# Borda/pyImSegm

Measured on AMD Instinct MI355X. Metric: Mpixels/s end-to-end SLIC+fts+GC, 2048x2048 RGB; % HBM roofline, higher is better.
Workload: dtype f64; 1 GPU; single 2048x2048 RGB uint8 per GPU, SLIC(sp_size=46, K=2025, 10 sweeps) + colour mean/std/energy + 3-class alpha-expansion GC (gc_regul=2.0, edge=model), pre-fitted GMM, host numpy in -> segm int32 in host numpy (BASELINE configs[1]); bench_config=2, images_per_launch_chain=1, images_in_flight_per_gpu=4, hardware_queues=4, input_memory=pageable numpy, input_ring=default (one rank: measured in round 4), parallelism=images sharded over 1 GPU(s), 4 in flight per GPU (one HIP stream each)

## Files before the change

include/imsegm_hip.h:

```cpp
#ifndef IMSEGM_HIP_H
#define IMSEGM_HIP_H

#include <stddef.h>
#include <stdint.h>

#ifdef __cplusplus
extern "C" {
#endif

#define IMSEGM_API __attribute__((visibility("default")))

#define IMSEGM_U8 0
#define IMSEGM_F64 1
#define IMSEGM_F32 2

#define IMSEGM_E_FUSED_PATH (-3)

#define IMSEGM_E_FIT_CAPS (-4)

typedef struct imsegm_ctx imsegm_ctx;
typedef struct imsegm_image2d imsegm_image2d;

IMSEGM_API const char *imsegm_last_error(void);
IMSEGM_API int imsegm_version(void);
IMSEGM_API int imsegm_device_count(int *count_out);
IMSEGM_API int imsegm_device_pci_bus_id(int device, char *id_out, int capacity);
IMSEGM_API int imsegm_device_mem_info(int device, size_t *free_bytes_out, size_t *total_bytes_out);
IMSEGM_API int imsegm_init(int hardware_queues);
IMSEGM_API void imsegm_debug_reload_env(void);

IMSEGM_API int imsegm_host_alloc(size_t bytes, void **ptr_out);
IMSEGM_API void imsegm_host_free(void *ptr);

IMSEGM_API int imsegm_device_alloc(int device, size_t bytes, void **ptr_out);
IMSEGM_API void imsegm_device_free(void *ptr);
IMSEGM_API int imsegm_set_device(int device);

IMSEGM_API int imsegm_ctx_create(int device, imsegm_ctx **ctx_out);
IMSEGM_API void imsegm_ctx_destroy(imsegm_ctx *ctx);
IMSEGM_API int imsegm_ctx_synchronize(imsegm_ctx *ctx);
IMSEGM_API int imsegm_ctx_stream(imsegm_ctx *ctx, void **hip_stream_out);
IMSEGM_API int imsegm_ctx_copy(imsegm_ctx *ctx, void *dst, const void *src, size_t bytes, int synchronize);

IMSEGM_API int imsegm_ctx_profile_enable(imsegm_ctx *ctx, int enable);
IMSEGM_API int imsegm_ctx_profile_reset(imsegm_ctx *ctx);
IMSEGM_API int imsegm_ctx_profile_get(imsegm_ctx *ctx, int group, double *total_ms_out, int *count_out);

IMSEGM_API int imsegm_image2d_create(imsegm_ctx *ctx, int height, int width, imsegm_image2d **img_out);
IMSEGM_API void imsegm_image2d_destroy(imsegm_image2d *img);

IMSEGM_API int imsegm_image2d_upload(imsegm_image2d *img, const void *host_pixels, int dtype);

IMSEGM_API int imsegm_image2d_slic(imsegm_image2d *img, int minmax_normalize, int n_segments, double compactness,
                        const double *taps_z, int radius_z, const double *taps_y, int radius_y,
                        const double *taps_x, int radius_x, int max_iter, int enforce_connectivity,
                        double min_size_factor, double max_size_factor, int start_label,
                        int max_candidates, int slic_zero, int *n_labels_out);

IMSEGM_API int imsegm_image2d_get_labels(imsegm_image2d *img, int64_t *labels_out);
IMSEGM_API int imsegm_image2d_set_labels(imsegm_image2d *img, const int32_t *labels, int n_labels);
IMSEGM_API long imsegm_debug_conn_general_runs(void);
IMSEGM_API int imsegm_debug_slic_sweep_runs(long *persistent_runs_out, long *fallback_runs_out);
IMSEGM_API long imsegm_debug_gc_grid_fallbacks(void);
IMSEGM_API int imsegm_image2d_enforce_connectivity(imsegm_image2d *img, const int32_t *labels, long min_size, long max_size,
                                                   int start_label, int *n_labels_out);
IMSEGM_API int imsegm_image2d_label_hist(imsegm_image2d *img, const int32_t *annot, int nb_annot, int64_t *hist_out);
IMSEGM_API int imsegm_image2d_get_lab(imsegm_image2d *img, double *lab_out);
IMSEGM_API int imsegm_image2d_get_nearest(imsegm_image2d *img, int32_t *nearest_out);

IMSEGM_API int imsegm_image2d_color_stats(imsegm_image2d *img, double *mean_out, double *energy_out, double *var_out);

IMSEGM_API int imsegm_image2d_graph(imsegm_image2d *img, int32_t *edges_out, int edge_capacity, int *n_edges_out,
                         double *centres_out, uint8_t *present_out);

IMSEGM_API int imsegm_image2d_gather(imsegm_image2d *img, const int32_t *graph_labels, const double *proba,
                          int n_classes, int32_t *segm_out, double *soft_out);

IMSEGM_API int imsegm_image2d_lm_features(imsegm_image2d *img, const double *weights, const int *n_kernels, int n_batteries, int radius,
                                          double clip, int feature_mask, double *features_out);

IMSEGM_API int imsegm_image2d_lm_features_sep(imsegm_image2d *img, const double *weights, const int *n_kernels, const int *dense_parity,
                                              const double *sep_taps, const int *sep_groups, const int *sep_rank, int n_batteries,
                                              int radius, double clip, int feature_mask, double *features_out);

IMSEGM_API int imsegm_image2d_lm_prepare(imsegm_image2d *img, const double *taps, int radius, const double *channel_mix);
IMSEGM_API int imsegm_image2d_lm_battery(imsegm_image2d *img, const double *weights, int n_kernels, int radius,
                                         double clip, double *sum_squares_out);
IMSEGM_API int imsegm_image2d_response_stats(imsegm_image2d *img, double mul, double div, double *mean_out,
                                             double *energy_out, double *var_out);
IMSEGM_API int imsegm_image2d_response_median(imsegm_image2d *img, double mul, double div, double *median_out);
IMSEGM_API int imsegm_image2d_response_mean_gradient(imsegm_image2d *img, double mul, double div, double *mean_out);
IMSEGM_API int imsegm_image2d_get_response(imsegm_image2d *img, double *planes_out);

IMSEGM_API int imsegm_volume_create(imsegm_ctx *ctx, int depth, int height, int width, imsegm_image2d **vol_out);
IMSEGM_API int imsegm_volume_upload(imsegm_image2d *vol, const void *host_voxels, int dtype, double slic_offset,
                                    double slic_scale);
IMSEGM_API int imsegm_volume_slic(imsegm_image2d *vol, int n_segments, double compactness, const double *taps_z,
                                  int radius_z, const double *taps_y, int radius_y, const double *taps_x, int radius_x,
                                  const double *spacing, int max_iter, int enforce_connectivity, double min_size_factor,
                                  double max_size_factor, int start_label, int *n_labels_out);
IMSEGM_API int imsegm_volume_label_cc(imsegm_image2d *vol, int *n_labels_out);
IMSEGM_API int imsegm_volume_gray_stats(imsegm_image2d *vol, double *mean_out, double *energy_out, double *var_out);
IMSEGM_API int imsegm_volume_graph(imsegm_image2d *vol, int32_t *edges_out, int edge_capacity, int *n_edges_out,
                                   double *centres_out, uint8_t *present_out);

IMSEGM_API int imsegm_image2d_features_color(imsegm_image2d *img, int feature_mask, double *features_out);

IMSEGM_API int imsegm_image2d_features_place(imsegm_image2d *img, int total_columns, int column);
IMSEGM_API int imsegm_image2d_get_features(imsegm_image2d *img, double *features_out, int capacity_columns);

typedef struct {
    int n_features, n_classes;
    const double *scaler_mean;
    const double *scaler_scale;
    const double *prec_chol;
    const double *mu_proj;
    const double *log_det;
    const double *log_weights;
    double const_term;
} imsegm_gmm;

#define IMSEGM_EDGE_CONST 0
#define IMSEGM_EDGE_SPATIAL 1
#define IMSEGM_EDGE_MODEL_LT 2
#define IMSEGM_EDGE_MODEL_L1 3
#define IMSEGM_EDGE_MODEL_L2 4
#define IMSEGM_EDGE_FEATURES 5
#define IMSEGM_EDGE_SPATIAL_NORM 0x100

typedef struct {
    int edge_capacity;
    int n_edges;
    int32_t *edges;
    double *edge_weights;
    int32_t *edge_weights_int;
    double *unary;
    int32_t *unary_int;
    double *centres;
    int64_t *energy;
    int keep_soft_on_device;
    int segm_u8;
    int soft_f32;
} imsegm_terms_debug;

// ... 66 lines not shown
```

pyimsegm_amd/_hip.py:

```python
import ctypes as C
import functools
import os
import threading

import numpy as np

_HERE = os.path.dirname(os.path.abspath(__file__))
LIB_PATH = os.environ.get('IMSEGM_HIP_LIBRARY') or os.path.join(_HERE, 'libimsegm_hip.so')

U8, F64, F32 = 0, 1, 2
PROFILE_GROUPS = {
    'slic_assign': 0,
    'slic': 1,
    'connectivity': 2,
    'color_stats': 3,
    'graph': 4,
    'graphcut': 5,
    'gather': 6,
    'slic_preprocess': 7,
    'terms': 8,
    'texture': 9,
}


class HipUnavailableError(RuntimeError):
    """the HIP library or a HIP device is not available (no CPU fallback exists)"""


class HipError(RuntimeError):
    """a C-ABI call returned an error status"""


class HipFusedPathError(HipError):
    """``IMSEGM_E_FUSED_PATH`` of include/imsegm_hip.h: the fused back half (``imsegm_image2d_segment`` /
    ``imsegm_image2d_graph_prepare``) does not apply to this label map on this device -- nothing is wrong with the session, the
    caller takes the staged calls (graph, terms, ``cut_general_graph``, gather) instead"""


class HipFitCapsError(HipError):
    """``IMSEGM_E_FIT_CAPS`` of include/imsegm_hip.h: the table or the model is outside the caps of the device fit
    (``imsegm_kmeans_lloyd`` / ``imsegm_mixture_em``: 16 features, 8 components, 16 restarts; the ``_wide`` pair: 17 to 256
    features, 8 components, 16 restarts) -- nothing is wrong with the context, the caller fits on the host"""


IMSEGM_E_FUSED_PATH = -3
IMSEGM_E_FIT_CAPS = -4


_lib = None
_lib_lock = threading.Lock()

_vp = C.c_void_p
_ip = C.POINTER(C.c_int)

class GmmParams(C.Structure):
    _fields_ = [('n_features', C.c_int), ('n_classes', C.c_int), ('scaler_mean', _vp), ('scaler_scale', _vp),
                ('prec_chol', _vp), ('mu_proj', _vp), ('log_det', _vp), ('log_weights', _vp), ('const_term', C.c_double)]


class TermsDebug(C.Structure):
    _fields_ = [('edge_capacity', C.c_int), ('n_edges', C.c_int), ('edges', _vp), ('edge_weights', _vp),
                ('edge_weights_int', _vp), ('unary', _vp), ('unary_int', _vp), ('centres', _vp), ('energy', _vp),
                ('keep_soft_on_device', C.c_int), ('segm_u8', C.c_int), ('soft_f32', C.c_int)]


EDGE_TYPES = {'': 0, 'const': 0, 'spatial': 1 | 0x100, 'model': 2 | 0x100, 'model_lT': 2, 'model_l1': 3, 'model_l2': 4,
              'features': 5 | 0x100}

_SIGNATURES = {
    'imsegm_last_error': (C.c_char_p, []),
    'imsegm_host_alloc': (C.c_int, [C.c_size_t, C.POINTER(_vp)]),
    'imsegm_host_free': (None, [_vp]),
    'imsegm_device_alloc': (C.c_int, [C.c_int, C.c_size_t, C.POINTER(_vp)]),
    'imsegm_device_free': (None, [_vp]),
    'imsegm_set_device': (C.c_int, [C.c_int]),
    'imsegm_ctx_stream': (C.c_int, [_vp, C.POINTER(_vp)]),
    'imsegm_ctx_copy': (C.c_int, [_vp, _vp, _vp, C.c_size_t, C.c_int]),
    'imsegm_image2d_features_color': (C.c_int, [_vp, C.c_int, _vp]),
    'imsegm_image2d_features_place': (C.c_int, [_vp, C.c_int, C.c_int]),
    'imsegm_image2d_get_features': (C.c_int, [_vp, _vp, C.c_int]),
    'imsegm_image2d_run_color': (C.c_int, [_vp, _vp, C.c_int, C.c_int, C.c_int, C.c_double, _vp, C.c_int, C.c_int, C.c_int, C.c_int,
                                           C.c_int, C.POINTER(GmmParams), C.c_int, _vp, C.c_int, C.c_double, C.c_int, _vp, _vp, _vp, _ip]),
    'imsegm_device_mem_info': (C.c_int, [C.c_int, C.POINTER(C.c_size_t), C.POINTER(C.c_size_t)]),
    'imsegm_image2d_graph_prepare': (C.c_int, [_vp]),
    'imsegm_image2d_segment': (C.c_int, [_vp, C.POINTER(GmmParams), _vp, C.c_int, _vp, C.c_int, C.c_double, C.c_int, _vp, _vp, _vp,
                                         _vp, _vp, C.POINTER(TermsDebug)]),
    'imsegm_version': (C.c_int, []),
    'imsegm_device_count': (C.c_int, [_ip]),
    'imsegm_ctx_create': (C.c_int, [C.c_int, C.POINTER(_vp)]),
    'imsegm_ctx_destroy': (None, [_vp]),
    'imsegm_ctx_synchronize': (C.c_int, [_vp]),
    'imsegm_ctx_profile_enable': (C.c_int, [_vp, C.c_int]),
    'imsegm_ctx_profile_reset': (C.c_int, [_vp]),
    'imsegm_ctx_profile_get': (C.c_int, [_vp, C.c_int, C.POINTER(C.c_double), _ip]),
    'imsegm_image2d_create': (C.c_int, [_vp, C.c_int, C.c_int, C.POINTER(_vp)]),
    'imsegm_image2d_destroy': (None, [_vp]),
    'imsegm_image2d_upload': (C.c_int, [_vp, _vp, C.c_int]),
    'imsegm_image2d_slic': (C.c_int, [_vp, C.c_int, C.c_int, C.c_double, _vp, C.c_int, _vp, C.c_int, _vp, C.c_int,
                                      C.c_int, C.c_int, C.c_double, C.c_double, C.c_int, C.c_int, C.c_int, _ip]),
    'imsegm_image2d_get_labels': (C.c_int, [_vp, _vp]),
    'imsegm_image2d_set_labels': (C.c_int, [_vp, _vp, C.c_int]),
    'imsegm_image2d_enforce_connectivity': (C.c_int, [_vp, _vp, C.c_long, C.c_long, C.c_int, _vp]),
    'imsegm_debug_conn_general_runs': (C.c_long, []),
    'imsegm_debug_slic_sweep_runs': (C.c_int, [_vp, _vp]),
    'imsegm_debug_gc_grid_fallbacks': (C.c_long, []),
    'imsegm_assume_bg_on_boundary': (C.c_int, [_vp, _vp, C.c_int, C.c_int, _vp, C.c_int, _ip]),
    'imsegm_image2d_all_finite': (C.c_int, [_vp, _ip]),
    'imsegm_image2d_lm_features': (C.c_int, [_vp, _vp, _vp, C.c_int, C.c_int, C.c_double, C.c_int, _vp]),
    'imsegm_batch2d_create': (C.c_int, [_vp, C.c_int, C.c_int, C.c_int, C.POINTER(_vp)]),
    'imsegm_batch2d_destroy': (None, [_vp]),
    'imsegm_batch2d_run_color': (C.c_int, [_vp, C.c_int, _vp, C.c_int, C.c_int, C.c_int, C.c_double, _vp, C.c_int, C.c_int, C.c_int,
                                           C.c_int, _vp, C.c_int, _vp, C.c_int, C.c_double, C.c_int, _vp, _vp, _vp]),
    'imsegm_batch2d_device_ptr': (C.c_int, [_vp, C.c_int, C.c_int, C.POINTER(_vp)]),
    'imsegm_device_pci_bus_id': (C.c_int, [C.c_int, C.c_char_p, C.c_int]),
    'imsegm_init': (C.c_int, [C.c_int]),
    'imsegm_debug_reload_env': (None, []),
    'imsegm_image2d_label_hist': (C.c_int, [_vp, _vp, C.c_int, _vp]),
    'imsegm_image2d_get_lab': (C.c_int, [_vp, _vp]),
    'imsegm_image2d_get_nearest': (C.c_int, [_vp, _vp]),
    'imsegm_image2d_color_stats': (C.c_int, [_vp, _vp, _vp, _vp]),
    'imsegm_image2d_graph': (C.c_int, [_vp, _vp, C.c_int, _ip, _vp, _vp]),
    'imsegm_image2d_gather': (C.c_int, [_vp, _vp, _vp, C.c_int, _vp, _vp]),
    'imsegm_image2d_lm_prepare': (C.c_int, [_vp, _vp, C.c_int, _vp]),
    'imsegm_image2d_lm_features_sep': (C.c_int, [_vp, _vp, _vp, _vp, _vp, _vp, _vp, C.c_int, C.c_int, C.c_double, C.c_int, _vp]),
    'imsegm_image2d_lm_battery': (C.c_int, [_vp, _vp, C.c_int, C.c_int, C.c_double, C.POINTER(C.c_double)]),
    'imsegm_image2d_response_stats': (C.c_int, [_vp, C.c_double, C.c_double, _vp, _vp, _vp]),
    'imsegm_image2d_response_median': (C.c_int, [_vp, C.c_double, C.c_double, _vp]),
    'imsegm_image2d_response_mean_gradient': (C.c_int, [_vp, C.c_double, C.c_double, _vp]),
    'imsegm_image2d_get_response': (C.c_int, [_vp, _vp]),
    'imsegm_image2d_device_ptr': (C.c_int, [_vp, C.c_int, C.POINTER(_vp)]),
    'imsegm_volume_create': (C.c_int, [_vp, C.c_int, C.c_int, C.c_int, C.POINTER(_vp)]),
    'imsegm_volume_upload': (C.c_int, [_vp, _vp, C.c_int, C.c_double, C.c_double]),
    'imsegm_volume_slic': (C.c_int, [_vp, C.c_int, C.c_double, _vp, C.c_int, _vp, C.c_int, _vp, C.c_int, _vp, C.c_int,
                                     C.c_int, C.c_double, C.c_double, C.c_int, _ip]),
    'imsegm_volume_label_cc': (C.c_int, [_vp, _ip]),
    'imsegm_volume_gray_stats': (C.c_int, [_vp, _vp, _vp, _vp]),
    'imsegm_volume_graph': (C.c_int, [_vp, _vp, C.c_int, _ip, _vp, _vp]),
    'imsegm_image2d_median': (C.c_int, [_vp, _vp]),
    'imsegm_image2d_mean_gradient': (C.c_int, [_vp, _vp]),
    'imsegm_label_hist2d': (C.c_int, [_vp, _vp, C.c_int, C.c_int, _vp, C.c_int, _vp, C.c_int, C.c_int, C.c_int, _vp]),
    'imsegm_ray_features_binary2d': (C.c_int, [_vp, _vp, C.c_int, C.c_int, _vp, C.c_int, _vp, C.c_int, C.c_int, _vp]),
    'imsegm_cut_general_graph': (C.c_int, [_vp, _vp, C.c_int, _vp, _vp, C.c_int, C.c_int, _vp, C.c_int, _vp,
                                           C.POINTER(C.c_int64)]),
    'imsegm_kmeans_lloyd': (C.c_int, [_vp, _vp, C.c_long, C.c_int, _vp, C.c_int, C.c_int, C.c_int, C.c_double, _vp, _vp, _vp, _vp, _vp]),
    'imsegm_mixture_em': (C.c_int, [_vp, C.c_int, C.c_int, _vp, _vp, _vp, _vp, C.c_double, C.c_double, C.c_int, _vp, _vp, _vp, _vp,
                                    _vp, _vp, _vp, _vp]),
    'imsegm_kmeans_lloyd_wide': (C.c_int, [_vp, _vp, C.c_long, C.c_int, _vp, C.c_int, C.c_int, C.c_int, C.c_double, _vp, _vp, _vp, _vp,
                                           _vp]),
    'imsegm_mixture_em_wide': (C.c_int, [_vp, C.c_int, C.c_int, _vp, _vp, _vp, _vp, C.c_double, C.c_double, C.c_int, _vp, _vp, _vp, _vp,
                                         _vp, _vp, _vp, _vp]),
}

EXPORTED_SYMBOLS = tuple(_SIGNATURES)


def load_library():
    global _lib
    with _lib_lock:
        if _lib is None:
            if not os.path.exists(LIB_PATH):
                raise HipUnavailableError(
                    'libimsegm_hip.so is not built (%s); run `python -m pyimsegm_amd.build`' % LIB_PATH)
            try:
                lib = C.CDLL(LIB_PATH)
            except OSError as ex:
                raise HipUnavailableError('cannot load %s: %s' % (LIB_PATH, ex))
            for name, (res, args) in _SIGNATURES.items():
                fn = getattr(lib, name)
                fn.restype = res
                fn.argtypes = args
            _lib = lib
    return _lib


def init(hardware_queues=8):
    status = load_library().imsegm_init(int(hardware_queues))
    if status < 0:
        raise HipError(load_library().imsegm_last_error().decode('utf-8', 'replace'))
    if status == 0:
        os.environ.setdefault('GPU_MAX_HW_QUEUES', str(int(hardware_queues)))
    return status == 0


def device_pci_bus_id(device=0):
    buf = C.create_string_buffer(64)
    _check(load_library().imsegm_device_pci_bus_id(int(device), buf, 64))
# ... 398 lines not shown
                        or not segm_out.flags.c_contiguous or not segm_out.flags.writeable:
                    raise ValueError('segm_out must be a writeable C-contiguous %s array of shape %r' % (want_dtype, tuple(self.shape)))
                out['segm'] = segm_out
            else:
                out['segm'] = alloc(self.shape, want_dtype)
        if want_soft:
            out['soft'] = alloc(self.shape + (nc, ), np.float32 if soft_f32 else np.float64)
        if want_graph_labels or debug:
            out['graph_labels'] = np.empty(k, dtype=np.int32)
        if want_proba or debug:
            out['proba'] = np.empty((k, nc), dtype=np.float64)
        dbg = None
        if debug or keep_soft_on_device or segm_u8 or soft_f32:
            dbg = TermsDebug()
            dbg.keep_soft_on_device = int(bool(keep_soft_on_device))
            dbg.segm_u8, dbg.soft_f32 = int(segm_u8), int(soft_f32)
        if debug:
            cap = (16 if len(self.shape) == 3 else 3) * k + 64
            ndim = len(self.shape)
            out.update(edges=np.empty((cap, 2), np.int32), edge_weights=np.empty(cap), edge_weights_int=np.empty(cap, np.int32),
                       unary=np.empty((k, nc)), unary_int=np.empty((k, nc), np.int32), centres=np.empty((k, ndim)),
                       energy=np.zeros(1, np.int64))
            dbg.edge_capacity = cap
            for name in ('edges', 'edge_weights', 'edge_weights_int', 'unary', 'unary_int', 'centres', 'energy'):
                setattr(dbg, name, _ptr(out[name]))
        _check(load_library().imsegm_image2d_segment(
            self._h, C.byref(gmm.params) if gmm is not None else None, _ptr(pr), nc, _ptr(pairwise), code, float(edge_cost),
            int(bool(use_graphcut)), _ptr(cl), _ptr(out.get('segm')), _ptr(out.get('soft')), _ptr(out.get('graph_labels')),
            _ptr(out.get('proba')), C.byref(dbg) if dbg is not None else None))
        if debug:
            ne = dbg.n_edges
            for name in ('edges', 'edge_weights', 'edge_weights_int'):
                out[name] = out[name][:ne]
            out['energy'] = int(out['energy'][0])
        return out

    def slic(self, n_segments, compactness, sigma=1., normalize=2, max_iter=10, enforce_connectivity=True,
             min_size_factor=0.5, max_size_factor=3., start_label=0, max_candidates=0, slic_zero=False):
        taps = gaussian_taps(sigma)
        r = -1 if taps is None else len(taps) - 1
        n_out = C.c_int(0)
        _check(load_library().imsegm_image2d_slic(
            self._h, int(normalize), int(n_segments), float(compactness), _ptr(taps), r, _ptr(taps), r, _ptr(taps), r,
            int(max_iter), int(bool(enforce_connectivity)), float(min_size_factor), float(max_size_factor),
            int(start_label), int(max_candidates), int(bool(slic_zero)), C.byref(n_out)))
        self.n_labels = n_out.value
        return self.n_labels

    def get_labels(self):
        out = np.empty(self.shape, dtype=np.int64)
        _check(load_library().imsegm_image2d_get_labels(self._h, _ptr(out)))
        return out

    def get_labels_int32(self):
        out = np.empty(self.shape, dtype=np.int32)
        src = _device_array(self, 0, self.shape, '<i4').__cuda_array_interface__['data'][0]
        self.ctx.copy(out.ctypes.data, src, out.nbytes, synchronize=True)
        return out

    def enforce_connectivity(self, labels, min_size, max_size, start_label=0):
        labels = np.ascontiguousarray(labels, dtype=np.int32)
        if labels.shape != self.shape:
            raise ValueError('label map %r does not match image %r' % (labels.shape, self.shape))
        n_out = C.c_int(0)
        _check(load_library().imsegm_image2d_enforce_connectivity(self._h, _ptr(labels), int(min_size), int(max_size),
                                                                  int(start_label), C.byref(n_out)))
        self.n_labels = n_out.value
        return self.get_labels()

    def set_labels(self, labels, n_labels=None):
        labels = np.ascontiguousarray(labels, dtype=np.int32)
        if labels.shape != self.shape:
            raise ValueError('label map %r does not match image %r' % (labels.shape, self.shape))
        if labels.size and labels.min() < 0:
            raise ValueError('labels must be non-negative')
        if n_labels is None:
            n_labels = int(labels.max()) + 1
        elif labels.size and int(labels.max()) >= n_labels:
            raise ValueError('label %d is out of range for n_labels = %d' % (int(labels.max()), n_labels))
        _check(load_library().imsegm_image2d_set_labels(self._h, _ptr(labels), int(n_labels)))
        self.n_labels = int(n_labels)
        return self

    def label_hist(self, annot, nb_annot=None):
        annot = np.ascontiguousarray(annot, dtype=np.int32)
        if annot.shape != self.shape:
            raise ValueError('annotation %r does not match the session %r' % (annot.shape, self.shape))
        if nb_annot is None:
            nb_annot = int(annot.max()) + 1 if annot.size else 1
        out = np.empty((self.n_labels, int(nb_annot)), dtype=np.int64)
        _check(load_library().imsegm_image2d_label_hist(self._h, _ptr(annot), int(nb_annot), _ptr(out)))
        return out

    def get_lab(self):
        out = np.empty((3,) + self.shape, dtype=np.float64)
        _check(load_library().imsegm_image2d_get_lab(self._h, _ptr(out)))
        return out

    def get_nearest(self):
        out = np.empty(self.shape, dtype=np.int32)
        _check(load_library().imsegm_image2d_get_nearest(self._h, _ptr(out)))
        return out

    def color_stats(self, mean=True, energy=True, var=True):
        k = self.n_labels
        m = np.empty((k, 3), dtype=np.float64) if mean else None
        e = np.empty((k, 3), dtype=np.float64) if energy else None
        v = np.empty((k, 3), dtype=np.float64) if var else None
        _check(load_library().imsegm_image2d_color_stats(self._h, _ptr(m), _ptr(e), _ptr(v)))
        return m, e, v

    def lm_prepare(self, sigma=150.):
        taps = gaussian_taps(sigma)
        radius = len(taps) - 1
        full = np.concatenate([taps[:0:-1], taps])
        mix = np.zeros((3, 3))
        for c_out in range(3):
            for j in range(-radius, radius + 1):
                i = (c_out + j) % 6
                mix[c_out, i if i < 3 else 5 - i] += full[j + radius]
        _check(load_library().imsegm_image2d_lm_prepare(self._h, _ptr(taps), radius, _ptr(np.ascontiguousarray(mix))))
        return self

    def lm_battery(self, battery, clip):
        battery = np.asarray(battery, dtype=np.float64)
        nk, side = battery.shape[0], battery.shape[1]
        if battery.ndim != 3 or battery.shape[2] != side or side % 2 != 1:
            raise ValueError('wrong battery dim %r' % (battery.shape, ))
        pad = {1: 1, 2: 2, 3: 4, 4: 4, 5: 8, 6: 8, 7: 8, 8: 8}.get(nk)
        if pad is None:
            raise ValueError('at most 8 kernels per battery')
        if pad != nk:
            battery = np.concatenate([battery, np.repeat(battery[-1:], pad - nk, axis=0)], axis=0)
        weights = np.ascontiguousarray(battery[:, ::-1, ::-1].transpose(2, 1, 0))
        ssq = C.c_double(0)
        _check(load_library().imsegm_image2d_lm_battery(self._h, _ptr(weights), pad, side // 2, float(clip), C.byref(ssq)))
        return float(np.sqrt(ssq.value))

    @staticmethod
    def _battery_weights(battery):
        battery = np.asarray(battery, dtype=np.float64)
        nk, side = battery.shape[0], battery.shape[1]
        if battery.ndim != 3 or battery.shape[2] != side or side % 2 != 1:
            raise ValueError('wrong battery dim %r' % (battery.shape, ))
        pad = {1: 1, 2: 2, 3: 4, 4: 4, 5: 8, 6: 8, 7: 8, 8: 8}.get(nk)
        if pad is None:
            raise ValueError('at most 8 kernels per battery')
        if pad != nk:
            battery = np.concatenate([battery, np.repeat(battery[-1:], pad - nk, axis=0)], axis=0)
        return np.ascontiguousarray(battery[:, ::-1, ::-1].transpose(2, 1, 0)), pad, side // 2

    SEPARABLE_TOLERANCE, SEPARABLE_MAX_RANK = 1e-13, 2

    MIRROR_TOLERANCE = 1e-12

    @classmethod
    def _mirror_pairs(cls, dense):
        left = list(range(len(dense)))
        pairs = []
        while left:
            a = left.pop(0)
            mirrored = dense[a][:, ::-1]
            bound = cls.MIRROR_TOLERANCE * np.abs(dense[a]).max()
            for b in left:
                hit = [m for m in (1., -1.) if np.abs(dense[b] - m * mirrored).max() <= bound]
                if hit:
# ... 493 lines not shown
```

pyimsegm_amd/csrc/api.hip:

```cpp
#include "../../include/imsegm_hip.h"
#include "slic.h"

#include <atomic>
#include <cstdio>
#include <cstdlib>
#include <cstring>
#include <vector>

namespace imsegm {

static thread_local std::string g_error;

void set_error(const std::string &msg) { g_error = msg; }

bool hip_ok(hipError_t e, const char *what, const char *file, int line)
{
    if (e == hipSuccess) return true;
    char buf[512];
    snprintf(buf, sizeof(buf), "HIP error %d (%s) in `%s` at %s:%d", (int)e, hipGetErrorString(e), what, file, line);
    g_error = buf;
    return false;
}

static Knobs read_knobs()
{
    auto flag = [](const char *n) { return getenv(n) != nullptr; };
    auto num = [](const char *n, int dflt) { const char *e = getenv(n); return e ? atoi(e) : dflt; };
    Knobs k;
    k.slic_graph = flag("IMSEGM_SLIC_GRAPH");
    k.pre_3pass = flag("IMSEGM_PRE_3PASS");
    k.separate_finalize = flag("IMSEGM_SEPARATE_FINALIZE");
    k.fuse_finalize = flag("IMSEGM_FUSE_FINALIZE");
    k.conn_general = flag("IMSEGM_CONN_GENERAL");
    k.gc_no_topo_regs = flag("IMSEGM_GC_NO_TOPO_REGS");
    k.sep_wide_tile = flag("IMSEGM_SEP_WIDE_TILE");
    k.cc_merge_full = flag("IMSEGM_CC_MERGE_FULL");
    k.label_general = flag("IMSEGM_LABEL_GENERAL");
    k.terms_one_workgroup = flag("IMSEGM_TERMS_ONE_WORKGROUP");
    k.adjacency_table = flag("IMSEGM_ADJACENCY_TABLE");
    k.brick_cap = num("IMSEGM_BRICK_CAP", 0);
    k.gc_lds_level = num("IMSEGM_GC_LDS_LEVEL", 4);
    k.gc_threads = num("IMSEGM_GC_THREADS", 0);
    k.gc_grid_min_sites = num("IMSEGM_GC_GRID_MIN_SITES", 0);
    k.gc_grid_blocks = num("IMSEGM_GC_GRID_BLOCKS", 0);
    k.gc_one_workgroup = flag("IMSEGM_GC_ONE_WORKGROUP");
    k.gc_grid_test_absent = flag("IMSEGM_GC_GRID_TEST_ABSENT");
    k.fused_bitmap_mb = num("IMSEGM_FUSED_BITMAP_MB", 0);
    const char *d = getenv("IMSEGM_PHASE_DUMP");
    k.phase_dump = d ? d : "";
    return k;
}
static std::atomic<const Knobs *> g_knobs{ nullptr };
const Knobs &knobs()
{
    const Knobs *k = g_knobs.load(std::memory_order_acquire);
    if (!k) {
        const Knobs *fresh = new Knobs(read_knobs());
        if (g_knobs.compare_exchange_strong(k, fresh, std::memory_order_acq_rel)) k = fresh;
        else delete fresh;
    }
    return *k;
}
void reload_knobs() { g_knobs.store(new Knobs(read_knobs()), std::memory_order_release); }

}

#include "session.h"

std::atomic<bool> g_runtime_started{ false };

extern "C" {

int imsegm_host_alloc(size_t bytes, void **ptr_out)
{
    g_runtime_started.store(true);
    if (!ptr_out) {
        set_error("null argument");
        return -1;
    }
    HIP_TRY(hipHostMalloc(ptr_out, bytes ? bytes : 1, hipHostMallocDefault));
    return 0;
}

void imsegm_host_free(void *ptr)
{
    if (ptr) (void)hipHostFree(ptr);
}

int imsegm_device_alloc(int device, size_t bytes, void **ptr_out)
{
    g_runtime_started.store(true);
    if (!ptr_out) {
        set_error("null argument");
        return -1;
    }
    HIP_TRY(hipSetDevice(device));
    HIP_TRY(hipMalloc(ptr_out, bytes ? bytes : 1));
    return 0;
}

void imsegm_device_free(void *ptr)
{
    if (ptr) (void)hipFree(ptr);
}

int imsegm_set_device(int device)
{
    g_runtime_started.store(true);
    HIP_TRY(hipSetDevice(device));
    return 0;
}

int imsegm_ctx_stream(imsegm_ctx *ctx, void **stream_out)
{
    if (bind(ctx)) return -1;
    *stream_out = ctx->stream;
    return 0;
}

int imsegm_ctx_copy(imsegm_ctx *ctx, void *dst, const void *src, size_t bytes, int synchronize)
{
    if (bind(ctx)) return -1;
    HIP_TRY(hipMemcpyAsync(dst, src, bytes, hipMemcpyDefault, ctx->stream));
    if (synchronize) HIP_TRY(hipStreamSynchronize(ctx->stream));
    return 0;
}

const char *imsegm_last_error(void) { return g_error.c_str(); }
int imsegm_version(void) { return 100; }
// ... 84 lines not shown
    if (bind(ctx)) return -1;
    HIP_TRY(hipStreamSynchronize(ctx->stream));
    return 0;
}

int imsegm_ctx_profile_enable(imsegm_ctx *ctx, int enable)
{
    if (bind(ctx)) return -1;
    ctx->collect();
    ctx->profile = enable != 0;
    return 0;
}

int imsegm_ctx_profile_reset(imsegm_ctx *ctx)
{
    if (bind(ctx)) return -1;
    ctx->collect();
    for (int i = 0; i < PG_COUNT; ++i) {
        ctx->acc_ms[i] = 0;
        ctx->acc_n[i] = 0;
    }
    return 0;
}

int imsegm_ctx_profile_get(imsegm_ctx *ctx, int group, double *total_ms_out, int *count_out)
{
    if (bind(ctx)) return -1;
    if (group < 0 || group >= PG_COUNT) {
        set_error("bad profile group");
        return -1;
    }
    ctx->collect();
    *total_ms_out = ctx->acc_ms[group];
    *count_out = ctx->acc_n[group];
    return 0;
}

int imsegm_image2d_create(imsegm_ctx *ctx, int height, int width, imsegm_image2d **img_out)
{
    if (bind(ctx)) return -1;
    if (height <= 0 || width <= 0 || (long)height * width > 0x3fffffffL) {
        set_error("bad image size");
        return -1;
    }
    imsegm_image2d *im = new imsegm_image2d();
    im->ctx = ctx;
    im->H = height;
    im->W = width;
    im->n = (size_t)height * width;
    *img_out = im;
    return 0;
}

void imsegm_image2d_destroy(imsegm_image2d *im)
{
    if (!im) return;
    (void)hipSetDevice(im->ctx->device);
    (void)hipStreamSynchronize(im->ctx->stream);
    DevBuf *all[] = { &im->img, &im->labA, &im->labB, &im->nearest, &im->labels, &im->conn_i32, &im->conn_u8, &im->small,
                      &im->cent, &im->tiles, &im->feat, &im->graph, &im->gather_lut, &im->gather_out_i, &im->gather_out_f,
                      &im->tex_planes, &im->tex_resp, &im->tex_small, &im->tex_aux, &im->vol_cent, &im->annot, &im->hist, &im->featK, &im->seg,
                      &im->gseg, &im->narrow };
    for (auto b : all) b->release();
    if (im->slic_fail_host) (void)hipHostFree(im->slic_fail_host);
    if (im->slic_exec) (void)hipGraphExecDestroy(im->slic_exec);
    delete im;
}

int imsegm_image2d_upload(imsegm_image2d *im, const void *host_pixels, int dtype)
{
    if (!im || bind(im->ctx)) return -1;
    if (wrong_kind(im, false)) return -1;
    im->tex_ready = false;
    size_t es = dtype == IMSEGM_U8 ? 1 : dtype == IMSEGM_F32 ? 4 : dtype == IMSEGM_F64 ? 8 : 0;
    if (!es) {
        set_error("unsupported dtype");
        return -1;
    }
    size_t bytes = im->n * 3 * es;
    if (im->img.ensure(bytes + 16)) return -1;
    HIP_TRY(hipMemcpyAsync(im->img.p, host_pixels, bytes, hipMemcpyHostToDevice, im->ctx->stream));
    if (!is_pinned(host_pixels)) HIP_TRY(hipStreamSynchronize(im->ctx->stream));
    im->dtype = dtype;
    im->feat_mask = 0;
    im->place_F = 0;
    return 0;
}

long imsegm_debug_conn_general_runs(void) { return conn_general_runs(); }

void imsegm_debug_reload_env(void) { reload_knobs(); }

long imsegm_debug_gc_grid_fallbacks(void) { return gc_grid_fallbacks(); }

int imsegm_debug_slic_sweep_runs(long *persistent_runs_out, long *fallback_runs_out)
{
    slic_sweep_counters(persistent_runs_out, fallback_runs_out);
    return 0;
}

int imsegm_image2d_all_finite(imsegm_image2d *im, int *all_finite_out)
{
    if (!im || !all_finite_out || bind(im->ctx)) return -1;
    if (im->dtype < 0 || !im->img.p) {
        set_error("all_finite needs an uploaded image or volume");
        return -1;
    }
    *all_finite_out = 1;
    if (im->dtype == IMSEGM_U8) return 0;
    hipStream_t st = im->ctx->stream;
    if (ensure_small(im)) return -1;
    unsigned int *count = reinterpret_cast<unsigned int *>(im->small.as<unsigned char>() + 256);
    const size_t values = im->is_volume ? im->n : im->n * 3;
    if (launch_count_nonfinite(im->img.p, im->dtype, values, count, st)) return -1;
    unsigned int bad = 0;
    HIP_TRY(hipMemcpyAsync(&bad, count, sizeof(bad), hipMemcpyDeviceToHost, st));
    HIP_TRY(hipStreamSynchronize(st));
    *all_finite_out = bad == 0;
    return 0;
}

int imsegm_image2d_device_ptr(imsegm_image2d *im, int which, void **ptr_out)
{
    if (!im || !ptr_out) {
        set_error("null argument");
        return -1;
    }
    if (which == 3 && (!im->have_labels || im->feat_mask == 0 || im->feat_F < 1)) {
        set_error("device_ptr: no resident feature table");
        return -1;
    }
    DevBuf *b = which == 0 ? &im->labels : which == 1 ? &im->gather_out_i : which == 2 ? &im->gather_out_f :
                which == 3 ? &im->featK : nullptr;
    if (!b || !b->p) {
        set_error("device_ptr: buffer not available");
        return -1;
    }
    *ptr_out = b->p;
    return 0;
}


}
```

pyimsegm_amd/csrc/api_fused.hip:

```cpp
#include "backhalf.h"

int imsegm::take_placement(imsegm_image2d *im, int own_F, bool to_host, int *table_F, int *col0)
{
    *table_F = own_F;
    *col0 = 0;
    if (im->place_F <= 0) return 0;
    const int total = im->place_F, column = im->place_col;
    im->place_F = 0;
    if (column + own_F > total) {
        set_error("features_place: the columns of this descriptor group do not fit the table");
        return -1;
    }
    if (to_host && own_F != total) {
        set_error("features_place: a group placed into a wider table stays on the device (imsegm_image2d_get_features reads the table)");
        return -1;
    }
    *table_F = total;
    *col0 = column;
    return 0;
}

extern "C" {

int imsegm_cut_general_graph(imsegm_ctx *ctx, const int32_t *edges, int n_edges, const double *edge_weights,
// ... 29 lines not shown
        return -1;
    }
    int32_t *ui = (int32_t *)(host + o_u), *wi = (int32_t *)(host + o_w), *si = (int32_t *)(host + o_s);
    int32_t *he = (int32_t *)(host + o_e), *arc_start = (int32_t *)(host + o_as), *arc_to = (int32_t *)(host + o_at);
    int32_t *arc_rev = (int32_t *)(host + o_ar), *edge_arc = (int32_t *)(host + o_ea);
    double mu = 0, mw = 0, mp = -DBL_MAX;
    for (size_t i = 0; i < (size_t)K * C; ++i) mu = std::max(mu, fabs(unary_cost[i]));
    for (int i = 0; i < E; ++i) mw = std::max(mw, fabs(edge_weights[i]));
    for (int i = 0; i < C * C; ++i) mp = std::max(mp, pairwise_cost[i]);
    double dwf = ((E > 0 && mw * mp > mu) ? mw * mp : mu) + 1e-10;
    for (size_t i = 0; i < (size_t)K * C; ++i) ui[i] = (int32_t)((unary_cost[i] / dwf) * 100000);
    for (int i = 0; i < E; ++i) wi[i] = (int32_t)((edge_weights[i] / dwf) * 1000);
    for (int i = 0; i < C * C; ++i) si[i] = (int32_t)(pairwise_cost[i] * 100);
    int smax = 0;
    for (int i = 0; i < C * C; ++i) smax = std::max(smax, std::abs(si[i]));
    for (int i = 0; i < E; ++i)
        if ((long long)std::abs(wi[i]) * smax > 10000000LL) {
            set_error("cut_general_graph: smoothness term is larger than GCO_MAX_ENERGYTERM");
            return -1;
        }
    if (E > 0) memcpy(he, edges, (size_t)E * 8);
    for (int i = 0; i <= K; ++i) arc_start[i] = 0;
    for (int j = 0; j < E; ++j) {
        arc_start[edges[2 * j] + 1]++;
        arc_start[edges[2 * j + 1] + 1]++;
    }
    for (int i = 0; i < K; ++i) arc_start[i + 1] += arc_start[i];
    {
        std::vector<int32_t> fill(arc_start, arc_start + K);
        for (int j = 0; j < E; ++j) {
            int a = edges[2 * j], b = edges[2 * j + 1];
            int ia = fill[a]++, ib = fill[b]++;
            arc_to[ia] = b;
            arc_to[ib] = a;
            arc_rev[ia] = ib;
            arc_rev[ib] = ia;
            edge_arc[2 * j] = ia;
            edge_arc[2 * j + 1] = ib;
        }
    }
    unsigned char *dev = ctx->gc_buf.as<unsigned char>();
    void *work = dev;
    unsigned char *io = dev + work_bytes;
    int32_t *d_lab = (int32_t *)(io + o_lab);
    long long *d_energy = (long long *)(io + o_en);
    int32_t *d_status = (int32_t *)(io + o_st);
    HIP_TRY(hipMemcpyAsync(io, host, up_bytes, hipMemcpyHostToDevice, st));
    HIP_TRY(hipMemsetAsync(d_status, 0, 4, st));
    GcProblem p;
    p.K = K; p.C = C; p.E = E;
    p.edges = (int32_t *)(io + o_e); p.w = (int32_t *)(io + o_w); p.unary = (int32_t *)(io + o_u); p.smooth = (int32_t *)(io + o_s);
    p.metric = smooth_is_metric(si, C);
    int sp = ctx->begin(PG_GC);
    if (launch_alpha_expansion(p, (int32_t *)(io + o_as), (int32_t *)(io + o_at), (int32_t *)(io + o_ar), (int32_t *)(io + o_ea),
                               n_iter, d_lab, d_energy, d_status, work, st))
        return -1;
    ctx->end(sp);
    HIP_TRY(hipMemcpyAsync(host + o_lab, d_lab, io_bytes - o_lab, hipMemcpyDeviceToHost, st));
    HIP_TRY(hipStreamSynchronize(st));
    memcpy(labels_out, host + o_lab, (size_t)K * 4);
    long long energy = *reinterpret_cast<long long *>(host + o_en);
    const int32_t misc[4] = { K, E, 0, *reinterpret_cast<int32_t *>(host + o_st) };
    if (backhalf_status(misc, 1)) return -1;
    if (energy_out) *energy_out = energy;
    return 0;
}


int imsegm_image2d_features_color(imsegm_image2d *im, int feature_mask, double *features_out)
{
    if (!im || bind(im->ctx)) return -1;
    if (!im->have_labels || im->dtype < 0) {
        set_error("features_color needs an uploaded image and a label map");
        return -1;
    }
    if (feature_mask < 1 || feature_mask > 7) {
        set_error("features_color: feature_mask is a combination of 1 (mean), 2 (std), 4 (energy)");
        return -1;
    }
    imsegm_ctx *ctx = im->ctx;
    hipStream_t st = ctx->stream;
    const int K = im->n_labels;
    double maxabs = 255.0;
    if (im->dtype != IMSEGM_U8) {
        if (ensure_small(im)) return -1;
        unsigned long long *keys = im->small.as<unsigned long long>();
        double *minmax = reinterpret_cast<double *>(keys + 2);
        if (launch_minmax(im->img.p, im->dtype, im->is_volume ? im->n : im->n * 3, keys, minmax, st)) return -1;
        double mm[2];
        HIP_TRY(hipMemcpyAsync(mm, minmax, 16, hipMemcpyDeviceToHost, st));
        HIP_TRY(hipStreamSynchronize(st));
        maxabs = std::max(fabs(mm[0]), fabs(mm[1]));
        if (!(maxabs < 1e300)) maxabs = 1e300;
    }
    if (im->feat.ensure(stats_scratch_bytes(K))) return -1;
    const StatsScratch ss = stats_scratch_at(im->feat.p, K);
    int sp = ctx->begin(PG_STATS);
    int rc;
    if (im->is_volume)
        rc = launch_color_stats(im->img.p, im->dtype, im->labels.as<int32_t>(), im->D * im->H, im->W, K, maxabs, (feature_mask & 2) != 0,
                                ss.acc, ss.mean, ss.energy, ss.var, ss.mean32, st, 1, 0, 1.0, 1.0, 0);
    else
        rc = launch_color_stats(im->img.p, im->dtype, im->labels.as<int32_t>(), im->H, im->W, K, maxabs, (feature_mask & 2) != 0, ss.acc,
                                ss.mean, ss.energy, ss.var, ss.mean32, st, 0, 0, 1.0, 1.0, -1);
    if (rc) return -1;
    const int F = color_feature_columns(feature_mask);
    int table_F = F, col0 = 0;
    if (take_placement(im, F, features_out != nullptr, &table_F, &col0)) return -1;
    if (im->featK.ensure((size_t)K * table_F * 8 + 64)) return -1;
    if (launch_features_assemble(ss.mean, ss.energy, ss.var, K, feature_mask, im->featK.as<double>(), st, table_F, col0)) return -1;
    ctx->end(sp);
    im->feat_mask = table_F == F ? feature_mask : 8;
    im->feat_F = table_F;
    if (features_out) {
        HIP_TRY(hipMemcpyAsync(features_out, im->featK.p, (size_t)K * F * 8, hipMemcpyDeviceToHost, st));
        HIP_TRY(hipStreamSynchronize(st));
    }
    return 0;
}

int imsegm_image2d_features_place(imsegm_image2d *im, int total_columns, int column)
{
    if (!im || bind(im->ctx)) return -1;
    if (total_columns < 1 || column < 0 || column >= total_columns) {
        set_error("features_place: 0 <= column < total_columns is required");
        return -1;
    }
    im->place_F = total_columns;
    im->place_col = column;
    return 0;
}

int imsegm_image2d_get_features(imsegm_image2d *im, double *features_out, int capacity_columns)
{
    if (!im || bind(im->ctx)) return -1;
    if (!im->have_labels || im->feat_mask == 0 || im->feat_F < 1) {
        set_error("get_features: no resident feature table");
        return -1;
    }
    if (!features_out || capacity_columns != im->feat_F) {
        set_error("get_features: the table has a different number of columns");
        return -1;
    }
    hipStream_t st = im->ctx->stream;
    HIP_TRY(hipMemcpyAsync(features_out, im->featK.p, (size_t)im->n_labels * im->feat_F * 8, hipMemcpyDeviceToHost, st));
    HIP_TRY(hipStreamSynchronize(st));
    return 0;
}

static int default_edge_capacity(const imsegm_image2d *im, int K) { return im->is_volume ? 16 * K + 64 : 3 * K + 64; }

static GraphPlan graph_plan(const imsegm_image2d *im, int K, int edge_capacity)
{
    auto al = [](size_t v) { return (v + 63) & ~(size_t)63; };
    GraphPlan g;
    g.K = K;
    g.Ecap = edge_capacity > 0 ? edge_capacity : default_edge_capacity(im, K);
    g.words = cdiv(K, 32);
    g.table = im->is_volume && ((double)K * (double)g.words * 4.0 > 256e6 || knobs().adjacency_table);
    g.cap = g.table ? 64 : 0;
    size_t d = 0;
    g.o_head = d; d += 64;
    g.o_edges = d; d += al((size_t)g.Ecap * 8);
    g.o_as = d; d += al((size_t)(K + 1) * 4);
    g.o_at = d; d += al((size_t)g.Ecap * 8);
    g.o_ar = d; d += al((size_t)g.Ecap * 8);
    g.o_ea = d; d += al((size_t)g.Ecap * 8);
    g.o_deg = d; d += al((size_t)K * 4);
    g.o_dlow = d; d += al((size_t)K * 4);
    g.o_es = d; d += al((size_t)K * 4);
    g.o_cent = d; d += al((size_t)K * 3 * 8);
    g.o_present = d; d += al((size_t)K);
    g.o_store = d; d += al(g.table ? (size_t)K * g.cap * 4 : (size_t)K * g.words * 4);
    g.o_cacc = d; d += al((size_t)K * 4 * 8);
    g.o_wp = d; d += g.table ? 0 : al((size_t)K * g.words * 4);
    g.bytes = d + 256;
    return g;
}

__global__ void k_graph_head(int32_t *head, int K)
{
    head[0] = K;
    head[1] = 0;
    head[2] = 0;
}

static int graph_enqueue(imsegm_image2d *im, const GraphPlan &g, int32_t *K_dev, int32_t *E_dev)
{
    imsegm_ctx *ctx = im->ctx;
    hipStream_t st = ctx->stream;
    if (im->gseg.ensure(g.bytes)) return -1;
    unsigned char *gb = im->gseg.as<unsigned char>();
    int32_t *head = reinterpret_cast<int32_t *>(gb + g.o_head);
    if (!K_dev || g.table) hipLaunchKernelGGL(k_graph_head, 1, 1, 0, st, head, g.K);
    if (!K_dev) {
        K_dev = head;
        E_dev = head + 1;
    }
    int32_t *store = reinterpret_cast<int32_t *>(gb + g.o_store);
    long long *cacc = reinterpret_cast<long long *>(gb + g.o_cacc);
    double *centres = reinterpret_cast<double *>(gb + g.o_cent);
    int sp = ctx->begin(PG_GRAPH);
    if (g.table) {
        if (launch_vol_adjacency_table(im->labels.as<int32_t>(), im->D, im->H, im->W, g.K, store, g.cap, head + 2, cacc, centres, gb + g.o_present, st))
            return -1;
        if (launch_graph_csr_table(store, K_dev, g.K, g.cap, head + 2, reinterpret_cast<int32_t *>(gb + g.o_deg), reinterpret_cast<int32_t *>(gb + g.o_dlow),
                                   reinterpret_cast<int32_t *>(gb + g.o_as), reinterpret_cast<int32_t *>(gb + g.o_es), E_dev, g.Ecap,
                                   reinterpret_cast<int32_t *>(gb + g.o_edges), reinterpret_cast<int32_t *>(gb + g.o_at),
                                   reinterpret_cast<int32_t *>(gb + g.o_ar), reinterpret_cast<int32_t *>(gb + g.o_ea), st))
            return -1;
    } else {
        uint32_t *bitmap = reinterpret_cast<uint32_t *>(store);
        if (im->is_volume) {
            if (launch_vol_adjacency(im->labels.as<int32_t>(), im->D, im->H, im->W, g.K, g.words, bitmap, cacc, centres, gb + g.o_present, st)) return -1;
        } else if (launch_adjacency_bitmap(im->labels.as<int32_t>(), im->H, im->W, g.K, bitmap, cacc, centres, gb + g.o_present, st)) {
            return -1;
        }
        if (launch_graph_csr(bitmap, K_dev, g.K, g.words, reinterpret_cast<int32_t *>(gb + g.o_wp), reinterpret_cast<int32_t *>(gb + g.o_deg),
                             reinterpret_cast<int32_t *>(gb + g.o_dlow), reinterpret_cast<int32_t *>(gb + g.o_as),
                             reinterpret_cast<int32_t *>(gb + g.o_es), E_dev, g.Ecap, reinterpret_cast<int32_t *>(gb + g.o_edges),
                             reinterpret_cast<int32_t *>(gb + g.o_at), reinterpret_cast<int32_t *>(gb + g.o_ar),
                             reinterpret_cast<int32_t *>(gb + g.o_ea), st))
            return -1;
    }
    ctx->end(sp);
    return 0;
}

static int graph_store_fits(imsegm_image2d *im, const GraphPlan &g)
{
    if (g.table) return 0;
    const double pair_bytes = 2.0 * (double)g.K * (double)g.words * 4.0;
    const int cap_mb = knobs().fused_bitmap_mb;
    if (cap_mb > 0 && pair_bytes > 1048576.0 * cap_mb) {
        set_error("segment: too many labels for the fused path (adjacency bitmap: IMSEGM_FUSED_BITMAP_MB)");
        return IMSEGM_E_FUSED_PATH;
    }
    if (pair_bytes > 16e6) {
        size_t free_b = 0, total_b = 0;
        HIP_TRY(hipMemGetInfo(&free_b, &total_b));
        const double usable = (double)free_b + (double)im->gseg.cap - 0.1 * (double)total_b;
        if (pair_bytes > usable || pair_bytes > 48e9) {
            set_error("segment: too many labels for the fused path (adjacency bitmap: the device has no room for it)");
            return IMSEGM_E_FUSED_PATH;
        }
    }
    return 0;
}

int imsegm_image2d_graph_prepare(imsegm_image2d *im)
{
    if (!im || bind(im->ctx)) return -1;
    if (!im->have_labels) {
        set_error("graph_prepare needs a label map");
        return -1;
    }
    im->graph_ready = false;
    const GraphPlan g = graph_plan(im, im->n_labels, 0);
    if (int rc = graph_store_fits(im, g)) return rc;
    if (graph_enqueue(im, g, nullptr, nullptr)) return -1;
    im->gplan = g;
    im->graph_ready = true;
    return 0;
}

static int segment_impl(imsegm_image2d *im, const imsegm_gmm *gmm, const double *proba, int n_classes,
                        const double *pairwise, int edge_type, double edge_cost, int use_graphcut,
                        const int32_t *classes_lut, int32_t *segm_out, double *soft_out, int32_t *graph_labels_out,
                        double *proba_out, imsegm_terms_debug *debug_out, int edge_capacity, int *edges_found)
{
    if (!im || bind(im->ctx)) return -1;
    if (!im->have_labels) {
        set_error("segment needs a label map");
        return -1;
    }
    const int K = im->n_labels, C = n_classes;
    if (C < 1 || C > 16 || !pairwise || (!gmm && !proba)) {
        set_error("segment: 1..16 classes, a pairwise matrix and either a class model or probabilities are required");
        return -1;
    }
    BackHalf bh;
    if (decode_edge_type(edge_type, &bh.edge_code, &bh.spatial_norm)) return -1;
    const bool need_features = gmm != nullptr || bh.edge_code == 5;
    if (need_features && im->feat_mask == 0) {
        set_error("segment: the class model / edge type needs the resident feature table (imsegm_image2d_features_color)");
        return -1;
    }
    const int F = need_features ? im->feat_F : 0;
    if (gmm && (gmm->n_features != F || gmm->n_classes != C)) {
        set_error("segment: class model does not match the resident features / number of classes");
        return -1;
    }
    if (check_pairwise(pairwise, C)) return -1;
    const bool prepared = im->graph_ready && im->gplan.K == K && (edge_capacity <= 0 || im->gplan.Ecap >= edge_capacity);
    const GraphPlan g = prepared ? im->gplan : graph_plan(im, K, edge_capacity);
    im->graph_ready = false;
    if (!prepared)
        if (int rc = graph_store_fits(im, g)) return rc;
// ... 17 lines not shown
    ctx->mark_stage_in_flight();
    int32_t *misc = bh.misc();
    bh.K_dev = misc; bh.E_dev = misc + 1;
    if (!prepared && graph_enqueue(im, g, bh.K_dev, bh.E_dev)) return -1;
    unsigned char *gb = im->gseg.as<unsigned char>();
    int32_t *ghead = reinterpret_cast<int32_t *>(gb + g.o_head);
    if (prepared) bh.E_dev = ghead + 1;
    bh.edges = reinterpret_cast<int32_t *>(gb + g.o_edges); bh.centres = reinterpret_cast<double *>(gb + g.o_cent);
    bh.arc_start = reinterpret_cast<int32_t *>(gb + g.o_as); bh.arc_to = reinterpret_cast<int32_t *>(gb + g.o_at);
    bh.arc_rev = reinterpret_cast<int32_t *>(gb + g.o_ar); bh.edge_arc = reinterpret_cast<int32_t *>(gb + g.o_ea);
    if (im->gather_out_i.ensure(n * 4)) return -1;
    const bool want_soft = soft_out != nullptr || (debug_out && debug_out->keep_soft_on_device);
    if (want_soft && im->gather_out_f.ensure(n * C * 8)) return -1;
    bh.features = need_features ? im->featK.as<double>() : nullptr;
    bh.labels = im->labels.as<int32_t>(); bh.n = n;
    bh.segm_out = im->gather_out_i.as<int32_t>(); bh.soft_out = want_soft ? im->gather_out_f.as<double>() : nullptr;
    bh.K_cap = K; bh.Ecap = g.Ecap; bh.ndim = im->is_volume ? 3 : 2;
    bh.edge_cost = edge_cost; bh.use_graphcut = use_graphcut;
    if (backhalf_enqueue(ctx, bh)) return -1;
    const bool segm_u8 = debug_out && debug_out->segm_u8, soft_f32 = debug_out && debug_out->soft_f32;
    if ((segm_u8 && segm_out) || (soft_f32 && soft_out)) {
        const size_t off_soft = (n + 255) & ~(size_t)255;
        if (im->narrow.ensure(off_soft + n * C * 4 + 64)) return -1;
        unsigned char *nb = im->narrow.as<unsigned char>();
        if (segm_u8 && segm_out) {
            if (launch_narrow_labels_u8(im->gather_out_i.as<int32_t>(), nb, n, st)) return -1;
            HIP_TRY(hipMemcpyAsync(segm_out, nb, n, hipMemcpyDeviceToHost, st));
            segm_out = nullptr;
        }
        if (soft_f32 && soft_out) {
            float *f32 = reinterpret_cast<float *>(nb + off_soft);
            if (launch_narrow_soft_f32(im->gather_out_f.as<double>(), f32, n * C, st)) return -1;
            HIP_TRY(hipMemcpyAsync(soft_out, f32, n * C * 4, hipMemcpyDeviceToHost, st));
            soft_out = nullptr;
        }
    }
    if (segm_out) HIP_TRY(hipMemcpyAsync(segm_out, im->gather_out_i.p, n * 4, hipMemcpyDeviceToHost, st));
    if (soft_out) HIP_TRY(hipMemcpyAsync(soft_out, im->gather_out_f.p, n * C * 8, hipMemcpyDeviceToHost, st));
    if (graph_labels_out) HIP_TRY(hipMemcpyAsync(graph_labels_out, bh.at<int32_t>(bh.scr.d_gl), (size_t)K * 4, hipMemcpyDeviceToHost, st));
    if (proba_out) HIP_TRY(hipMemcpyAsync(proba_out, bh.at<double>(bh.scr.d_proba), (size_t)K * C * 8, hipMemcpyDeviceToHost, st));
    int32_t hmisc[4] = { 0, 0, 0, 0 }, hgraph[4] = { 0, 0, 0, 0 };
    HIP_TRY(hipMemcpyAsync(hmisc, misc, sizeof(hmisc), hipMemcpyDeviceToHost, st));
    if (prepared || g.table) HIP_TRY(hipMemcpyAsync(hgraph, ghead, sizeof(hgraph), hipMemcpyDeviceToHost, st));
    if (debug_out) {
        if (debug_out->unary) HIP_TRY(hipMemcpyAsync(debug_out->unary, bh.at<double>(bh.scr.d_unary), (size_t)K * C * 8, hipMemcpyDeviceToHost, st));
        if (debug_out->unary_int) HIP_TRY(hipMemcpyAsync(debug_out->unary_int, bh.at<int32_t>(bh.scr.d_unary_i), (size_t)K * C * 4, hipMemcpyDeviceToHost, st));
        if (debug_out->centres) HIP_TRY(hipMemcpyAsync(debug_out->centres, bh.centres, (size_t)K * bh.ndim * 8, hipMemcpyDeviceToHost, st));
        if (debug_out->energy) HIP_TRY(hipMemcpyAsync(debug_out->energy, misc + 4, 8, hipMemcpyDeviceToHost, st));
    }
    HIP_TRY(hipStreamSynchronize(st));
    const int E = prepared ? hgraph[1] : hmisc[1];
    if (g.table && hgraph[2]) {
        set_error("segment: too many labels for the fused path (a label with more than 64 neighbours in the neighbour table)");
        return IMSEGM_E_FUSED_PATH;
    }
    if (debug_out) {
        debug_out->n_edges = E;
        const int Ec = std::min(E, debug_out->edge_capacity);
        if (Ec > 0) {
            if (debug_out->edges) HIP_TRY(hipMemcpy(debug_out->edges, bh.edges, (size_t)Ec * 8, hipMemcpyDeviceToHost));
            if (debug_out->edge_weights) HIP_TRY(hipMemcpy(debug_out->edge_weights, bh.at<double>(bh.scr.d_w), (size_t)Ec * 8, hipMemcpyDeviceToHost));
            if (debug_out->edge_weights_int) HIP_TRY(hipMemcpy(debug_out->edge_weights_int, bh.at<int32_t>(bh.scr.d_wi), (size_t)Ec * 4, hipMemcpyDeviceToHost));
        }
    }
    if (edges_found) *edges_found = E;
    return backhalf_status(hmisc, use_graphcut);
}

int imsegm_image2d_segment(imsegm_image2d *im, const imsegm_gmm *gmm, const double *proba, int n_classes,
                           const double *pairwise, int edge_type, double edge_cost, int use_graphcut,
                           const int32_t *classes_lut, int32_t *segm_out, double *soft_out, int32_t *graph_labels_out,
                           double *proba_out, imsegm_terms_debug *debug_out)
{
    int found = 0;
    int rc = segment_impl(im, gmm, proba, n_classes, pairwise, edge_type, edge_cost, use_graphcut, classes_lut, segm_out, soft_out,
                          graph_labels_out, proba_out, debug_out, 0, &found);
    if (rc == -2)
        rc = segment_impl(im, gmm, proba, n_classes, pairwise, edge_type, edge_cost, use_graphcut, classes_lut, segm_out, soft_out,
                          graph_labels_out, proba_out, debug_out, found + 64, &found);
    return rc == -2 ? -1 : rc;
}


int imsegm_image2d_run_color(imsegm_image2d *im, const void *host_pixels, int dtype, int minmax_normalize, int n_segments,
                             double compactness, const double *taps, int radius, int max_iter, int start_label, int slic_zero,
                             int feature_mask, const imsegm_gmm *gmm, int n_classes, const double *pairwise, int edge_type,
                             double edge_cost, int use_graphcut, const int32_t *classes_lut, int32_t *segm_out, double *soft_out,
                             int *n_labels_out)
{
    if (imsegm_image2d_upload(im, host_pixels, dtype)) return -1;
    int n_labels = 0;
    if (imsegm_image2d_slic(im, minmax_normalize, n_segments, compactness, taps, radius, taps, radius, taps, radius, max_iter, 1, 0.5,
                            3.0, start_label, 0, slic_zero, &n_labels))
        return -1;
    if (n_labels_out) *n_labels_out = n_labels;
    if (imsegm_image2d_features_color(im, feature_mask, nullptr)) return -1;
    return imsegm_image2d_segment(im, gmm, nullptr, n_classes, pairwise, edge_type, edge_cost, use_graphcut, classes_lut, segm_out,
                                  soft_out, nullptr, nullptr, nullptr);
}

}
```

pyimsegm_amd/csrc/api_image2d.hip:

```cpp
#include "session.h"

int slic_geometry(int H, int W, int n_segments, double compactness, int minmax_normalize, int max_candidates, int slic_zero,
                  SlicState &s, SlicGeometry &geo)
{
    long shape[3] = { 1, H, W };
    GridAxis ax[3];
    regular_grid3(shape, n_segments, ax);
    long ny = 0, nx = 0;
    for (long y = ax[1].start; y < H; y += ax[1].step) ny++;
    for (long x = ax[2].start; x < W; x += ax[2].step) nx++;
    const int K = (int)(ny * nx);
    if (K < 1) {
        set_error("slic: empty centroid grid");
        return -1;
    }
    double fsteps[3];
    for (int i = 0; i < 3; ++i) fsteps[i] = ax[i].all ? 1.0 : (double)ax[i].step;
    float step = (float)std::max(fsteps[0], std::max(fsteps[1], fsteps[2]));
    GridAxis axk[3];
    regular_grid3(shape, K, axk);
    memset(&s, 0, sizeof(s));
    s.H = H; s.W = W; s.K = K;
    s.step_y = axk[1].all ? 1 : (int)axk[1].step;
    s.step_x = axk[2].all ? 1 : (int)axk[2].step;
// ... 110 lines not shown
        if (!phase_buf) {
            HIP_TRY(hipMalloc(&phase_buf, PHASE_SLOTS * 32 * sizeof(long long)));
            HIP_TRY(hipMemset(phase_buf, 0, PHASE_SLOTS * 32 * sizeof(long long)));
        }
        s.phase_prof = phase_buf;
    }
    if (!im->slic_fail_host) HIP_TRY(hipHostMalloc((void **)&im->slic_fail_host, 64, hipHostMallocDefault));
    slic_place_state(s, geo, im->cent.as<unsigned char>(), im->tiles.as<unsigned char>(), premax, im->slic_fail_host);
    double *init_dev = nullptr;

    const ProfHook hook = ctx->hook();
    const bool use_graph = !ctx->profile && !s.phase_prof && knobs().slic_graph;
    bool used_persistent = false;
    if (use_graph) {
        struct SlicGraphKey {
            SlicState s;
            const double *lab;
            int32_t *labels;
            int max_iter, max_cand;
        } key;
        memset(&key, 0, sizeof(key));
        memcpy(&key.s, &s, sizeof(s));
        key.lab = im->labA.as<double>(); key.labels = im->nearest.as<int32_t>();
        key.max_iter = max_iter; key.max_cand = max_candidates;
        const bool same = im->slic_exec && im->slic_key.size() == sizeof(key) && !memcmp(im->slic_key.data(), &key, sizeof(key));
        if (!same) {
            if (im->slic_exec) {
                HIP_TRY(hipGraphExecDestroy(im->slic_exec));
                im->slic_exec = nullptr;
            }
            if (slic_prepare_device()) return -1;
            hipGraph_t graph = nullptr;
            HIP_TRY(hipStreamBeginCapture(st, hipStreamCaptureModeThreadLocal));
            SlicState captured = s;
            captured.done = nullptr;
            const int rc = launch_slic_iterations(captured, im->labA.as<double>(), init_dev, im->nearest.as<int32_t>(), max_iter,
                                                  max_candidates, hook, st);
            const hipError_t ec = hipStreamEndCapture(st, &graph);
            if (rc || ec != hipSuccess || !graph) {
                if (graph) (void)hipGraphDestroy(graph);
                if (!rc) set_error(std::string("slic: stream capture failed: ") + hipGetErrorString(ec));
                return -1;
            }
            const hipError_t ei = hipGraphInstantiate(&im->slic_exec, graph, nullptr, nullptr, 0);
            (void)hipGraphDestroy(graph);
            if (ei != hipSuccess) {
                im->slic_exec = nullptr;
                set_error(std::string("slic: graph instantiation failed: ") + hipGetErrorString(ei));
                return -1;
            }
            im->slic_key.assign(reinterpret_cast<unsigned char *>(&key), reinterpret_cast<unsigned char *>(&key) + sizeof(key));
        }
        HIP_TRY(hipGraphLaunch(im->slic_exec, st));
    } else {
        if (launch_slic_iterations(s, im->labA.as<double>(), init_dev, im->nearest.as<int32_t>(), max_iter, max_candidates, hook, st,
                                   &used_persistent))
            return -1;
    }

    if (s.phase_prof) {
        std::vector<long long> all((size_t)PHASE_SLOTS * 32);
        HIP_TRY(hipMemcpy(all.data(), s.phase_prof, all.size() * 8, hipMemcpyDeviceToHost));
        HIP_TRY(hipMemset(s.phase_prof, 0, all.size() * 8));
        bool any = false;
        for (size_t i = 15; i < all.size() && !any; i += 16) any = all[i] != 0;
        if (any && !knobs().phase_dump.empty()) {
            FILE *f = fopen(knobs().phase_dump.c_str(), "wb");
            if (f) {
                fwrite(all.data(), 8, all.size(), f);
                fclose(f);
            }
        }
        long long h[32] = { 0 };
        for (size_t i = 0; i < all.size(); ++i) h[i % 32] += all[i];
        for (int v = 0; v < 2; ++v) {
            const long long *q = h + v * 16;
            if (!q[15]) continue;
            fprintf(stderr, "[phase prof %s] waves=%lld  cycles/wave:", v ? "accum" : "last ", q[15]);
            for (int j = 0; j < 10; ++j) fprintf(stderr, " p%d=%.0f", j, (double)q[j] / (double)q[15]);
            fprintf(stderr, "\n");
        }
    }
    int n_labels = K + start_label;
    for (int attempt = 0; attempt < 2; ++attempt) {
        if (attempt == 1) {
            slic_sweep_note_fallback();
            SlicState plain = s;
            plain.done = nullptr;
            if (launch_slic_iterations(plain, im->labA.as<double>(), init_dev, im->nearest.as<int32_t>(), max_iter, max_candidates, hook, st))
                return -1;
        }
        if (enforce_connectivity) {
            double segment_size = (double)n / (double)K;
            long min_size = (long)(min_size_factor * segment_size);
            long max_size = (long)(max_size_factor * segment_size);
            if (im->conn_i32.ensure(conn_i32_bytes(n, H, W)) || im->conn_u8.ensure(2 * n + 64)) return -1;
            ConnWork w = make_conn_work(im);
            int spc = ctx->begin(PG_CONN);
            if (launch_enforce_connectivity(im->nearest.as<int32_t>(), 1, H, W, min_size, max_size, start_label, w,
                                            im->labels.as<int32_t>(), &n_labels, st))
                return -1;
            ctx->end(spc);
        } else {
            if (start_label != 0) {
                set_error("enforce_connectivity=False is only supported with start_label=0");
                return -1;
            }
            HIP_TRY(hipMemcpyAsync(im->labels.p, im->nearest.p, n * 4, hipMemcpyDeviceToDevice, st));
            if (used_persistent) HIP_TRY(hipStreamSynchronize(st));
        }
        if (!used_persistent || *im->slic_fail_host == 0) break;
        static const bool verbose = getenv("IMSEGM_DEBUG_SWEEPS") != nullptr;
        if (verbose) fprintf(stderr, "[slic sweeps] %d x %d, K = %d: handed back, code %d\n", H, W, K, *im->slic_fail_host);
        used_persistent = false;
    }
    ctx->end(sp_all);
    im->n_labels = n_labels;
    im->have_labels = true;
    im->labels_connected = false;
    im->graph_ready = false;
    if (n_labels_out) *n_labels_out = n_labels;
    return 0;
}

int imsegm_image2d_get_labels(imsegm_image2d *im, int64_t *labels_out)
{
    if (!im || bind(im->ctx)) return -1;
    if (!im->have_labels) {
        set_error("no label map");
        return -1;
    }
    std::vector<int32_t> tmp(im->n);
    HIP_TRY(hipMemcpyAsync(tmp.data(), im->labels.p, im->n * 4, hipMemcpyDeviceToHost, im->ctx->stream));
    HIP_TRY(hipStreamSynchronize(im->ctx->stream));
    for (size_t i = 0; i < im->n; ++i) labels_out[i] = tmp[i];
    return 0;
}

int imsegm_image2d_set_labels(imsegm_image2d *im, const int32_t *labels, int n_labels)
{
    if (!im || bind(im->ctx)) return -1;
    if (n_labels < 1) {
        set_error("n_labels must be positive");
        return -1;
    }
    if (im->labels.ensure(im->n * 4)) return -1;
    HIP_TRY(hipMemcpyAsync(im->labels.p, labels, im->n * 4, hipMemcpyHostToDevice, im->ctx->stream));
    HIP_TRY(hipStreamSynchronize(im->ctx->stream));
    im->n_labels = n_labels;
    im->have_labels = true;
    im->labels_connected = false;
    im->graph_ready = false;
    return 0;
}

int imsegm_image2d_enforce_connectivity(imsegm_image2d *im, const int32_t *labels, long min_size, long max_size, int start_label,
                                        int *n_labels_out)
{
    if (!im || bind(im->ctx)) return -1;
    if (!labels || min_size < 0 || max_size < 1) {
        set_error("enforce_connectivity: label map, min_size >= 0 and max_size >= 1 are required");
        return -1;
    }
    if (start_label != 0 && start_label != 1) {
        set_error("start_label should be 0 or 1.");
        return -1;
    }
    hipStream_t st = im->ctx->stream;
    const size_t n = im->n;
    if (im->nearest.ensure(n * 4) || im->labels.ensure(n * 4)) return -1;
    if (im->conn_i32.ensure(conn_i32_bytes(n, im->D == 1 ? im->H : 0, im->D == 1 ? im->W : 0)) || im->conn_u8.ensure(2 * n + 64)) return -1;
    HIP_TRY(hipMemcpyAsync(im->nearest.p, labels, n * 4, hipMemcpyHostToDevice, st));
    ConnWork w = make_conn_work(im);
    int n_labels = 0;
    if (launch_enforce_connectivity(im->nearest.as<int32_t>(), im->D, im->H, im->W, min_size, max_size, start_label, w,
                                    im->labels.as<int32_t>(), &n_labels, st))
        return -1;
    im->n_labels = n_labels;
    im->have_labels = true;
    im->labels_connected = false;
    im->graph_ready = false;
    if (n_labels_out) *n_labels_out = n_labels;
    return 0;
}

int imsegm_image2d_label_hist(imsegm_image2d *im, const int32_t *annot, int nb_annot, int64_t *hist_out)
{
    if (!im || bind(im->ctx)) return -1;
    if (!im->have_labels) {
        set_error("label_hist needs a label map (run slic or set_labels first)");
        return -1;
    }
    if (!annot || !hist_out || nb_annot < 1) {
        set_error("label_hist: annotation, output and a positive number of annotation labels are required");
        return -1;
    }
    const size_t bins = (size_t)im->n_labels * (size_t)nb_annot;
    if (bins > ((size_t)1 << 31)) {
        set_error("label_hist: histogram of more than 2^31 bins");
        return -1;
    }
    hipStream_t st = im->ctx->stream;
    if (im->annot.ensure(im->n * 4 + 32) || im->hist.ensure(bins * 8)) return -1;
    HIP_TRY(hipMemcpyAsync(im->annot.p, annot, im->n * 4, hipMemcpyHostToDevice, st));
    if (launch_label_hist(im->labels.as<int32_t>(), im->annot.as<int32_t>(), im->n, im->n_labels, nb_annot,
                          im->hist.as<unsigned long long>(), st))
        return -1;
    HIP_TRY(hipMemcpyAsync(hist_out, im->hist.p, bins * 8, hipMemcpyDeviceToHost, st));
    HIP_TRY(hipStreamSynchronize(st));
    return 0;
}

int imsegm_image2d_get_lab(imsegm_image2d *im, double *lab_out)
{
    if (!im || bind(im->ctx)) return -1;
    if (wrong_kind(im, false)) return -1;
    if (im->labA.cap < 3 * im->n * 8) {
        set_error("slic has not been run");
        return -1;
    }
    HIP_TRY(hipMemcpyAsync(lab_out, im->labA.p, 3 * im->n * 8, hipMemcpyDeviceToHost, im->ctx->stream));
    HIP_TRY(hipStreamSynchronize(im->ctx->stream));
    return 0;
}

int imsegm_image2d_get_nearest(imsegm_image2d *im, int32_t *nearest_out)
{
    if (!im || bind(im->ctx)) return -1;
    if (im->nearest.cap < im->n * 4) {
        set_error("slic has not been run");
        return -1;
    }
    HIP_TRY(hipMemcpyAsync(nearest_out, im->nearest.p, im->n * 4, hipMemcpyDeviceToHost, im->ctx->stream));
    HIP_TRY(hipStreamSynchronize(im->ctx->stream));
    return 0;
}

int imsegm_image2d_color_stats(imsegm_image2d *im, double *mean_out, double *energy_out, double *var_out)
{
    if (!im || bind(im->ctx)) return -1;
    if (wrong_kind(im, false)) return -1;
    if (!im->have_labels || im->dtype < 0) {
        set_error("color_stats needs an uploaded image and a label map");
        return -1;
    }
    imsegm_ctx *ctx = im->ctx;
    hipStream_t st = ctx->stream;
    double maxabs = 255.0;
    if (im->dtype != IMSEGM_U8) {
        if (ensure_small(im)) return -1;
        unsigned long long *keys = im->small.as<unsigned long long>();
        double *minmax = reinterpret_cast<double *>(keys + 2);
        if (launch_minmax(im->img.p, im->dtype, im->n * 3, keys, minmax, st)) return -1;
        double mm[2];
        HIP_TRY(hipMemcpyAsync(mm, minmax, 16, hipMemcpyDeviceToHost, st));
        HIP_TRY(hipStreamSynchronize(st));
        maxabs = std::max(fabs(mm[0]), fabs(mm[1]));
        if (!(maxabs < 1e300)) maxabs = 1e300;
    }
    return stats_run(im, im->img.p, im->dtype, maxabs, 0, 0, 1.0, 1.0, mean_out, energy_out, var_out);
}

int imsegm_image2d_graph(imsegm_image2d *im, int32_t *edges_out, int edge_capacity, int *n_edges_out,
                         double *centres_out, uint8_t *present_out)
// ... 123 lines not shown
```

pyimsegm_amd/csrc/batch.hip:

```cpp
#include "backhalf.h"

#include <string>

struct imsegm_batch2d {
    imsegm_ctx *ctx = nullptr;
    int B = 0, H = 0, W = 0;
    size_t n = 0;
    DevBuf arena;
    size_t slice = 0;
    std::vector<unsigned char> key;
    int *fail_host = nullptr;
    void *pinned = nullptr;
    size_t pinned_cap = 0;
    int last_n = 0;
    std::vector<int> n_labels;
};

namespace {

using namespace imsegm;

inline size_t al256(size_t v) { return (v + 255) & ~(size_t)255; }

struct Layout {
// ... 136 lines not shown
    if (!(compactness > 0) || n_segments < 1 || max_iter < 1 || (start_label != 0 && start_label != 1)) {
        set_error("slic: n_segments, compactness and max_iter must be positive, start_label 0 or 1");
        return -1;
    }
    if (feature_mask < 1 || feature_mask > 7 || !gmm || C < 1 || C > 16 || !pairwise) {
        set_error("batch2d_run_color: colour features (mask 1..7), a device class model, 1..16 classes and a pairwise matrix are required");
        return -1;
    }
    BackHalf bh;
    if (decode_edge_type(edge_type, &bh.edge_code, &bh.spatial_norm)) return -1;
    const int F = color_feature_columns(feature_mask);
    if (gmm->n_features != F || gmm->n_classes != C) {
        set_error("segment: class model does not match the resident features / number of classes");
        return -1;
    }
    if (check_pairwise(pairwise, C)) return -1;
    Taps tz, ty, tx;
    if (fill_taps(tz, taps, radius) || fill_taps(ty, taps, radius) || fill_taps(tx, taps, radius)) return -1;
    if (radius > 8 || knobs().pre_3pass) {
        set_error("batch2d_run_color: blur radius above 8 (sigma > 2) takes the single-image path");
        return -1;
    }

    SlicState s;
    SlicGeometry geo;
    if (slic_geometry(H, W, n_segments, compactness, minmax_normalize, 0, 0, s, geo)) return -1;
    const int K = geo.K;
    const double segment_size = (double)n / (double)K;
    const long min_size = (long)(0.5 * segment_size), max_size = (long)(3.0 * segment_size);
    if (min_size < 1) {
        set_error("batch2d_run_color: superpixels of under two pixels take the single-image path");
        return -1;
    }
    const Layout L = make_layout(H, W, es, K, geo.n_tiles, min_size, C, F);
    const size_t slice = L.total;
    const size_t stage_row = al256(std::max<size_t>(L.par.bytes, 256));
    const size_t arena_bytes = slice * bt->B + stage_row * bt->B + 4096;
    const bool same = bt->key.size() == sizeof(L) && !memcmp(bt->key.data(), &L, sizeof(L)) && bt->slice == slice && bt->arena.cap >= arena_bytes;
    if (!same) {
        HIP_TRY(hipStreamSynchronize(st));
        if (bt->arena.ensure(arena_bytes)) return -1;
        HIP_TRY(hipMemsetAsync(bt->arena.p, 0, bt->arena.cap, st));
        bt->slice = slice;
        bt->key.assign(reinterpret_cast<const unsigned char *>(&L), reinterpret_cast<const unsigned char *>(&L) + sizeof(L));
    }
    if (!bt->fail_host) HIP_TRY(hipHostMalloc((void **)&bt->fail_host, 64, hipHostMallocDefault));
    unsigned char *base = bt->arena.as<unsigned char>();
    unsigned char *stage_dev = base + slice * bt->B;
    ZBatch zb;
    zb.nz = n_images;
    zb.zs = slice;
    bt->last_n = n_images;

    bool all_pinned = true;
    for (int b = 0; b < n_images; ++b) {
        if (!host_pixels[b]) {
            set_error("batch2d_run_color: null image");
            return -1;
        }
        HIP_TRY(hipMemcpyAsync(base + (size_t)b * slice + L.img, host_pixels[b], n * 3 * es, hipMemcpyHostToDevice, st));
        all_pinned = all_pinned && is_pinned(host_pixels[b]);
    }
    if (!all_pinned) HIP_TRY(hipStreamSynchronize(st));

    unsigned long long *keys = reinterpret_cast<unsigned long long *>(base + L.small);
    double *minmax = reinterpret_cast<double *>(keys + 2);
    double *premax = minmax + 2;
    double *lab = reinterpret_cast<double *>(base + L.lab);
    int32_t *nearest = reinterpret_cast<int32_t *>(base + L.nearest), *labels = reinterpret_cast<int32_t *>(base + L.labels);
    const int sp_all = ctx->begin(PG_SLIC);
    const int sp_pre = ctx->begin(PG_PRE);
    if (launch_minmax(base + L.img, dtype, n * 3, keys, minmax, st, premax, zb)) return -1;
    if (launch_preprocess_color2d(base + L.img, dtype, H, W, minmax_normalize, minmax, tz, ty, tx, 1.0 / compactness, lab, nullptr, premax,
                                  st, true, zb))
        return -1;
    ctx->end(sp_pre);
    slic_place_state(s, geo, base + L.cent, base + L.tiles, premax, bt->fail_host);
    const ProfHook hook = ctx->hook();
    bool fused_update = false;
    if (launch_slic_iterations(s, lab, nullptr, nearest, max_iter, 0, hook, st, &fused_update, zb)) return -1;

    ConnWork w = conn_work_from(reinterpret_cast<int32_t *>(base + L.conn_i32), L.conn_i32_bytes, base + L.conn_u8, n);
    std::vector<int> &nl = bt->n_labels;
    for (int attempt = 0; attempt < 2; ++attempt) {
        if (attempt == 1) {
            slic_sweep_note_fallback();
            SlicState plain = s;
            plain.done = nullptr;
            if (launch_slic_iterations(plain, lab, nullptr, nearest, max_iter, 0, hook, st, nullptr, zb)) return -1;
        }
        const int spc = ctx->begin(PG_CONN);
        if (launch_enforce_connectivity_batch(nearest, H, W, min_size, max_size, start_label, w, labels, nl.data(), st, zb,
                                              reinterpret_cast<int32_t *>(stage_dev)))
            return -1;
        ctx->end(spc);
        if (!fused_update || *bt->fail_host == 0) break;
        fused_update = false;
    }
    for (int b = 0; b < n_images; ++b) {
        if (nl[b] >= 0) continue;
        unsigned char *sb = base + (size_t)b * slice;
        ConnWork wb = conn_work_from(reinterpret_cast<int32_t *>(sb + L.conn_i32), L.conn_i32_bytes, sb + L.conn_u8, n);
        int got = 0;
        if (launch_enforce_connectivity(reinterpret_cast<int32_t *>(sb + L.nearest), 1, H, W, min_size, max_size, start_label, wb,
                                        reinterpret_cast<int32_t *>(sb + L.labels), &got, st))
            return -1;
        nl[b] = got;
    }
    ctx->end(sp_all);
    int K_cap = 1;
    for (int b = 0; b < n_images; ++b) {
        if (nl[b] > L.Kb) {
            set_error("batch2d_run_color: more labels than the bound the buffers were sized for");
            return -1;
        }
        K_cap = std::max(K_cap, nl[b]);
        if (n_labels_out) n_labels_out[b] = nl[b];
    }
    const int words = cdiv(K_cap, 32);
    const int Ecap = std::min(L.Ecap, 3 * K_cap + 64);

    {
        const StatsScratch ss = stats_scratch_at(base + L.feat, L.Kb);
        const double *mm_dev = nullptr;
        if (dtype != IMSEGM_U8) {
            if (launch_minmax(base + L.img, dtype, n * 3, keys, minmax, st, nullptr, zb)) return -1;
            mm_dev = minmax;
        }
        const int sps = ctx->begin(PG_STATS);
        if (launch_color_stats(base + L.img, dtype, labels, H, W, K_cap, 255.0, (feature_mask & 2) != 0, ss.acc, ss.mean, ss.energy, ss.var,
                               ss.mean32, st, 0, 0, 1.0, 1.0, -1, nullptr, zb, mm_dev))
            return -1;
        if (launch_features_assemble(ss.mean, ss.energy, ss.var, K_cap, feature_mask, reinterpret_cast<double *>(base + L.featK), st, 0, 0, zb))
            return -1;
        ctx->end(sps);
    }

    unsigned char *seg = base + L.seg;
    if (batch_pinned(bt, stage_row * n_images + 64)) return -1;
    unsigned char *host = static_cast<unsigned char *>(bt->pinned);
    memset(host, 0, stage_row);
    bh.par = L.par; bh.scr = L.scr; bh.C = C; bh.F = F;
    param_fill(bh, host, nl[0], pairwise, classes_lut, gmm, nullptr);
    for (int b = 1; b < n_images; ++b) {
        memcpy(host + (size_t)b * stage_row, host, stage_row);
        reinterpret_cast<int32_t *>(host + (size_t)b * stage_row + L.par.o_misc)[0] = nl[b];
    }
    HIP_TRY(hipMemcpyAsync(stage_dev, host, stage_row * n_images, hipMemcpyHostToDevice, st));
    if (launch_copy_rows(seg, slice, stage_dev, stage_row, L.par.bytes, n_images, st)) return -1;
    bh.base = seg;
    int32_t *misc = bh.misc();
    bh.K_dev = misc; bh.E_dev = misc + 1;

    uint32_t *bitmap = reinterpret_cast<uint32_t *>(seg + L.d_bitmap);
    long long *cacc = reinterpret_cast<long long *>(seg + L.d_cacc);
    bh.centres = reinterpret_cast<double *>(seg + L.d_cent); bh.edges = reinterpret_cast<int32_t *>(seg + L.d_edges);
    bh.arc_start = reinterpret_cast<int32_t *>(seg + L.d_as); bh.arc_to = reinterpret_cast<int32_t *>(seg + L.d_at);
    bh.arc_rev = reinterpret_cast<int32_t *>(seg + L.d_ar); bh.edge_arc = reinterpret_cast<int32_t *>(seg + L.d_ea);
    const int spg = ctx->begin(PG_GRAPH);
    if (launch_adjacency_bitmap(labels, H, W, K_cap, bitmap, cacc, bh.centres, seg + L.d_present, st, zb)) return -1;
    if (launch_graph_csr(bitmap, bh.K_dev, K_cap, words, reinterpret_cast<int32_t *>(seg + L.d_wp), reinterpret_cast<int32_t *>(seg + L.d_deg),
                         reinterpret_cast<int32_t *>(seg + L.d_dlow), bh.arc_start, reinterpret_cast<int32_t *>(seg + L.d_es), bh.E_dev, Ecap,
                         bh.edges, bh.arc_to, bh.arc_rev, bh.edge_arc, st, zb))
        return -1;
    ctx->end(spg);

    bh.features = reinterpret_cast<double *>(base + L.featK);
    bh.labels = labels; bh.n = n;
    bh.segm_out = reinterpret_cast<int32_t *>(base + L.segm_out); bh.soft_out = nullptr;
    bh.K_cap = K_cap; bh.Ecap = Ecap; bh.ndim = 2;
    bh.edge_cost = edge_cost; bh.use_graphcut = use_graphcut; bh.zb = zb;
    if (backhalf_enqueue(ctx, bh)) return -1;
    if (segm_out)
        for (int b = 0; b < n_images; ++b)
            if (segm_out[b])
                HIP_TRY(hipMemcpyAsync(segm_out[b], base + (size_t)b * slice + L.segm_out, n * 4, hipMemcpyDeviceToHost, st));
    if (launch_copy_rows(stage_dev, 16, misc, slice, 16, n_images, st)) return -1;
    std::vector<int32_t> hmisc((size_t)4 * n_images);
    HIP_TRY(hipMemcpyAsync(hmisc.data(), stage_dev, (size_t)16 * n_images, hipMemcpyDeviceToHost, st));
    HIP_TRY(hipStreamSynchronize(st));
    for (int b = 0; b < n_images; ++b) {
        const int rc = backhalf_status(hmisc.data() + (size_t)4 * b, use_graphcut);
        if (rc == -2) set_error("batch2d_run_color: image " + std::to_string(b) + " has more graph edges than a planar graph of its labels");
        if (rc) return -1;
    }
    return 0;
}

}
```

pyimsegm_amd/csrc/common.h:

```cpp
#pragma once
#include <hip/hip_runtime.h>
#include <stdint.h>
#include <string>
#include <type_traits>

#define IMSEGM_WAVE 64

namespace imsegm {

void set_error(const std::string &msg);
bool hip_ok(hipError_t e, const char *what, const char *file, int line);

#define HIP_TRY(expr)                                                                   \
    do {                                                                                \
        if (!::imsegm::hip_ok((expr), #expr, __FILE__, __LINE__)) return -1;            \
    } while (0)

struct Knobs {
    bool slic_graph, pre_3pass, separate_finalize, fuse_finalize, conn_general, gc_no_topo_regs,
        adjacency_table,
        cc_merge_full,
        terms_one_workgroup,
        label_general,
        sep_wide_tile;
    int brick_cap;
    int gc_lds_level;
    int gc_threads;
    int gc_grid_min_sites;
    int gc_grid_blocks;
    bool gc_one_workgroup;
    bool gc_grid_test_absent;
    int fused_bitmap_mb;
    std::string phase_dump;
};
const Knobs &knobs();
void reload_knobs();

constexpr int IMSEGM_MAX_DEVICES = 64;
__host__ __device__ static inline int cdiv(long a, long b) { return (int)((a + b - 1) / b); }

struct ZBatch {
    int nz = 1;
    size_t zs = 0;
};
template <typename T> __device__ __forceinline__ T *zshift(T *p, size_t zs)
{
    typedef typename std::conditional<std::is_const<T>::value, const char, char>::type byte_t;
    T *const shifted = reinterpret_cast<T *>(reinterpret_cast<byte_t *>(p) + (size_t)blockIdx.z * zs);
    return p ? shifted : nullptr;
}
template <typename T> __device__ __forceinline__ T *zshift_nn(T *p, size_t zs)
{
    typedef typename std::conditional<std::is_const<T>::value, const char, char>::type byte_t;
    return reinterpret_cast<T *>(reinterpret_cast<byte_t *>(p) + (size_t)blockIdx.z * zs);
}
#define ZSHIFT(p, zs) (p) = ::imsegm::zshift((p), (zs))
#define ZSHIFT_NN(p, zs) (p) = ::imsegm::zshift_nn((p), (zs))

__device__ __forceinline__ double det_cbrt(double x)
{
    long long i = __double_as_longlong(x);
    i = 0x553ef0ff289dd796LL - i / 3;
    double y = __longlong_as_double(i);
    const double third = 1.0 / 3.0;
#pragma unroll
    for (int it = 0; it < 5; ++it) {
        double y3 = y * y * y;
        double r = 1.0 - x * y3;
        y = y + y * (r * third);
    }
    double yy = y * y;
    double c = x * yy;
    double e = c * c * c - x;
    c = c - e * (yy * third);
    return c;
}

__device__ __forceinline__ double div_by_const_in_range(double x, double c, double rc)
{
    const double q = x * rc;
    const double r = fma(-q, c, x);
    return fma(r, rc, q);
}
#define DIV_CONST_IN_RANGE(x, C) ::imsegm::div_by_const_in_range((x), (C), 1.0 / (C))

__device__ __forceinline__ double det_pow24(double t)
{
    long long i = __double_as_longlong(t);
    i = 0x4cb8a8c154c985f0LL - i / 5;
    double y = __longlong_as_double(i);
#pragma unroll
    for (int it = 0; it < 5; ++it) {
        double y2 = y * y;
        double y5 = y2 * y2 * y;
        double r = 1.0 - t * y5;
        y = y + y * (r * 0.2);
    }
    double p = t * y;
    return p * p * p;
}

__device__ __forceinline__ void rgb2lab_px(double r, double g, double b, double &L, double &A, double &B)
{
    double lin[3] = { r, g, b };
#pragma unroll
    for (int c = 0; c < 3; ++c) {
        double v = lin[c];
        lin[c] = (v > 0.04045) ? det_pow24((v + 0.055) / 1.055) : v / 12.92;
    }
    double X = lin[0] * 0.412453 + lin[1] * 0.357580 + lin[2] * 0.180423;
    double Y = lin[0] * 0.212671 + lin[1] * 0.715160 + lin[2] * 0.072169;
    double Z = lin[0] * 0.019334 + lin[1] * 0.119193 + lin[2] * 0.950227;
    double f[3] = { X / 0.95047, Y / 1.0, Z / 1.08883 };
#pragma unroll
// ... 353 lines not shown
```

pyimsegm_amd/csrc/connectivity.hip:

```cpp
#include "slic.h"

#include <atomic>

namespace imsegm {

enum { ST_ACTIVE = 0, ST_FINAL = 1 };
enum { CNT_OVER = 0, CNT_SMALL = 1, CNT_CURSOR = 2, CNT_KEPT = 3, CNT_FALLBACK = 4, CNT_BIG = 5, CNT_LITTLE = 6,
       CNT_LROOT = 8, CNT_FLAG = 9, CNT_FB = 10, CNT_FB2 = 11 };

__device__ __forceinline__ int neighbour(int p, int D, int H, int W, int d)
{
    const int x = p % W, y = (p / W) % H, z = p / (W * H);
    switch (d) {
        case 0: return x + 1 < W ? p + 1 : -1;
        case 1: return x > 0 ? p - 1 : -1;
        case 2: return y + 1 < H ? p + W : -1;
        case 3: return y > 0 ? p - W : -1;
        case 4: return z + 1 < D ? p + W * H : -1;
        default: return z > 0 ? p - W * H : -1;
    }
}

__device__ __forceinline__ int uf_find(const int32_t *parent, int a)
{
// ... 1342 lines not shown
                        __asm__ volatile("" ::: "memory");
                        if (lane == 0) cs[cu] = 3;
                        if (u0 == 1) { if (lane == k) { c = cu + 1; cs[c] = (uint8_t)(4 + k); } ++k; }
                        if (u1 == 1) { if (lane == k) { c = cu - 1; cs[c] = (uint8_t)(4 + k); } ++k; }
                        if (u2 == 1) { if (lane == k) { c = cu + bw; cs[c] = (uint8_t)(4 + k); } ++k; }
                        if (u3 == 1) { if (lane == k) { c = cu - bw; cs[c] = (uint8_t)(4 + k); } ++k; }
                        f = k;
                        continue;
                    }
                    const bool act = lane < f;
                    if (!act) c = 2 * bw + 2;
                    const int v0 = cs[c + 1], v1 = cs[c - 1], v2 = cs[c + bw], v3 = cs[c - bw];
                    const int e0 = cs[c + 2], e1 = cs[c - 2], e2 = cs[c + 2 * bw], e3 = cs[c - 2 * bw];
                    const int epp = cs[c + 1 + bw], epm = cs[c + 1 - bw], emp = cs[c - 1 + bw], emm = cs[c - 1 - bw];
                    auto lower = [lane](int v) { return (unsigned int)(v - 4) < (unsigned int)lane; };
                    const bool w0 = act && v0 == 1 && !(lower(e0) || lower(epp) || lower(epm));
                    const bool w1 = act && v1 == 1 && !(lower(e1) || lower(emp) || lower(emm));
                    const bool w2 = act && v2 == 1 && !(lower(e2) || lower(epp) || lower(emp));
                    const bool w3 = act && v3 == 1 && !(lower(e3) || lower(epm) || lower(emm));
                    const unsigned long long con = __ballot(act && (v0 == 2 || v1 == 2 || v2 == 2 || v3 == 2));
                    if (con) {
                        const int cand = v3 == 2 ? c - bw : (v2 == 2 ? c + bw : (v1 == 2 ? c - 1 : c + 1));
                        adj_cell = __builtin_amdgcn_readlane(cand, 63 - __clzll((long long)con));
                    }
                    const unsigned long long b0 = __ballot(w0), b1 = __ballot(w1), b2 = __ballot(w2), b3 = __ballot(w3);
                    const int total = __popcll(b0) + __popcll(b1) + __popcll(b2) + __popcll(b3);
                    if (total > 64) {
                        reject = true;
                        break;
                    }
                    const int p0 = __popcll(b0 & lt) + __popcll(b1 & lt) + __popcll(b2 & lt) + __popcll(b3 & lt);
                    const int p1 = p0 + (w0 ? 1 : 0), p2 = p1 + (w1 ? 1 : 0), p3 = p2 + (w2 ? 1 : 0);
                    __asm__ volatile("" ::: "memory");
                    if (act) cs[c] = 3;
                    if (w0) { fr[p0] = c + 1; cs[c + 1] = (uint8_t)(4 + p0); }
                    if (w1) { fr[p1] = c - 1; cs[c - 1] = (uint8_t)(4 + p1); }
                    if (w2) { fr[p2] = c + bw; cs[c + bw] = (uint8_t)(4 + p2); }
                    if (w3) { fr[p3] = c - bw; cs[c - bw] = (uint8_t)(4 + p3); }
                    f = total;
                    __asm__ volatile("" ::: "memory");
                    c = fr[lane];
                }
            }
        }
        if (tid == 0) {
            if (reject) {
                adjptr[root] = -1;
                const int i = atomicAdd(&counters[rej_counter], 1);
                if (i < CONN_FB_CAP) {
                    rej_list[i] = root;
                    rej_bbox[6 * i + 0] = ry; rej_bbox[6 * i + 1] = y1;
                    rej_bbox[6 * i + 2] = x0; rej_bbox[6 * i + 3] = x1;
                    rej_bbox[6 * i + 4] = 0; rej_bbox[6 * i + 5] = 0;
                }
            } else {
                int adj = -1;
                if (adj_cell >= 0) {
                    const int cy = adj_cell / bw, cx = adj_cell - cy * bw;
                    adj = parent[parent[(size_t)(by0 + cy) * W + bx0 + cx]];
                }
                adjptr[root] = adj;
            }
        }
    }
}

__global__ void __launch_bounds__(256)
k_lroot_labels(const int32_t *__restrict__ lroots, const int32_t *__restrict__ ntile, int n_slots,
               const int32_t *__restrict__ counters, const int32_t *__restrict__ parent,
               const int32_t *__restrict__ csize, const int32_t *__restrict__ adjptr, int min_size, int32_t *newlabel, size_t zs)
{
    ZSHIFT(lroots, zs); ZSHIFT(ntile, zs); ZSHIFT(counters, zs); ZSHIFT(parent, zs); ZSHIFT(csize, zs); ZSHIFT(adjptr, zs); ZSHIFT(newlabel, zs);
    if (counters[CNT_FLAG]) return;
    const int i = blockIdx.x * 256 + threadIdx.x;
    if (i >= n_slots || (i & (CT_SLOTS - 1)) >= ntile[i / CT_SLOTS]) return;
    const int r = lroots[i];
    int g = parent[r];
    const bool kept_root = g == r && csize[g] >= min_size;
    if (kept_root) return;
    while (g >= 0 && csize[g] < min_size) g = adjptr[g];
    newlabel[r] = g >= 0 ? newlabel[g] : 0;
}

static int conn_fast_2d(const int32_t *labels_in, int H, int W, int min_size, int max_size, int start_label, const ConnWork &w,
                        int32_t *labels_out, int *n_kept, bool *ok, hipStream_t st, ZBatch zb = ZBatch(), int32_t *batch_stage = nullptr)
{
    if (zb.nz > 1 && !batch_stage) {
        set_error("connectivity: a batch needs a staging area for its counters");
        return -1;
    }
    const int n = H * W;
    const unsigned nz = (unsigned)zb.nz;
    const size_t zs = zb.zs;
    const dim3 tiles(cdiv(W, CT_W), cdiv(H, CT_H), nz);
    const int n_tiles = tiles.x * tiles.y, n_slots = n_tiles * CT_SLOTS;
    if (CONN_DENSE_INTS + (size_t)n_tiles * (3 * CT_SLOTS + 1) > w.dense_ints) {
        for (unsigned b = 0; b < nz; ++b) ok[b] = false;
        return 0;
    }
    const ConnDense d = conn_dense(w, n_tiles);
    int32_t *ymax_g = w.queue, *xmin_g = w.slotmap, *xmax_g = w.bbox;
    std::vector<int32_t> host_counters((size_t)16 * nz);
    if (launch_zero(w.counters, 16 * sizeof(int32_t), st, zb)) return -1;
    hipLaunchKernelGGL(k_ccl_tile, tiles, 256, 0, st, labels_in, H, W, w.parent, w.csize, ymax_g, xmin_g, xmax_g, d.lroots, d.lsize,
                       d.lbox, d.ntile, w.counters, zs);
    const long nborder = (long)((H - 1) / CT_H) * W + (long)((W - 1) / CT_W) * H;
    if (nborder > 0)
        hipLaunchKernelGGL(k_ccl_border, dim3(cdiv(nborder, 256), 1, nz), 256, 0, st, labels_in, H, W, w.parent, w.counters, zs);
    const dim3 lgrid(cdiv(n_slots, 256), 1, nz);
    hipLaunchKernelGGL(k_lroot_merge, lgrid, 256, 0, st, d.lroots, d.lsize, d.lbox, d.ntile, n_slots, w.counters, w.parent, w.csize, ymax_g,
                       xmin_g, xmax_g, W, zs);
    hipLaunchKernelGGL(k_root_classify, dim3(cdiv(n_slots, 1024), 1, nz), 1024, 0, st, d.lroots, d.ntile, n_slots, w.counters, w.parent, w.csize,
                       min_size, max_size, d.kept, w.list, zs);
    const int bfs_blocks = nz > 1 ? std::max(64, 2048 / (int)nz) : 2048;
    hipLaunchKernelGGL(k_small_bfs_reg, dim3(bfs_blocks + 1, 1, nz), 256, BR_CELLS + 256, st, w.list, w.counters + CNT_SMALL, n, w.counters, w.parent,
                       ymax_g, xmin_g, xmax_g, H, W, w.adjptr, d.fb_list, (int)CNT_FB, d.fb_bbox, BR_CELLS, 1, d.kept, start_label,
                       d.sorted, w.newlabel, zs);
    {
        static bool big_attr[IMSEGM_MAX_DEVICES];
        int dev = 0;
        HIP_TRY(hipGetDevice(&dev));
        if (dev < 0 || dev >= IMSEGM_MAX_DEVICES || !big_attr[dev]) {
            HIP_TRY(hipFuncSetAttribute((const void *)k_small_bfs_reg, hipFuncAttributeMaxDynamicSharedMemorySize, BR_CELLS_BIG + 256));
            if (dev >= 0 && dev < IMSEGM_MAX_DEVICES) big_attr[dev] = true;
        }
    }
    hipLaunchKernelGGL(k_small_bfs_reg, dim3(nz > 1 ? 32 : 128, 1, nz), 256, BR_CELLS_BIG + 256, st, d.fb_list, w.counters + CNT_FB, CONN_FB_CAP,
                       w.counters, w.parent, ymax_g, xmin_g, xmax_g, H, W, w.adjptr, d.fb2_list, (int)CNT_FB2, d.fb2_bbox, BR_CELLS_BIG, 0,
                       d.kept, start_label, d.sorted, w.newlabel, zs);
    hipLaunchKernelGGL((k_small_bfs_wave<8192, 2048, true>), dim3(nz > 1 ? 64 : 256, 1, nz), 64, 0, st, d.fb2_list, w.counters, w.counters + CNT_FB2,
                       w.parent, d.fb2_bbox, 1, H, W, (const int32_t *)nullptr, CONN_FB_CAP, w.adjptr, d.fb_reject, zs);
    hipLaunchKernelGGL(k_lroot_labels, lgrid, 256, 0, st, d.lroots, d.ntile, n_slots, w.counters, w.parent, w.csize, w.adjptr, min_size,
                       w.newlabel, zs);
    hipLaunchKernelGGL(k_write_labels, dim3(cdiv(cdiv(n, 4), 256), 1, nz), 256, 0, st, w.parent, w.newlabel, n, labels_out,
                       (const int32_t *)(w.counters + CNT_FLAG), zs);
    HIP_TRY(hipGetLastError());
    if (nz == 1) {
        HIP_TRY(hipMemcpyAsync(host_counters.data(), w.counters, 16 * sizeof(int32_t), hipMemcpyDeviceToHost, st));
    } else {
        int32_t *stage = batch_stage;
        if (launch_copy_rows(stage, 16 * sizeof(int32_t), w.counters, zs, 16 * sizeof(int32_t), (int)nz, st)) return -1;
        HIP_TRY(hipMemcpyAsync(host_counters.data(), stage, (size_t)nz * 16 * sizeof(int32_t), hipMemcpyDeviceToHost, st));
    }
    HIP_TRY(hipStreamSynchronize(st));
    for (unsigned b = 0; b < nz; ++b) {
        const int32_t *hc = host_counters.data() + (size_t)16 * b;
        ok[b] = hc[CNT_FLAG] == 0 && hc[CNT_OVER] == 0 && hc[CNT_FALLBACK] == 0 && hc[CNT_KEPT] <= CONN_KEPT_CAP &&
                hc[CNT_FB] <= CONN_FB_CAP && hc[CNT_FB2] <= CONN_FB_CAP;
        n_kept[b] = hc[CNT_KEPT];
    }
    return 0;
}

int launch_enforce_connectivity_batch(const int32_t *labels_in, int H, int W, long min_size_l, long max_size_l, int start_label, ConnWork w,
                                      int32_t *labels_out, int *n_labels_out, hipStream_t st, ZBatch zb, int32_t *stage_dev)
{
    const int min_size = (int)std::min<long>(min_size_l, 0x7fffffff);
    const int max_size = (int)std::min<long>(max_size_l, 0x7fffffff);
    std::vector<int> n_kept(zb.nz);
    std::vector<char> ok(zb.nz);
    static_assert(sizeof(bool) == sizeof(char), "ok flags");
    if (conn_fast_2d(labels_in, H, W, min_size, max_size, start_label, w, labels_out, n_kept.data(), reinterpret_cast<bool *>(ok.data()), st, zb,
                     stage_dev))
        return -1;
    for (int b = 0; b < zb.nz; ++b) n_labels_out[b] = ok[b] ? (n_kept[b] > 0 ? start_label + n_kept[b] : 1) : -1;
    return 0;
}

static std::atomic<long> g_conn_general_runs{0};
long conn_general_runs() { return g_conn_general_runs.load(); }

int launch_enforce_connectivity(const int32_t *labels_in, int D, int H, int W, long min_size_l, long max_size_l,
                                int start_label, ConnWork w, int32_t *labels_out, int *n_labels_out_host,
                                hipStream_t st)
{
    const int n = D * H * W;
    const int grid = cdiv(n, 256);
    const int min_size = (int)std::min<long>(min_size_l, 0x7fffffff);
    const int max_size = (int)std::min<long>(max_size_l, 0x7fffffff);
    uint8_t *state = w.visited + n;
    int32_t host_counters[16];

    if (D == 1 && !knobs().conn_general) {
        bool ok = false;
        int n_kept = 0;
        if (conn_fast_2d(labels_in, H, W, min_size, max_size, start_label, w, labels_out, &n_kept, &ok, st)) return -1;
        if (ok) {
            *n_labels_out_host = n_kept > 0 ? start_label + n_kept : 1;
            return 0;
        }
        g_conn_general_runs.fetch_add(1);
    }

    HIP_TRY(hipMemsetAsync(w.counters, 0, 16 * sizeof(int32_t), st));
    conn_ccl_round<true>(labels_in, D, H, W, max_size, w, state, st);
    if (conn_tail(w.csize, w.adjptr, D, H, W, min_size, start_label, w, labels_out, st, true, max_size)) return -1;
    HIP_TRY(hipMemcpyAsync(host_counters, w.counters, 8 * sizeof(int32_t), hipMemcpyDeviceToHost, st));
    HIP_TRY(hipStreamSynchronize(st));

    if (host_counters[CNT_OVER] > 0) {
        int32_t *csize_final = w.adjptr;
        HIP_TRY(hipMemsetAsync(state, ST_ACTIVE, n, st));
        for (int round = 0;; ++round) {
            HIP_TRY(hipMemsetAsync(w.visited, 0, n, st));
            HIP_TRY(hipMemsetAsync(w.counters, 0, 3 * sizeof(int32_t), st));
            conn_ccl_round<false>(labels_in, D, H, W, max_size, w, state, st);
            HIP_TRY(hipMemcpyAsync(host_counters, w.counters, 4 * sizeof(int32_t), hipMemcpyDeviceToHost, st));
            HIP_TRY(hipStreamSynchronize(st));
            int n_over = host_counters[CNT_OVER];
            if (n_over > 0) {
                if ((long)n_over * max_size > (long)n) {
                    set_error("enforce_connectivity: internal queue overflow");
                    return -1;
                }
                hipLaunchKernelGGL(k_oversize_bfs, cdiv(n_over, 64), 64, 0, st, w.list, n_over, w.parent, state, D, H, W,
                                   max_size, w.queue, w.visited, w.counters);
            }
            hipLaunchKernelGGL(k_oversize_commit, grid, 256, 0, st, w.parent, state, csize_final, w.csize, w.visited, n,
                               max_size);
            if (n_over == 0) break;
            if (round > n) {
                set_error("enforce_connectivity: did not converge");
                return -1;
            }
        }
        if (conn_tail(csize_final, w.csize, D, H, W, min_size, start_label, w, labels_out, st, false)) return -1;
        HIP_TRY(hipMemcpyAsync(host_counters, w.counters, 8 * sizeof(int32_t), hipMemcpyDeviceToHost, st));
        HIP_TRY(hipStreamSynchronize(st));
    }
    int n_kept = host_counters[CNT_KEPT];
    *n_labels_out_host = n_kept > 0 ? start_label + n_kept : 1;
    return 0;
}

}
```

pyimsegm_amd/csrc/graph.hip:

```cpp
#include "slic.h"

namespace imsegm {

constexpr int GR_ROWS = 4;
constexpr int GR_SLOTS = 64;

__global__ void __launch_bounds__(256)
k_adjacency_centres(const int32_t *__restrict__ labels, int H, int W, int K, int words, uint32_t *bitmap,
                    long long *__restrict__ cacc, size_t zs)
{
    ZSHIFT(labels, zs); ZSHIFT(bitmap, zs); ZSHIFT(cacc, zs);
    __shared__ int h_key[GR_SLOTS], h_n[GR_SLOTS], h_sy[GR_SLOTS], h_sx[GR_SLOTS];
    const int lane = threadIdx.x & 63, wave = threadIdx.x >> 6;
    if (threadIdx.x < GR_SLOTS) {
        h_key[threadIdx.x] = -1;
        h_n[threadIdx.x] = 0;
        h_sy[threadIdx.x] = 0;
        h_sx[threadIdx.x] = 0;
    }
    __syncthreads();
    const int x = blockIdx.x * 64 + lane;
    const int y0 = (blockIdx.y * 4 + wave) * GR_ROWS;
    const bool xin = x < W;
    int lab[GR_ROWS + 1], right[GR_ROWS];
// ... 131 lines not shown
{
    const int lane = threadIdx.x & 63;
    const int b = (blockIdx.x * blockDim.x + threadIdx.x) >> 6;
    if (b >= K) return;
    int c = 0;
    for (int i = lane; i < cap; i += 64) {
        const int a = table[(size_t)b * cap + i];
        c += a >= 0 && a < b;
    }
#pragma unroll
    for (int off = 32; off > 0; off >>= 1) c += __shfl_xor(c, off, 64);
    if (lane == 0) rowcount[b] = c;
}

__global__ void __launch_bounds__(256) k_table_emit(const int32_t *__restrict__ table, int K, int cap, const int32_t *__restrict__ offsets,
                                                    int32_t *edges, int capacity)
{
    const int lane = threadIdx.x & 63;
    const int b = (blockIdx.x * blockDim.x + threadIdx.x) >> 6;
    if (b >= K) return;
    const int32_t *row = table + (size_t)b * cap;
    const int o = offsets[b];
    for (int i = lane; i < cap; i += 64) {
        const int a = row[i];
        if (a < 0 || a >= b) continue;
        int rank = 0;
        for (int j = 0; j < cap; ++j) {
            const int other = row[j];
            rank += other >= 0 && other < a;
        }
        if (o + rank < capacity) {
            edges[2 * (o + rank) + 0] = a;
            edges[2 * (o + rank) + 1] = b;
        }
    }
}

int launch_edge_extract_table(const int32_t *table, int K, int cap, int32_t *rowcount, int32_t *edges_out, int edge_capacity,
                              int32_t *n_edges_dev, hipStream_t st)
{
    hipLaunchKernelGGL(k_table_rowcount, cdiv((long)K * 64, 256), 256, 0, st, table, K, cap, rowcount);
    hipLaunchKernelGGL(k_edge_scan, 1, 256, 0, st, rowcount, K, n_edges_dev);
    hipLaunchKernelGGL(k_table_emit, cdiv((long)K * 64, 256), 256, 0, st, table, K, cap, rowcount, edges_out, edge_capacity);
    HIP_TRY(hipGetLastError());
    return 0;
}

__global__ void __launch_bounds__(256) k_zero_words(uint32_t *p, size_t words, size_t zs)
{
    ZSHIFT(p, zs);
    for (size_t i = (size_t)blockIdx.x * 256 + threadIdx.x; i < words; i += (size_t)gridDim.x * 256) p[i] = 0u;
}

int launch_zero(void *ptr, size_t bytes, hipStream_t st, ZBatch zb)
{
    if (zb.nz <= 1) {
        HIP_TRY(hipMemsetAsync(ptr, 0, bytes, st));
        return 0;
    }
    const size_t words = (bytes + 3) / 4;
    const int gx = (int)std::min<size_t>(std::max<size_t>(cdiv((long)words, 256 * 8), 1), 256);
    hipLaunchKernelGGL(k_zero_words, dim3(gx, 1, zb.nz), 256, 0, st, static_cast<uint32_t *>(ptr), words, zb.zs);
    HIP_TRY(hipGetLastError());
    return 0;
}

__global__ void __launch_bounds__(256) k_copy_rows(uint32_t *dst, size_t dst_stride, const uint32_t *src, size_t src_stride, size_t words)
{
    dst = zshift(dst, dst_stride);
    src = zshift(src, src_stride);
    for (size_t i = (size_t)blockIdx.x * 256 + threadIdx.x; i < words; i += (size_t)gridDim.x * 256) dst[i] = src[i];
}

int launch_copy_rows(void *dst, size_t dst_stride, const void *src, size_t src_stride, size_t bytes, int rows, hipStream_t st)
{
    const size_t words = (bytes + 3) / 4;
    const int gx = (int)std::min<size_t>(std::max<size_t>(cdiv((long)words, 256 * 4), 1), 64);
    hipLaunchKernelGGL(k_copy_rows, dim3(gx, 1, rows), 256, 0, st, static_cast<uint32_t *>(dst), dst_stride, static_cast<const uint32_t *>(src),
                       src_stride, words);
    HIP_TRY(hipGetLastError());
    return 0;
}

int launch_adjacency_bitmap(const int32_t *labels, int H, int W, int K, uint32_t *bitmap, long long *cacc, double *centres_out,
                            uint8_t *present_out, hipStream_t st, ZBatch zb)
{
    int words = cdiv(K, 32);
    const size_t bm_bytes = (size_t)K * words * sizeof(uint32_t), gap = (size_t)((const char *)cacc - (const char *)bitmap);
    if ((const char *)cacc >= (const char *)bitmap + bm_bytes && gap <= bm_bytes + 64) {
        if (launch_zero(bitmap, gap + (size_t)K * 3 * sizeof(long long), st, zb)) return -1;
    } else {
        if (launch_zero(bitmap, bm_bytes, st, zb) || launch_zero(cacc, (size_t)K * 3 * sizeof(long long), st, zb)) return -1;
    }
    dim3 grid(cdiv(W, 64), cdiv(H, 4 * GR_ROWS), zb.nz);
    hipLaunchKernelGGL(k_adjacency_centres, grid, 256, 0, st, labels, H, W, K, words, bitmap, cacc, zb.zs);
    hipLaunchKernelGGL(k_centres_finalize, dim3(cdiv(K, 256), 1, zb.nz), 256, 0, st, cacc, K, centres_out, present_out, zb.zs);
    HIP_TRY(hipGetLastError());
    return 0;
}

int launch_adjacency_centres(const int32_t *labels, int H, int W, int K, uint32_t *bitmap, long long *cacc,
                             int32_t *edges_out, int edge_capacity, int32_t *n_edges_dev, double *centres_out,
                             uint8_t *present_out, int32_t *rowcount, hipStream_t st)
{
    if (launch_adjacency_bitmap(labels, H, W, K, bitmap, cacc, centres_out, present_out, st, ZBatch())) return -1;
    return launch_edge_extract(bitmap, K, cdiv(K, 32), rowcount, edges_out, edge_capacity, n_edges_dev, st);
}

int launch_edge_extract(const uint32_t *bitmap, int K, int words, int32_t *rowcount, int32_t *edges_out, int edge_capacity,
                        int32_t *n_edges_dev, hipStream_t st)
{
    hipLaunchKernelGGL(k_edge_rowcount, cdiv(K, 256), 256, 0, st, bitmap, K, words, rowcount);
    hipLaunchKernelGGL(k_edge_scan, 1, 256, 0, st, rowcount, K, n_edges_dev);
    hipLaunchKernelGGL(k_edge_emit, cdiv(K, 256), 256, 0, st, bitmap, K, words, rowcount, edges_out, edge_capacity);
    HIP_TRY(hipGetLastError());
    return 0;
}

__global__ void __launch_bounds__(256)
k_gather_i32(const int32_t *__restrict__ lut, const int32_t *__restrict__ idx, size_t n, int32_t *__restrict__ out, size_t zs)
{
    ZSHIFT(lut, zs); ZSHIFT(idx, zs); ZSHIFT(out, zs);
    const size_t i = ((size_t)blockIdx.x * blockDim.x + threadIdx.x) * 4;
    if (i >= n) return;
    const bool aligned = ((reinterpret_cast<uintptr_t>(idx) | reinterpret_cast<uintptr_t>(out)) & 15) == 0;
    if (aligned && i + 4 <= n) {
        const int4 q = *reinterpret_cast<const int4 *>(idx + i);
        *reinterpret_cast<int4 *>(out + i) = make_int4(lut[q.x], lut[q.y], lut[q.z], lut[q.w]);
    } else {
        for (size_t j = i; j < n && j < i + 4; ++j) out[j] = lut[idx[j]];
    }
}

__global__ void __launch_bounds__(256)
k_gather_f64(const double *__restrict__ lut, int C, const int32_t *__restrict__ idx, size_t total,
             double *__restrict__ out)
{
    size_t i = (size_t)blockIdx.x * blockDim.x + threadIdx.x;
    if (i >= total) return;
    size_t p = i / C;
    int c = (int)(i - p * C);
    out[i] = lut[(size_t)idx[p] * C + c];
}

int launch_gather_labels(const int32_t *lut, const int32_t *idx, size_t n, int32_t *out, hipStream_t st, ZBatch zb)
{
    hipLaunchKernelGGL(k_gather_i32, dim3(cdiv(cdiv((long)n, 4), 256), 1, zb.nz), 256, 0, st, lut, idx, n, out, zb.zs);
    HIP_TRY(hipGetLastError());
    return 0;
}

int launch_gather_proba(const double *lut, int C, const int32_t *idx, size_t n, double *out, hipStream_t st)
{
    size_t total = n * C;
    hipLaunchKernelGGL(k_gather_f64, cdiv((long)total, 256), 256, 0, st, lut, C, idx, total, out);
    HIP_TRY(hipGetLastError());
    return 0;
}

}
```

pyimsegm_amd/csrc/session.h:

```cpp
#pragma once
#include "../../include/imsegm_hip.h"
#include "slic.h"

#include <atomic>
#include <cstdio>
#include <cstdlib>
#include <cstring>
#include <vector>

namespace imsegm {

struct DevBuf {
    void *p = nullptr;
    size_t cap = 0;
    int ensure(size_t bytes)
    {
        if (bytes <= cap) return 0;
        if (p) HIP_TRY(hipFree(p));
        p = nullptr;
        cap = 0;
        size_t want = bytes + bytes / 8 + 256;
        HIP_TRY(hipMalloc(&p, want));
        cap = want;
        return 0;
// ... 63 lines not shown
            hipEvent_t e = pool.back();
            pool.pop_back();
            return e;
        }
        hipEvent_t e;
        (void)hipEventCreate(&e);
        return e;
    }
    int begin(int group)
    {
        if (!profile) return -1;
        Span s;
        s.group = group;
        s.a = get_event();
        s.b = get_event();
        (void)hipEventRecord(s.a, stream);
        spans.push_back(s);
        return (int)spans.size() - 1;
    }
    void end(int id)
    {
        if (id >= 0) (void)hipEventRecord(spans[id].b, stream);
    }
    void pair(int group, hipEvent_t *a, hipEvent_t *b)
    {
        Span s;
        s.group = group;
        s.a = get_event();
        s.b = get_event();
        spans.push_back(s);
        *a = s.a;
        *b = s.b;
    }
    ProfHook hook()
    {
        ProfHook hook;
        if (profile) {
            hook.user = this;
            hook.begin = [](void *u, int g) { return static_cast<imsegm_ctx *>(u)->begin(g); };
            hook.end = [](void *u, int id) { static_cast<imsegm_ctx *>(u)->end(id); };
            hook.pair = [](void *u, int g, hipEvent_t *a, hipEvent_t *b) { static_cast<imsegm_ctx *>(u)->pair(g, a, b); };
        }
        return hook;
    }
    void collect()
    {
        if (spans.empty()) return;
        (void)hipStreamSynchronize(stream);
        for (auto &s : spans) {
            float ms = 0;
            if (hipEventElapsedTime(&ms, s.a, s.b) == hipSuccess) {
                acc_ms[s.group] += ms;
                acc_n[s.group] += 1;
            }
            pool.push_back(s.a);
            pool.push_back(s.b);
        }
        spans.clear();
    }
};

struct GraphPlan {
    int K = 0, Ecap = 0, cap = 0, words = 0;
    bool table = false;
    size_t o_head = 0, o_edges = 0, o_as = 0, o_at = 0, o_ar = 0, o_ea = 0, o_deg = 0, o_dlow = 0, o_es = 0, o_cent = 0, o_present = 0,
           o_store = 0, o_cacc = 0, o_wp = 0, bytes = 0;
};

struct imsegm_image2d {
    imsegm_ctx *ctx = nullptr;
    int D = 1, H = 0, W = 0;
    size_t n = 0;
    int dtype = -1;
    int n_labels = 0;
    bool have_labels = false;
    bool labels_connected = false;
    bool tex_ready = false;
    bool is_volume = false;
    double vol_off = 0.0, vol_scale = 1.0;
    DevBuf img, labA, labB, nearest, labels, conn_i32, conn_u8, small, cent, tiles, feat, graph, gather_lut, gather_out_i, gather_out_f,
        tex_planes, tex_resp, tex_small, tex_aux, vol_cent, annot, hist, featK, seg, gseg, narrow;
    GraphPlan gplan;
    bool graph_ready = false;
    int *slic_fail_host = nullptr;
    int feat_mask = 0, feat_F = 0;
    int place_F = 0, place_col = 0;
    hipGraphExec_t slic_exec = nullptr;
    std::vector<unsigned char> slic_key;
};

inline int wrong_kind(const imsegm_image2d *im, bool want_volume)
{
    if (im && im->is_volume != want_volume) {
        set_error(want_volume ? "this call needs a volume session" : "this call needs a 2-D colour image session");
        return 1;
    }
    return 0;
}

extern std::atomic<bool> g_runtime_started;

inline int bind(imsegm_ctx *ctx)
{
    if (!ctx) {
        set_error("null context");
        return -1;
    }
    HIP_TRY(hipSetDevice(ctx->device));
    return 0;
}

inline int ensure_small(imsegm_image2d *im)
{
    if (im->small.cap >= 4096) return 0;
    if (im->small.ensure(4096)) return -1;
    HIP_TRY(hipMemsetAsync(im->small.p, 0, 4096, im->ctx->stream));
    return 0;
}

struct GridAxis {
    long start, step;
    bool all;
};
inline void regular_grid3(const long shape[3], long n_points, GridAxis out[3])
{
    int order[3] = { 0, 1, 2 };
    std::stable_sort(order, order + 3, [&](int a, int b) { return shape[a] < shape[b]; });
    double sorted_dims[3] = { (double)shape[order[0]], (double)shape[order[1]], (double)shape[order[2]] };
    double space = sorted_dims[0] * sorted_dims[1] * sorted_dims[2];
    if (space <= (double)n_points) {
        for (int i = 0; i < 3; ++i) out[i] = { 0, 1, true };
        return;
    }
    double steps[3];
    for (int i = 0; i < 3; ++i) steps[i] = pow(space / (double)n_points, 1.0 / 3);
    bool any_small = false;
    for (int i = 0; i < 3; ++i) any_small |= sorted_dims[i] < steps[i];
    if (any_small) {
        for (int dim = 0; dim < 3; ++dim) {
            steps[dim] = sorted_dims[dim];
            double sp = 1.0;
            for (int j = dim + 1; j < 3; ++j) sp *= sorted_dims[j];
            if (dim < 2) {
                double s = pow(sp / (double)n_points, 1.0 / (3 - dim - 1));
                for (int j = dim + 1; j < 3; ++j) steps[j] = s;
            }
            bool ok = true;
            for (int j = 0; j < 3; ++j) ok &= sorted_dims[j] >= steps[j];
            if (ok) break;
        }
    }
    for (int i = 0; i < 3; ++i) {
        long start = (long)floor(steps[i] / 2.0);
        long step = (long)nearbyint(steps[i]);
        out[order[i]] = { start, step, false };
    }
}

inline int fill_taps(Taps &t, const double *w, int r)
{
    t.r = -1;
    for (int i = 0; i < 17; ++i) t.w[i] = 0;
    if (r < 0 || !w) return 0;
    if (r > 16) {
        set_error("gaussian kernel radius > 16 is not supported");
        return -1;
// ... 76 lines not shown
```

pyimsegm_amd/csrc/slic.h:

```cpp
#pragma once
#include "common.h"
#include <algorithm>
#include <cfloat>
#include <cmath>

namespace imsegm {

enum { DT_U8 = 0, DT_F64 = 1, DT_F32 = 2 };

struct Taps {
    int r;
    double w[17];
};

constexpr int SLIC_TILE_X = 64, SLIC_TILE_Y = 32, SLIC_MAXC = 64;
struct Cand {
    double cy, cx, cL, ca, cb;
    int4 win;
    int k;
    float ry, rx;
    float fL, fa, fb;
    double mdc;
};

// ... 43 lines not shown

int launch_minmax(const void *src, int dtype, size_t n, unsigned long long *keys, double *out2, hipStream_t st, double *also_zero = nullptr,
                  ZBatch zb = ZBatch());
int launch_preprocess_color2d(const void *img, int dtype, int H, int W, int normalize, const double *minmax_dev,
                              const Taps &tz, const Taps &ty, const Taps &tx, double ratio, double *bufA,
                              double *bufB, double *premax_dev, hipStream_t st, bool premax_zeroed = false, ZBatch zb = ZBatch());
int launch_absmax_f64(const double *src, size_t n, double *out_dev, hipStream_t st);
struct ProfHook {
    void *user = nullptr;
    int (*begin)(void *, int) = nullptr;
    void (*end)(void *, int) = nullptr;
    void (*pair)(void *, int, hipEvent_t *, hipEvent_t *) = nullptr;
};
int slic_prepare_device();
void slic_sweep_counters(long *persistent_runs, long *fallback_runs);
void slic_sweep_note_fallback();
int launch_slic_iterations(SlicState s, const double *lab, const double *init_yx_dev, int32_t *labels, int max_iter,
                           int max_cand, const ProfHook &prof, hipStream_t st, bool *fused_update = nullptr, ZBatch zb = ZBatch());

struct VolState {
    int D, H, W, K;
    int step_z, step_y, step_x;
    double spatial_weight;
    double sz, sy, sx;
    double *cen;
    int *win;
    long long *acc;
    const double *premax;
    int grid_0[3], grid_d[3], grid_n[3];
    int nbz, nby, nbx;
    int brick_cap;
    int *brick_count;
    int *brick_list;
    int *brick_entries;
    float *cen32;
    int *bbox;
};
constexpr int VOL_BX = 64, VOL_BY = 16, VOL_BZ = 16;
int launch_vol_preprocess(const void *src, int dtype, double off, double scale, int D, int H, int W, const Taps &tz, const Taps &ty,
                          const Taps &tx, double ratio, double *bufA, double *bufB, hipStream_t st);
int launch_vol_slic(VolState s, const double *vol, int32_t *labels, int max_iter, hipStream_t st);
int launch_vol_preprocess_f32(const float *src, int D, int H, int W, const Taps &tz, const Taps &ty, const Taps &tx, double ratio,
                              double *bufA, double *bufB, hipStream_t st);
int launch_vol_slic_f32(VolState s, const float *vol, int32_t *labels, int max_iter, hipStream_t st, const ProfHook *prof = nullptr);
int launch_label_cc(int32_t *labels_inout, int D, int H, int W, int32_t *parent, int32_t *newlabel, int32_t *blocksum,
                    int32_t *total_dev, hipStream_t st);
int launch_vol_adjacency(const int32_t *labels, int D, int H, int W, int K, int words, uint32_t *bitmap, long long *cacc,
                         double *centres, uint8_t *present, hipStream_t st);
int launch_vol_adjacency_table(const int32_t *labels, int D, int H, int W, int K, int32_t *table, int cap, int *overflow, long long *cacc,
                               double *centres, uint8_t *present, hipStream_t st);
int launch_edge_extract_table(const int32_t *table, int K, int cap, int32_t *rowcount, int32_t *edges_out, int edge_capacity,
                              int32_t *n_edges_dev, hipStream_t st);
int launch_edge_extract(const uint32_t *bitmap, int K, int words, int32_t *rowcount, int32_t *edges_out, int edge_capacity,
                        int32_t *n_edges_dev, hipStream_t st);

struct ConnWork {
    int32_t *parent;
    int32_t *csize;
    int32_t *newlabel;
    int32_t *adjptr;
    int32_t *queue;
    uint8_t *visited;
    int32_t *blocksum;
    int32_t *list;
    int32_t *counters;
    int32_t *slotmap;
    int32_t *bbox;
    int32_t *dense;
    size_t dense_ints;
};
constexpr size_t CONN_DENSE_INTS = 2 * 65536 + 16 * 4096;
constexpr int CONN_TILE_PIXELS = 64 * 32, CONN_TILE_SLOTS = 256;
static inline size_t conn_i32_bytes(size_t n, size_t H = 0, size_t W = 0)
{
    const size_t n_tiles = ((W + 63) / 64) * ((H + 31) / 32);
    return n * 4 * 8 + ((n / 4096) + 64) * 4 + 256 + (CONN_DENSE_INTS + n_tiles * (3 * CONN_TILE_SLOTS + 1)) * 4;
}
int launch_label_connected(int32_t *labels_inout, size_t n, int n_labels, int32_t *first, uint32_t *bitmap, int32_t *blocksum,
                           int32_t *counters, int32_t *total_dev, hipStream_t st);
long conn_general_runs();
long gc_grid_fallbacks();
int launch_enforce_connectivity(const int32_t *labels_in, int D, int H, int W, long min_size, long max_size,
                                int start_label, ConnWork w, int32_t *labels_out, int *n_labels_out_host,
                                hipStream_t st);
int launch_enforce_connectivity_batch(const int32_t *labels_in, int H, int W, long min_size, long max_size, int start_label, ConnWork w,
                                      int32_t *labels_out, int *n_labels_out, hipStream_t st, ZBatch zb, int32_t *stage_dev);

int launch_label_hist(const int32_t *labels, const int32_t *annot, size_t n, int K, int nb, unsigned long long *hist,
                      hipStream_t st);
int launch_color_stats(const void *img, int dtype, const int32_t *labels, int H, int W, int K, double maxabs,
                       int want_var, long long *acc, double *mean_out, double *energy_out, double *var_out,
                       float *mean32_scratch, hipStream_t st, int planar = 0, int prescale = 0, double mul = 1.0,
                       double div = 1.0, long plane_stride = -1, const double *ssq_dev = nullptr, ZBatch zb = ZBatch(),
                       const double *minmax_dev = nullptr);

struct SepJob {
    double *resp;
    const double *taps;
    int groups, rank, merge;
};
constexpr int SEP_MAX_JOBS = 5;
struct SepJobs {
    int n;
    SepJob job[SEP_MAX_JOBS];
};
int launch_battery_dense(const double *planes, int H, int W, const double *wgt_dev, int nk, int radius, double clip, double *resp,
                         hipStream_t st, int P, int parity);
size_t sep_sumsq_scratch(int H, int W, int P, int radius, int jobs);
int launch_battery_sep(const double *planes, int H, int W, int radius, double clip, const SepJobs &jobs, hipStream_t st, int P,
                       double *ssq_scratch, double *const *ssq_out);
int launch_response_sumsq(const double *resp, size_t count, double *partial, double *sumsq_dev, hipStream_t st);
int launch_texture_prepare(const void *img, int dtype, int H, int W, const double *taps_dev, int radius,
                           const double *mix_dev, double *planes, double *tmpA, double *tmpB, hipStream_t st, double *fullpad);
int launch_texture_prepare_volume(const void *vol, int dtype, int P, int H, int W, const double *taps_dev, int radius, double *planes,
                                  double *tmpA, double *tmpB, hipStream_t st, double *fullpad);
int launch_filter_battery(const double *planes, int H, int W, const double *wgt_dev, int nk, int radius, double clip,
                          double *resp, double *partial, double *sumsq_dev, hipStream_t st, int P = 3, const double *sep_dev = nullptr,
                          int sep_groups = 0, int sep_rank = 0, int parity = 0);

int launch_adjacency_centres(const int32_t *labels, int H, int W, int K, uint32_t *bitmap, long long *cacc,
                             int32_t *edges_out, int edge_capacity, int32_t *n_edges_dev, double *centres_out,
                             uint8_t *present_out, int32_t *rowcount, hipStream_t st);
int launch_adjacency_bitmap(const int32_t *labels, int H, int W, int K, uint32_t *bitmap, long long *cacc, double *centres_out,
                            uint8_t *present_out, hipStream_t st, ZBatch zb = ZBatch());
int launch_gather_labels(const int32_t *lut, const int32_t *idx, size_t n, int32_t *out, hipStream_t st, ZBatch zb = ZBatch());
int launch_zero(void *ptr, size_t bytes, hipStream_t st, ZBatch zb);
int launch_copy_rows(void *dst, size_t dst_stride, const void *src, size_t src_stride, size_t bytes, int rows, hipStream_t st);
int launch_gather_proba(const double *lut, int C, const int32_t *idx, size_t n, double *out, hipStream_t st);

int launch_boundary_minmax(const int32_t *labels, int W, const int rects[16], int32_t *out2_dev, hipStream_t st);
int launch_boundary_hist(const int32_t *labels, int W, const int rects[16], unsigned long long *hist_dev, int nb, hipStream_t st);
int launch_swap_labels(int32_t *labels, size_t n, int a, int b, hipStream_t st);
int launch_narrow_labels_u8(const int32_t *src, uint8_t *dst, size_t n, hipStream_t st);
int launch_narrow_soft_f32(const double *src, float *dst, size_t n, hipStream_t st);
int launch_count_nonfinite(const void *src, int dtype, size_t n, unsigned int *count_dev, hipStream_t st);

struct MedianNorm { int on; double mul, div; };
int launch_gradient_image(const void *src, void *dst, int dtype, int S, int H, int W, int C, hipStream_t st,
                          MedianNorm norm = MedianNorm{ 0, 1.0, 1.0 });
size_t median_scratch_bytes(size_t n, int K);
int launch_segment_median(const void *img, int dtype, int C, size_t pix_stride, size_t chan_stride, size_t n, const int32_t *labels,
                          int K, MedianNorm norm, void *scratch, size_t scratch_bytes, double *out, hipStream_t st);

int launch_label_hist2d(const int16_t *segm, int H, int W, const int32_t *windows, int P, const int16_t *selem, int SH, int SW,
                        int nb_labels, unsigned int *hist, hipStream_t st);
int launch_ray_features_binary2d(const int8_t *seg, int H, int W, const int32_t *positions, int P, const float *grad, int A, int edge,
                                 float *out, hipStream_t st);

struct GcProblem {
    int K, C, E;
    const int32_t *E_dev = nullptr;
    const int32_t *K_dev = nullptr;
    const int32_t *edges;
    const int32_t *w;
    const int32_t *unary;
    const int32_t *smooth;
    int metric = 0;
};
static inline int smooth_is_metric(const int32_t *s, int C)
{
    for (int a = 0; a < C; ++a) {
        if (s[a * C + a] != 0) return 0;
        for (int b = 0; b < C; ++b)
            if (s[a * C + b] < 0 || s[a * C + b] != s[b * C + a]) return 0;
    }
    for (int a = 0; a < C; ++a)
        for (int b = 0; b < C; ++b)
            for (int c = 0; c < C; ++c)
                if ((long long)s[a * C + b] > (long long)s[a * C + c] + (long long)s[c * C + b]) return 0;
    return 1;
}
int launch_alpha_expansion(GcProblem p, const int32_t *arc_start, const int32_t *arc_to, const int32_t *arc_rev,
                           const int32_t *edge_arc, int n_iter, int32_t *labels_dev, long long *energy_dev,
                           int32_t *status_dev, void *work, hipStream_t st, ZBatch zb = ZBatch());
size_t alpha_expansion_work_bytes(int K, int E);

struct TermsArgs {
    const int *Kp;
    int K_cap;
    const int *Ep;
    int edge_capacity;
    int F, C;
    const double *features;
    int gmm;
    const double *scaler_mean, *scaler_scale;
    const double *prec_chol;
    const double *mu_proj;
    const double *log_det;
    const double *log_w;
    double const_term;
    double *proba;
    int edge_type;
    int spatial_norm;
    double edge_cost;
    const int32_t *edges;
    const double *centres;
    int ndim;
    double *edge_dist, *edge_len;
    double *unary;
    double *weights;
    const double *pairwise;
    double pairwise_max;
    int32_t *unary_i, *weights_i;
    int smooth_max;
    int32_t *status;
    double *scalars;
    double *fstd;
// ... 17 lines not shown
```

pyimsegm_amd/csrc/stats.hip:

```cpp
#include "slic.h"

namespace imsegm {

constexpr int ST_ROWS = 16;
constexpr int ST_SLOTS = 64;

__device__ __forceinline__ void fix_split_sh(double v, double scale, long long &hi, long long &lo)
{
    double t = v * scale;
    long long h = (long long)t;
    double r = t - (double)h;
    hi = h;
    lo = (long long)(r * 4294967296.0);
}

template <typename T> __device__ __forceinline__ float load_f32(const T *p, size_t i) { return (float)p[i]; }

struct StatParams {
    int H, W, K;
    double scale_v, scale_e;
    int planar;
    size_t plane_stride;
    size_t n_pixels;
    int u8_int;
    int prescale;
    double mul, div;
    const double *ssq_dev;
    size_t zs;
    const double *minmax;
};

__host__ __device__ inline double pow2_scale(double n_pixels, double maxabs)
{
    int e_n, e_m;
    frexp(n_pixels, &e_n);
    frexp(maxabs > 0.0 ? maxabs : 1.0, &e_m);
    int sh = 62 - e_n - e_m;
    if (sh > 44 - e_m) sh = 44 - e_m;
    return ldexp(1.0, sh);
}

__host__ __device__ inline void stat_scales(double n_pixels, double maxabs, double &scale_v, double &scale_e)
{
    if (!(maxabs < 1e300)) maxabs = 1e300;
    scale_v = pow2_scale(n_pixels, maxabs);
    scale_e = pow2_scale(n_pixels, 4.0 * maxabs * maxabs);
}

__device__ __forceinline__ void image_scales(const StatParams &sp, double &scale_v, double &scale_e)
{
    scale_v = sp.scale_v;
    scale_e = sp.scale_e;
    if (sp.minmax) {
        stat_scales((double)sp.n_pixels, fmax(fabs(sp.minmax[0]), fabs(sp.minmax[1])), scale_v, scale_e);
    } else if (sp.prescale == 2) {
        const double norm = sqrt(*sp.ssq_dev);
        const bool dead = !(norm > 0.0) || norm > DBL_MAX;
        stat_scales((double)sp.n_pixels, dead ? 0.0 : fabs(log(1.0 + norm) / 0.03), scale_v, scale_e);
    }
}

template <typename T, int NC = 3, int PASS = 1> struct StatRows { static constexpr int value = (sizeof(T) == 8 || (NC == 1 && PASS == 1)) ? ST_ROWS / 2 : ST_ROWS; };

template <typename T, int PASS, bool U8INT, int NC = 3>
__global__ void __launch_bounds__(256, 4)
k_color_stats(const T *__restrict__ img, const int32_t *__restrict__ labels, StatParams sp,
              const float *__restrict__ mean32, long long *__restrict__ acc)
{
    constexpr int RW = StatRows<T, NC, PASS>::value;
    ZSHIFT(img, sp.zs); ZSHIFT(labels, sp.zs); ZSHIFT(mean32, sp.zs); ZSHIFT(acc, sp.zs); ZSHIFT(sp.ssq_dev, sp.zs);
    ZSHIFT(sp.minmax, sp.zs);
    double scale_v, scale_e;
    image_scales(sp, scale_v, scale_e);
    constexpr int NQ = (PASS == 1) ? 13 : 6;
    __shared__ int keys[ST_SLOTS];
    __shared__ long long lacc[ST_SLOTS][13];
    const int tid = threadIdx.x, lane = tid & 63, wave = tid >> 6;
    if (tid < ST_SLOTS) {
        keys[tid] = -1;
        for (int j = 0; j < NQ; ++j) lacc[tid][j] = 0;
    }
    __syncthreads();
    const int x = blockIdx.x * 64 + lane;
    const int y0 = (blockIdx.y * 4 + wave) * RW;
    static_assert(!U8INT || (PASS == 1 && sizeof(T) == 1 && NC == 3), "integer block sums: uint8 colour image, first pass");
    int lab[RW];
    float v[RW][NC];
    double mul = sp.mul, div = sp.div;
    bool dead = false;
    if (sp.prescale == 2) {
        const double norm = sqrt(*sp.ssq_dev);
        dead = !(norm > 0.0) || norm > DBL_MAX;
        mul = log(1.0 + norm) / 0.03;
        div = norm;
    }
#pragma unroll
    for (int r = 0; r < RW; ++r) {
        const int y = y0 + r;
        const bool ok = (y < sp.H) && (x < sp.W);
        const size_t p = ok ? (size_t)y * sp.W + x : 0;
        lab[r] = ok ? labels[p] : 0x7fffffff;
        if (NC == 3 && sizeof(T) == 1 && !sp.planar && !sp.prescale && p + 1 < sp.n_pixels) {
            uint32_t w;
            __builtin_memcpy(&w, reinterpret_cast<const uint8_t *>(img) + 3 * p, 4);
            v[r][0] = (float)(w & 0xffu);
            v[r][NC > 1 ? 1 : 0] = (float)((w >> 8) & 0xffu);
            v[r][NC > 1 ? 2 : 0] = (float)((w >> 16) & 0xffu);
            continue;
        }
#pragma unroll
        for (int c = 0; c < NC; ++c) {
            const size_t idx = NC == 1 ? p : (sp.planar ? (size_t)c * sp.plane_stride + p : 3 * p + c);
            v[r][c] = sp.prescale ? (dead ? 0.f : (float)(((double)img[idx] * mul) / div)) : load_f32(img, idx);
        }
    }
    double limb[(NC == 1 && PASS == 1) ? RW : 1][(NC == 1 && PASS == 1) ? 4 : 1];
    if constexpr (NC == 1 && PASS == 1) {
#pragma unroll
        for (int r = 0; r < RW; ++r) {
            const float val = v[r][0];
            const float term = __fmul_rn(val, val);
            const double t = (double)term * scale_e, h = trunc(t);
            const double tv = (double)val * scale_v, hv = trunc(tv);
            limb[r][0] = hv;
            limb[r][1] = trunc((tv - hv) * 4294967296.0);
            limb[r][2] = h;
            limb[r][3] = trunc((t - h) * 4294967296.0);
        }
    }
    while (true) {
        int mine = 0x7fffffff;
#pragma unroll
        for (int r = 0; r < RW; ++r) mine = min(mine, lab[r]);
        if (!__any(mine != 0x7fffffff)) break;
        const int k = row16_min_i32(mine);
        if constexpr (U8INT) {
            int qi[8] = { 0, 0, 0, 0, 0, 0, 0, 0 };
#pragma unroll
            for (int r = 0; r < RW; ++r) {
                if (lab[r] != k || k == 0x7fffffff) continue;
                lab[r] = 0x7fffffff;
                qi[0] += 1;
#pragma unroll
                for (int c = 0; c < 3; ++c) {
                    const int val = (int)v[r][c];
                    qi[1 + c] += val;
                    qi[4 + c] += val * val;
                }
            }
            const int toti = row16_reduce8_i32(qi, lane);
            const int j = ((lane >> 3) & 1) * 4 + ((lane >> 2) & 1) * 2 + ((lane >> 1) & 1);
            int slot = -1;
            if ((lane & 15) == 0 && k != 0x7fffffff) {
                int sidx = k & (ST_SLOTS - 1), probes = 0;
                while (probes < ST_SLOTS) {
                    int old = atomicCAS(&keys[sidx], -1, k);
                    if (old == -1 || old == k) break;
                    sidx = (sidx + 1) & (ST_SLOTS - 1);
                    ++probes;
                }
                slot = probes < ST_SLOTS ? sidx : -1;
            }
            slot = __shfl(slot, lane & 48, 64);
            if ((lane & 1) == 0 && j < 7 && toti != 0 && k != 0x7fffffff) {
                const int col = j == 0 ? 0 : (j < 4 ? 1 + 2 * (j - 1) : 7 + 2 * (j - 4));
                const long long tot = j == 0 ? (long long)toti
                                             : (long long)toti * (long long)(j < 4 ? scale_v : scale_e);
                if (slot >= 0) atomic_add_i64(&lacc[slot][col], tot);
                else atomic_add_i64(acc + (size_t)k * 13 + col, tot);
            }
            continue;
        }
        int slot = -1;
        if ((lane & 15) == 0 && k != 0x7fffffff) {
            int sidx = k & (ST_SLOTS - 1), probes = 0;
            while (probes < ST_SLOTS) {
                int old = atomicCAS(&keys[sidx], -1, k);
                if (old == -1 || old == k) break;
                sidx = (sidx + 1) & (ST_SLOTS - 1);
                ++probes;
            }
            slot = probes < ST_SLOTS ? sidx : -1;
        }
        slot = __shfl(slot, lane & 48, 64);
// ... 7 lines not shown
            for (int r = 0; r < RW; ++r) {
                const bool on = lab[r] == k && live;
                lab[r] = on ? 0x7fffffff : lab[r];
                if (PASS == 1) {
                    q[0] += on ? limb[r][0] : 0.0;
                    q[1] += on ? limb[r][1] : 0.0;
                    q[2] += on ? limb[r][2] : 0.0;
                    q[3] += on ? limb[r][3] : 0.0;
                    q[6] += on ? 1.0 : 0.0;
                } else if (on) {
                    const float d = __fsub_rn(v[r][0], m32);
                    float term = __fmul_rn(d, d);
                    asm volatile("" : "+v"(term));
                    const double t = (double)term * scale_e, h = trunc(t);
                    q[0] += h;
                    q[1] += trunc((t - h) * 4294967296.0);
                }
            }
            const long long tot = (long long)row16_reduce8_f64(reinterpret_cast<const double (&)[8]>(q), lane);
            const int j = ((lane >> 3) & 1) * 4 + ((lane >> 2) & 1) * 2 + ((lane >> 1) & 1);
            const bool owner = (lane & 1) == 0 && (PASS == 1 ? (j < 4 || j == 6) : j < 2);
            if (owner && tot != 0 && live) {
                const int col = PASS == 1 ? (j == 6 ? 0 : (j < 2 ? 1 + j : 5 + j)) : j;
                if (slot >= 0)
                    atomic_add_i64(&lacc[slot][col], tot);
                else
                    atomic_add_i64(acc + (size_t)k * 13 + ((PASS == 1) ? col : 7 + col), tot);
            }
            continue;
        }
        if constexpr (NC == 3) {
        auto one_round = [&](auto round_tag) {
            constexpr int round = decltype(round_tag)::value;
            double q[8];
#pragma unroll
            for (int j = 0; j < 8; ++j) q[j] = 0;
#pragma unroll
            for (int r = 0; r < RW; ++r) {
                if (lab[r] != k || k == 0x7fffffff) continue;
                if (PASS == 1 && round == 0) q[6] += 1.0;
#pragma unroll
                for (int c = 0; c < 3; ++c) {
                    float term;
                    if (PASS == 1) {
                        const float val = v[r][c];
                        term = round == 0 ? val : __fmul_rn(val, val);
                    } else {
                        const float d = __fsub_rn(v[r][c], mean32[3 * k + c]);
                        term = __fmul_rn(d, d);
                    }
                    asm volatile("" : "+v"(term));
                    const double t = (double)term * ((PASS == 1 && round == 0) ? scale_v : scale_e), h = trunc(t);
                    q[2 * c] += h;
                    q[2 * c + 1] += trunc((t - h) * 4294967296.0);
                }
            }
            const long long tot = (long long)row16_reduce8_f64(reinterpret_cast<const double (&)[8]>(q), lane);
            const int j = ((lane >> 3) & 1) * 4 + ((lane >> 2) & 1) * 2 + ((lane >> 1) & 1);
            const bool owner = (lane & 1) == 0 && (j < 6 || (PASS == 1 && round == 0 && j == 6));
            if (owner && tot != 0 && k != 0x7fffffff) {
                const int col = PASS == 1 ? (round == 0 ? (j == 6 ? 0 : 1 + j) : 7 + j) : j;
                if (slot >= 0)
                    atomic_add_i64(&lacc[slot][col], tot);
                else
                    atomic_add_i64(acc + (size_t)k * 13 + ((PASS == 1) ? col : 7 + col), tot);
            }
        };
        one_round(std::integral_constant<int, 0>());
        if (PASS == 1) one_round(std::integral_constant<int, 1>());
#pragma unroll
        for (int r = 0; r < RW; ++r)
            if (lab[r] == k) lab[r] = 0x7fffffff;
        }
    }
    __syncthreads();
    for (int i = tid; i < ST_SLOTS * NQ; i += 256) {
        int slot = i / NQ, j = i - slot * NQ;
        int k = keys[slot];
        if (k < 0) continue;
        long long val = lacc[slot][j];
        if (val == 0) continue;
        int col = (PASS == 1) ? j : 7 + j;
        atomic_add_i64(acc + (size_t)k * 13 + col, val);
    }
}

__global__ void k_stats_clear(long long *acc, int K, int from, int to, size_t zs)
{
    ZSHIFT(acc, zs);
    int i = blockIdx.x * blockDim.x + threadIdx.x;
    if (i >= K) return;
    for (int j = from; j < to; ++j) acc[(size_t)i * 13 + j] = 0;
}

__global__ void k_stats_finalize1(long long *__restrict__ acc, StatParams sp, double *mean_out, double *energy_out,
                                  float *mean32)
{
    ZSHIFT(acc, sp.zs); ZSHIFT(mean_out, sp.zs); ZSHIFT(energy_out, sp.zs); ZSHIFT(mean32, sp.zs);
    ZSHIFT(sp.ssq_dev, sp.zs); ZSHIFT(sp.minmax, sp.zs);
    int k = blockIdx.x * blockDim.x + threadIdx.x;
    if (k >= sp.K) return;
    double scale_v, scale_e;
    image_scales(sp, scale_v, scale_e);
    long long *a = acc + (size_t)k * 13;
    long long n = a[0];
    const bool gray = sp.planar && sp.plane_stride == 0 && !sp.prescale;
    for (int c = 0; c < 3; ++c) {
        const int s = gray ? 0 : c;
        double sv = (i64_to_double(a[1 + 2 * s]) + i64_to_double(a[2 + 2 * s]) * (1.0 / 4294967296.0)) / scale_v;
        double se = (i64_to_double(a[7 + 2 * s]) + i64_to_double(a[8 + 2 * s]) * (1.0 / 4294967296.0)) / scale_e;
        double m = n > 0 ? sv / (double)n : 0.0;
        double e = n > 0 ? se / (double)n : 0.0;
        if (mean_out) mean_out[3 * k + c] = m;
        if (energy_out) energy_out[3 * k + c] = e;
        mean32[3 * k + c] = (float)m;
    }
    for (int j = 7; j < 13; ++j) a[j] = 0;
}

__global__ void k_stats_finalize2(const long long *__restrict__ acc, StatParams sp, double *var_out)
{
    ZSHIFT(acc, sp.zs); ZSHIFT(var_out, sp.zs); ZSHIFT(sp.ssq_dev, sp.zs); ZSHIFT(sp.minmax, sp.zs);
    int k = blockIdx.x * blockDim.x + threadIdx.x;
    if (k >= sp.K) return;
    double scale_v, scale_e;
    image_scales(sp, scale_v, scale_e);
    const long long *a = acc + (size_t)k * 13;
    long long n = a[0];
    const bool gray = sp.planar && sp.plane_stride == 0 && !sp.prescale;
    for (int c = 0; c < 3; ++c) {
        const int j = gray ? 0 : c;
        double s = (i64_to_double(a[7 + 2 * j]) + i64_to_double(a[8 + 2 * j]) * (1.0 / 4294967296.0)) / scale_e;
        var_out[3 * k + c] = n > 0 ? s / (double)n : 0.0;
    }
}

template <typename T>
static void launch_pass(int pass, const T *img, const int32_t *labels, StatParams sp, const float *mean32,
                        long long *acc, hipStream_t st, int nz)
{
    dim3 grid(cdiv(sp.W, 64), cdiv(sp.H, 4 * StatRows<T>::value), nz);
    if (sp.planar && sp.plane_stride == 0 && !sp.prescale) {
        grid.y = cdiv(sp.H, 4 * (pass == 1 ? StatRows<T, 1, 1>::value : StatRows<T, 1, 2>::value));
        if (pass == 1) hipLaunchKernelGGL((k_color_stats<T, 1, false, 1>), grid, 256, 0, st, img, labels, sp, mean32, acc);
        else hipLaunchKernelGGL((k_color_stats<T, 2, false, 1>), grid, 256, 0, st, img, labels, sp, mean32, acc);
        return;
    }
    if (pass == 1 && sizeof(T) == 1 && sp.u8_int)
        hipLaunchKernelGGL((k_color_stats<T, 1, sizeof(T) == 1>), grid, 256, 0, st, img, labels, sp, mean32, acc);
    else if (pass == 1)
        hipLaunchKernelGGL((k_color_stats<T, 1, false>), grid, 256, 0, st, img, labels, sp, mean32, acc);
    else
        hipLaunchKernelGGL((k_color_stats<T, 2, false>), grid, 256, 0, st, img, labels, sp, mean32, acc);
}

int launch_color_stats(const void *img, int dtype, const int32_t *labels, int H, int W, int K, double maxabs,
                       int want_var, long long *acc, double *mean_out, double *energy_out, double *var_out,
                       float *mean32_scratch, hipStream_t st, int planar, int prescale, double mul, double div,
                       long plane_stride, const double *ssq_dev, ZBatch zb, const double *minmax_dev)
{
    StatParams sp;
    sp.zs = zb.zs;
    const unsigned nz = (unsigned)zb.nz;
    sp.H = H; sp.W = W; sp.K = K;
    sp.n_pixels = (size_t)H * W;
    sp.planar = planar; sp.prescale = prescale; sp.mul = mul; sp.div = div; sp.ssq_dev = ssq_dev;
    sp.plane_stride = plane_stride >= 0 ? (size_t)plane_stride : (size_t)H * W;
    sp.minmax = minmax_dev;
    stat_scales((double)H * W, maxabs, sp.scale_v, sp.scale_e);
    sp.u8_int = (dtype == DT_U8 && !prescale && sp.scale_v >= 1.0 && sp.scale_e >= 1.0) ? 1 : 0;
    const dim3 kgrid(cdiv(K, 256), 1, nz);
    hipLaunchKernelGGL(k_stats_clear, kgrid, 256, 0, st, acc, K, 0, 13, zb.zs);
    if (dtype == DT_U8) launch_pass<uint8_t>(1, (const uint8_t *)img, labels, sp, mean32_scratch, acc, st, zb.nz);
    else if (dtype == DT_F32) launch_pass<float>(1, (const float *)img, labels, sp, mean32_scratch, acc, st, zb.nz);
    else launch_pass<double>(1, (const double *)img, labels, sp, mean32_scratch, acc, st, zb.nz);
    hipLaunchKernelGGL(k_stats_finalize1, kgrid, 256, 0, st, acc, sp, mean_out, energy_out, mean32_scratch);
    if (want_var) {
        if (dtype == DT_U8) launch_pass<uint8_t>(2, (const uint8_t *)img, labels, sp, mean32_scratch, acc, st, zb.nz);
        else if (dtype == DT_F32) launch_pass<float>(2, (const float *)img, labels, sp, mean32_scratch, acc, st, zb.nz);
        else launch_pass<double>(2, (const double *)img, labels, sp, mean32_scratch, acc, st, zb.nz);
        hipLaunchKernelGGL(k_stats_finalize2, kgrid, 256, 0, st, acc, sp, var_out);
    }
    HIP_TRY(hipGetLastError());
    return 0;
}

constexpr int LH_RUN = 8;

__global__ void __launch_bounds__(256)
k_label_hist(const int32_t *__restrict__ labels, const int32_t *__restrict__ annot, size_t n, int K, int nb,
             unsigned long long *__restrict__ hist)
{
    const size_t base = ((size_t)blockIdx.x * 256 + threadIdx.x) * LH_RUN;
    if (base >= n) return;
    int lb[LH_RUN], an[LH_RUN];
    if (base + LH_RUN <= n) {
        const int4 l0 = *reinterpret_cast<const int4 *>(labels + base), l1 = *reinterpret_cast<const int4 *>(labels + base + 4);
        const int4 a0 = *reinterpret_cast<const int4 *>(annot + base), a1 = *reinterpret_cast<const int4 *>(annot + base + 4);
        lb[0] = l0.x; lb[1] = l0.y; lb[2] = l0.z; lb[3] = l0.w; lb[4] = l1.x; lb[5] = l1.y; lb[6] = l1.z; lb[7] = l1.w;
        an[0] = a0.x; an[1] = a0.y; an[2] = a0.z; an[3] = a0.w; an[4] = a1.x; an[5] = a1.y; an[6] = a1.z; an[7] = a1.w;
    } else {
#pragma unroll
        for (int i = 0; i < LH_RUN; ++i) {
            const bool ok = base + i < n;
            lb[i] = ok ? labels[base + i] : -1;
            an[i] = ok ? annot[base + i] : -1;
        }
    }
    long long cur = -1;
    unsigned run = 0;
#pragma unroll
    for (int i = 0; i < LH_RUN; ++i) {
        const bool ok = lb[i] >= 0 && lb[i] < K && an[i] >= 0 && an[i] < nb;
        const long long bin = ok ? (long long)lb[i] * nb + an[i] : -1;
        if (bin != cur) {
            if (cur >= 0) atomicAdd(hist + cur, (unsigned long long)run);
            cur = bin;
            run = 0;
        }
        run++;
    }
    if (cur >= 0) atomicAdd(hist + cur, (unsigned long long)run);
}

int launch_label_hist(const int32_t *labels, const int32_t *annot, size_t n, int K, int nb, unsigned long long *hist,
                      hipStream_t st)
{
    HIP_TRY(hipMemsetAsync(hist, 0, (size_t)K * nb * sizeof(unsigned long long), st));
    if (n) hipLaunchKernelGGL(k_label_hist, cdiv((long)((n + LH_RUN - 1) / LH_RUN), 256), 256, 0, st, labels, annot, n, K, nb, hist);
    HIP_TRY(hipGetLastError());
    return 0;
}

}
```

Measured before the change: 5793 Mpixels/s.

## Fuse label write-back with colour-stats pass 1 and adjacency/centre sums

Adds a fused kernel that resolves connectivity labels (parent→newlabel), writes the final label map, and in the same pass accumulates the first colour-stats moments, the adjacency bitmap and superpixel centre sums. Later stats and graph stages skip the work already done. This removes separate full-image passes over labels and pixels. In exchange it adds LDS hash tables, extra state flags and a size limit on tiles, and keeps a staged fallback behind an environment variable.

```diff
diff --git a/include/imsegm_hip.h b/include/imsegm_hip.h
--- a/include/imsegm_hip.h
+++ b/include/imsegm_hip.h
@@ -60,6 +60,7 @@
 IMSEGM_API int imsegm_image2d_get_labels(imsegm_image2d *img, int64_t *labels_out);
 IMSEGM_API int imsegm_image2d_set_labels(imsegm_image2d *img, const int32_t *labels, int n_labels);
 IMSEGM_API long imsegm_debug_conn_general_runs(void);
+IMSEGM_API int imsegm_debug_label_consumers(imsegm_image2d *img, const int32_t *labels, int n_labels);
 IMSEGM_API int imsegm_debug_slic_sweep_runs(long *persistent_runs_out, long *fallback_runs_out);
 IMSEGM_API long imsegm_debug_gc_grid_fallbacks(void);
 IMSEGM_API int imsegm_image2d_enforce_connectivity(imsegm_image2d *img, const int32_t *labels, long min_size, long max_size,
diff --git a/pyimsegm_amd/_hip.py b/pyimsegm_amd/_hip.py
--- a/pyimsegm_amd/_hip.py
+++ b/pyimsegm_amd/_hip.py
@@ -102,6 +102,7 @@
     'imsegm_image2d_set_labels': (C.c_int, [_vp, _vp, C.c_int]),
     'imsegm_image2d_enforce_connectivity': (C.c_int, [_vp, _vp, C.c_long, C.c_long, C.c_int, _vp]),
     'imsegm_debug_conn_general_runs': (C.c_long, []),
+    'imsegm_debug_label_consumers': (C.c_int, [_vp, _vp, C.c_int]),
     'imsegm_debug_slic_sweep_runs': (C.c_int, [_vp, _vp]),
     'imsegm_debug_gc_grid_fallbacks': (C.c_long, []),
     'imsegm_assume_bg_on_boundary': (C.c_int, [_vp, _vp, C.c_int, C.c_int, _vp, C.c_int, _ip]),
@@ -666,6 +667,16 @@
         self.n_labels = int(n_labels)
         return self
 
+    def debug_label_consumers(self, labels, n_labels=None):
+        labels = np.ascontiguousarray(labels, dtype=np.int32)
+        if labels.shape != self.shape:
+            raise ValueError('label map %r does not match image %r' % (labels.shape, self.shape))
+        if n_labels is None:
+            n_labels = int(labels.max()) + 1
+        _check(load_library().imsegm_debug_label_consumers(self._h, _ptr(labels), int(n_labels)))
+        self.n_labels = int(n_labels)
+        return self
+
     def label_hist(self, annot, nb_annot=None):
         annot = np.ascontiguousarray(annot, dtype=np.int32)
         if annot.shape != self.shape:
diff --git a/pyimsegm_amd/csrc/api.hip b/pyimsegm_amd/csrc/api.hip
--- a/pyimsegm_amd/csrc/api.hip
+++ b/pyimsegm_amd/csrc/api.hip
@@ -45,6 +45,10 @@
     k.gc_grid_blocks = num("IMSEGM_GC_GRID_BLOCKS", 0);
     k.gc_one_workgroup = flag("IMSEGM_GC_ONE_WORKGROUP");
     k.gc_grid_test_absent = flag("IMSEGM_GC_GRID_TEST_ABSENT");
+    {
+        const char *lc = getenv("IMSEGM_LABEL_CONSUMERS");
+        k.label_consumers_staged = lc && !strcmp(lc, "staged");
+    }
     k.fused_bitmap_mb = num("IMSEGM_FUSED_BITMAP_MB", 0);
     const char *d = getenv("IMSEGM_PHASE_DUMP");
     k.phase_dump = d ? d : "";
@@ -295,6 +299,7 @@
     HIP_TRY(hipMemcpyAsync(im->img.p, host_pixels, bytes, hipMemcpyHostToDevice, im->ctx->stream));
     if (!is_pinned(host_pixels)) HIP_TRY(hipStreamSynchronize(im->ctx->stream));
     im->dtype = dtype;
+    im->lc_pass1 = false;
     im->feat_mask = 0;
     im->place_F = 0;
     return 0;
diff --git a/pyimsegm_amd/csrc/api_fused.hip b/pyimsegm_amd/csrc/api_fused.hip
--- a/pyimsegm_amd/csrc/api_fused.hip
+++ b/pyimsegm_amd/csrc/api_fused.hip
@@ -135,7 +135,11 @@
     hipStream_t st = ctx->stream;
     const int K = im->n_labels;
     double maxabs = 255.0;
-    if (im->dtype != IMSEGM_U8) {
+    const bool pass1_done = im->lc_pass1 && im->lc_K == K && !im->is_volume;
+    im->lc_pass1 = false;
+    if (pass1_done) {
+        maxabs = im->lc_maxabs;
+    } else if (im->dtype != IMSEGM_U8) {
         if (ensure_small(im)) return -1;
         unsigned long long *keys = im->small.as<unsigned long long>();
         double *minmax = reinterpret_cast<double *>(keys + 2);
@@ -155,7 +159,7 @@
                                 ss.acc, ss.mean, ss.energy, ss.var, ss.mean32, st, 1, 0, 1.0, 1.0, 0);
     else
         rc = launch_color_stats(im->img.p, im->dtype, im->labels.as<int32_t>(), im->H, im->W, K, maxabs, (feature_mask & 2) != 0, ss.acc,
-                                ss.mean, ss.energy, ss.var, ss.mean32, st, 0, 0, 1.0, 1.0, -1);
+                                ss.mean, ss.energy, ss.var, ss.mean32, st, 0, 0, 1.0, 1.0, -1, nullptr, ZBatch(), nullptr, pass1_done);
     if (rc) return -1;
     const int F = color_feature_columns(feature_mask);
     int table_F = F, col0 = 0;
@@ -264,9 +268,12 @@
             return -1;
     } else {
         uint32_t *bitmap = reinterpret_cast<uint32_t *>(store);
+        const bool sums_done = im->lc_adj && im->lc_K == g.K && im->lc_Ecap == g.Ecap && !im->is_volume;
+        im->lc_adj = false;
         if (im->is_volume) {
             if (launch_vol_adjacency(im->labels.as<int32_t>(), im->D, im->H, im->W, g.K, g.words, bitmap, cacc, centres, gb + g.o_present, st)) return -1;
-        } else if (launch_adjacency_bitmap(im->labels.as<int32_t>(), im->H, im->W, g.K, bitmap, cacc, centres, gb + g.o_present, st)) {
+        } else if (launch_adjacency_bitmap(im->labels.as<int32_t>(), im->H, im->W, g.K, bitmap, cacc, centres, gb + g.o_present, st, ZBatch(),
+                                           sums_done)) {
             return -1;
         }
         if (launch_graph_csr(bitmap, K_dev, g.K, g.words, reinterpret_cast<int32_t *>(gb + g.o_wp), reinterpret_cast<int32_t *>(gb + g.o_deg),
@@ -450,21 +457,112 @@
 }
 
 
+static int label_consumers_enqueue(imsegm_image2d *im)
+{
+    imsegm_ctx *ctx = im->ctx;
+    hipStream_t st = ctx->stream;
+    const int K = im->n_labels;
+    im->labels_deferred = false;
+    const ConnWork w = make_conn_work(im);
+    const GraphPlan g = graph_plan(im, K, 0);
+    if (g.table || graph_store_fits(im, g)) return launch_conn_write_labels(w, (int)im->n, im->labels.as<int32_t>(), st);
+    double maxabs = 255.0;
+    if (im->dtype != IMSEGM_U8) {
+        if (ensure_small(im)) return -1;
+        unsigned long long *keys = im->small.as<unsigned long long>();
+        double *minmax = reinterpret_cast<double *>(keys + 2);
+        if (launch_minmax(im->img.p, im->dtype, im->n * 3, keys, minmax, st)) return -1;
+        double mm[2];
+        HIP_TRY(hipMemcpyAsync(mm, minmax, 16, hipMemcpyDeviceToHost, st));
+        HIP_TRY(hipStreamSynchronize(st));
+        maxabs = std::max(fabs(mm[0]), fabs(mm[1]));
+        if (!(maxabs < 1e300)) maxabs = 1e300;
+    }
+    if (im->feat.ensure(stats_scratch_bytes(K)) || im->gseg.ensure(g.bytes)) return -1;
+    const StatsScratch ss = stats_scratch_at(im->feat.p, K);
+    unsigned char *gb = im->gseg.as<unsigned char>();
+    const int sp = ctx->begin(PG_STATS);
+    if (launch_label_consumers(im->img.p, im->dtype, w.parent, w.newlabel, im->labels.as<int32_t>(), im->H, im->W, K, maxabs, ss.acc,
+                               reinterpret_cast<uint32_t *>(gb + g.o_store), reinterpret_cast<long long *>(gb + g.o_cacc), st))
+        return -1;
+    ctx->end(sp);
+    im->lc_pass1 = im->lc_adj = true;
+    im->lc_K = K; im->lc_Ecap = g.Ecap; im->lc_maxabs = maxabs;
+    return 0;
+}
+
+int imsegm_debug_label_consumers(imsegm_image2d *im, const int32_t *labels, int n_labels)
+{
+    if (!im || bind(im->ctx)) return -1;
+    if (im->is_volume || im->dtype < 0 || !labels || n_labels < 1 || !label_consumers_take(im->H, im->W)) {
+        set_error("debug_label_consumers: an uploaded 2-D colour image, a label map and n_labels >= 1 are required");
+        return -1;
+    }
+    const size_t n = im->n;
+    std::vector<int32_t> own(n);
+    for (size_t i = 0; i < n; ++i) {
+        if (labels[i] < 0 || labels[i] >= n_labels) {
+            set_error("debug_label_consumers: label out of range");
+            return -1;
+        }
+        own[i] = (int32_t)i;
+    }
+    hipStream_t st = im->ctx->stream;
+    if (im->labels.ensure(n * 4) || im->conn_i32.ensure(conn_i32_bytes(n, im->H, im->W)) || im->conn_u8.ensure(2 * n + 64)) return -1;
+    const ConnWork w = make_conn_work(im);
+    HIP_TRY(hipMemcpyAsync(w.parent, own.data(), n * 4, hipMemcpyHostToDevice, st));
+    HIP_TRY(hipMemcpyAsync(w.newlabel, labels, n * 4, hipMemcpyHostToDevice, st));
+    HIP_TRY(hipStreamSynchronize(st));
+    im->n_labels = n_labels;
+    im->have_labels = true;
+    im->labels_connected = false;
+    im->graph_ready = false;
+    im->lc_pass1 = im->lc_adj = false;
+    if (label_consumers_enqueue(im)) {
+        im->have_labels = false;
+        return -1;
+    }
+    return 0;
+}
+
+static int run_color_impl(imsegm_image2d *im, const void *host_pixels, int dtype, int minmax_normalize, int n_segments,
+                          double compactness, const double *taps, int radius, int max_iter, int start_label, int slic_zero,
+                          int feature_mask, const imsegm_gmm *gmm, int n_classes, const double *pairwise, int edge_type,
+                          double edge_cost, int use_graphcut, const int32_t *classes_lut, int32_t *segm_out, double *soft_out,
+                          int *n_labels_out)
+{
+    if (imsegm_image2d_upload(im, host_pixels, dtype)) return -1;
+    int n_labels = 0;
+    im->defer_labels = !im->is_volume && !knobs().label_consumers_staged && label_consumers_take(im->H, im->W);
+    const int rc = imsegm_image2d_slic(im, minmax_normalize, n_segments, compactness, taps, radius, taps, radius, taps, radius, max_iter, 1,
+                                       0.5, 3.0, start_label, 0, slic_zero, &n_labels);
+    im->defer_labels = false;
+    if (rc) return -1;
+    if (n_labels_out) *n_labels_out = n_labels;
+    if (im->labels_deferred && label_consumers_enqueue(im)) {
+        im->have_labels = false;
+        return -1;
+    }
+    if (imsegm_image2d_features_color(im, feature_mask, nullptr)) return -1;
+    return imsegm_image2d_segment(im, gmm, nullptr, n_classes, pairwise, edge_type, edge_cost, use_graphcut, classes_lut, segm_out,
+                                  soft_out, nullptr, nullptr, nullptr);
+}
+
 int imsegm_image2d_run_color(imsegm_image2d *im, const void *host_pixels, int dtype, int minmax_normalize, int n_segments,
                              double compactness, const double *taps, int radius, int max_iter, int start_label, int slic_zero,
                              int feature_mask, const imsegm_gmm *gmm, int n_classes, const double *pairwise, int edge_type,
                              double edge_cost, int use_graphcut, const int32_t *classes_lut, int32_t *segm_out, double *soft_out,
                              int *n_labels_out)
 {
-    if (imsegm_image2d_upload(im, host_pixels, dtype)) return -1;
-    int n_labels = 0;
-    if (imsegm_image2d_slic(im, minmax_normalize, n_segments, compactness, taps, radius, taps, radius, taps, radius, max_iter, 1, 0.5,
-                            3.0, start_label, 0, slic_zero, &n_labels))
-        return -1;
-    if (n_labels_out) *n_labels_out = n_labels;
-    if (imsegm_image2d_features_color(im, feature_mask, nullptr)) return -1;
-    return imsegm_image2d_segment(im, gmm, nullptr, n_classes, pairwise, edge_type, edge_cost, use_graphcut, classes_lut, segm_out,
-                                  soft_out, nullptr, nullptr, nullptr);
-}
-
-}
+    if (!im) {
+        set_error("null image session");
+        return -1;
+    }
+    const int rc = run_color_impl(im, host_pixels, dtype, minmax_normalize, n_segments, compactness, taps, radius, max_iter, start_label,
+                                  slic_zero, feature_mask, gmm, n_classes, pairwise, edge_type, edge_cost, use_graphcut, classes_lut, segm_out,
+                                  soft_out, n_labels_out);
+    im->labels_deferred = im->lc_pass1 = im->lc_adj = false;
+    return rc;
+}
+
+}
diff --git a/pyimsegm_amd/csrc/api_image2d.hip b/pyimsegm_amd/csrc/api_image2d.hip
--- a/pyimsegm_amd/csrc/api_image2d.hip
+++ b/pyimsegm_amd/csrc/api_image2d.hip
@@ -216,6 +216,7 @@
         }
     }
     int n_labels = K + start_label;
+    bool write_deferred = false;
     for (int attempt = 0; attempt < 2; ++attempt) {
         if (attempt == 1) {
             slic_sweep_note_fallback();
@@ -232,7 +233,7 @@
             ConnWork w = make_conn_work(im);
             int spc = ctx->begin(PG_CONN);
             if (launch_enforce_connectivity(im->nearest.as<int32_t>(), 1, H, W, min_size, max_size, start_label, w,
-                                            im->labels.as<int32_t>(), &n_labels, st))
+                                            im->labels.as<int32_t>(), &n_labels, st, im->defer_labels ? &write_deferred : nullptr))
                 return -1;
             ctx->end(spc);
         } else {
@@ -253,6 +254,8 @@
     im->have_labels = true;
     im->labels_connected = false;
     im->graph_ready = false;
+    im->lc_pass1 = im->lc_adj = false;
+    im->labels_deferred = write_deferred;
     if (n_labels_out) *n_labels_out = n_labels;
     return 0;
 }
@@ -285,6 +288,7 @@
     im->have_labels = true;
     im->labels_connected = false;
     im->graph_ready = false;
+    im->lc_pass1 = im->lc_adj = false;
     return 0;
 }
 
@@ -314,6 +318,7 @@
     im->have_labels = true;
     im->labels_connected = false;
     im->graph_ready = false;
+    im->lc_pass1 = im->lc_adj = false;
     if (n_labels_out) *n_labels_out = n_labels;
     return 0;
 }
diff --git a/pyimsegm_amd/csrc/batch.hip b/pyimsegm_amd/csrc/batch.hip
--- a/pyimsegm_amd/csrc/batch.hip
+++ b/pyimsegm_amd/csrc/batch.hip
@@ -242,6 +242,7 @@
 
     ConnWork w = conn_work_from(reinterpret_cast<int32_t *>(base + L.conn_i32), L.conn_i32_bytes, base + L.conn_u8, n);
     std::vector<int> &nl = bt->n_labels;
+    const bool defer_labels = !knobs().label_consumers_staged && label_consumers_take(H, W);
     for (int attempt = 0; attempt < 2; ++attempt) {
         if (attempt == 1) {
             slic_sweep_note_fallback();
@@ -251,12 +252,15 @@
         }
         const int spc = ctx->begin(PG_CONN);
         if (launch_enforce_connectivity_batch(nearest, H, W, min_size, max_size, start_label, w, labels, nl.data(), st, zb,
-                                              reinterpret_cast<int32_t *>(stage_dev)))
+                                              reinterpret_cast<int32_t *>(stage_dev), defer_labels))
             return -1;
         ctx->end(spc);
         if (!fused_update || *bt->fail_host == 0) break;
         fused_update = false;
     }
+    bool consumers_fused = defer_labels;
+    for (int b = 0; b < n_images; ++b) consumers_fused = consumers_fused && nl[b] >= 0;
+    if (defer_labels && !consumers_fused && launch_conn_write_labels(w, (int)n, labels, st, zb)) return -1;
     for (int b = 0; b < n_images; ++b) {
         if (nl[b] >= 0) continue;
         unsigned char *sb = base + (size_t)b * slice;
@@ -288,8 +292,13 @@
             mm_dev = minmax;
         }
         const int sps = ctx->begin(PG_STATS);
+        if (consumers_fused &&
+            launch_label_consumers(base + L.img, dtype, w.parent, w.newlabel, labels, H, W, K_cap, 255.0, ss.acc,
+                                   reinterpret_cast<uint32_t *>(base + L.seg + L.d_bitmap), reinterpret_cast<long long *>(base + L.seg + L.d_cacc),
+                                   st, zb, mm_dev))
+            return -1;
         if (launch_color_stats(base + L.img, dtype, labels, H, W, K_cap, 255.0, (feature_mask & 2) != 0, ss.acc, ss.mean, ss.energy, ss.var,
-                               ss.mean32, st, 0, 0, 1.0, 1.0, -1, nullptr, zb, mm_dev))
+                               ss.mean32, st, 0, 0, 1.0, 1.0, -1, nullptr, zb, mm_dev, consumers_fused))
             return -1;
         if (launch_features_assemble(ss.mean, ss.energy, ss.var, K_cap, feature_mask, reinterpret_cast<double *>(base + L.featK), st, 0, 0, zb))
             return -1;
@@ -318,7 +327,7 @@
     bh.arc_start = reinterpret_cast<int32_t *>(seg + L.d_as); bh.arc_to = reinterpret_cast<int32_t *>(seg + L.d_at);
     bh.arc_rev = reinterpret_cast<int32_t *>(seg + L.d_ar); bh.edge_arc = reinterpret_cast<int32_t *>(seg + L.d_ea);
     const int spg = ctx->begin(PG_GRAPH);
-    if (launch_adjacency_bitmap(labels, H, W, K_cap, bitmap, cacc, bh.centres, seg + L.d_present, st, zb)) return -1;
+    if (launch_adjacency_bitmap(labels, H, W, K_cap, bitmap, cacc, bh.centres, seg + L.d_present, st, zb, consumers_fused)) return -1;
     if (launch_graph_csr(bitmap, bh.K_dev, K_cap, words, reinterpret_cast<int32_t *>(seg + L.d_wp), reinterpret_cast<int32_t *>(seg + L.d_deg),
                          reinterpret_cast<int32_t *>(seg + L.d_dlow), bh.arc_start, reinterpret_cast<int32_t *>(seg + L.d_es), bh.E_dev, Ecap,
                          bh.edges, bh.arc_to, bh.arc_rev, bh.edge_arc, st, zb))
diff --git a/pyimsegm_amd/csrc/common.h b/pyimsegm_amd/csrc/common.h
--- a/pyimsegm_amd/csrc/common.h
+++ b/pyimsegm_amd/csrc/common.h
@@ -30,6 +30,7 @@
     int gc_grid_blocks;
     bool gc_one_workgroup;
     bool gc_grid_test_absent;
+    bool label_consumers_staged;
     int fused_bitmap_mb;
     std::string phase_dump;
 };
diff --git a/pyimsegm_amd/csrc/connectivity.hip b/pyimsegm_amd/csrc/connectivity.hip
--- a/pyimsegm_amd/csrc/connectivity.hip
+++ b/pyimsegm_amd/csrc/connectivity.hip
@@ -1448,8 +1448,17 @@
     newlabel[r] = g >= 0 ? newlabel[g] : 0;
 }
 
+int launch_conn_write_labels(const ConnWork &w, int n, int32_t *labels_out, hipStream_t st, ZBatch zb)
+{
+    hipLaunchKernelGGL(k_write_labels, dim3(cdiv(cdiv(n, 4), 256), 1, (unsigned)zb.nz), 256, 0, st, w.parent, w.newlabel, n, labels_out,
+                       (const int32_t *)(w.counters + CNT_FLAG), zb.zs);
+    HIP_TRY(hipGetLastError());
+    return 0;
+}
+
 static int conn_fast_2d(const int32_t *labels_in, int H, int W, int min_size, int max_size, int start_label, const ConnWork &w,
-                        int32_t *labels_out, int *n_kept, bool *ok, hipStream_t st, ZBatch zb = ZBatch(), int32_t *batch_stage = nullptr)
+                        int32_t *labels_out, int *n_kept, bool *ok, hipStream_t st, ZBatch zb = ZBatch(), int32_t *batch_stage = nullptr,
+                        bool defer_write = false)
 {
     if (zb.nz > 1 && !batch_stage) {
         set_error("connectivity: a batch needs a staging area for its counters");
@@ -1498,8 +1507,7 @@
                        w.parent, d.fb2_bbox, 1, H, W, (const int32_t *)nullptr, CONN_FB_CAP, w.adjptr, d.fb_reject, zs);
     hipLaunchKernelGGL(k_lroot_labels, lgrid, 256, 0, st, d.lroots, d.ntile, n_slots, w.counters, w.parent, w.csize, w.adjptr, min_size,
                        w.newlabel, zs);
-    hipLaunchKernelGGL(k_write_labels, dim3(cdiv(cdiv(n, 4), 256), 1, nz), 256, 0, st, w.parent, w.newlabel, n, labels_out,
-                       (const int32_t *)(w.counters + CNT_FLAG), zs);
+    if (!defer_write && launch_conn_write_labels(w, n, labels_out, st, zb)) return -1;
     HIP_TRY(hipGetLastError());
     if (nz == 1) {
         HIP_TRY(hipMemcpyAsync(host_counters.data(), w.counters, 16 * sizeof(int32_t), hipMemcpyDeviceToHost, st));
@@ -1519,7 +1527,7 @@
 }
 
 int launch_enforce_connectivity_batch(const int32_t *labels_in, int H, int W, long min_size_l, long max_size_l, int start_label, ConnWork w,
-                                      int32_t *labels_out, int *n_labels_out, hipStream_t st, ZBatch zb, int32_t *stage_dev)
+                                      int32_t *labels_out, int *n_labels_out, hipStream_t st, ZBatch zb, int32_t *stage_dev, bool defer_write)
 {
     const int min_size = (int)std::min<long>(min_size_l, 0x7fffffff);
     const int max_size = (int)std::min<long>(max_size_l, 0x7fffffff);
@@ -1527,7 +1535,7 @@
     std::vector<char> ok(zb.nz);
     static_assert(sizeof(bool) == sizeof(char), "ok flags");
     if (conn_fast_2d(labels_in, H, W, min_size, max_size, start_label, w, labels_out, n_kept.data(), reinterpret_cast<bool *>(ok.data()), st, zb,
-                     stage_dev))
+                     stage_dev, defer_write))
         return -1;
     for (int b = 0; b < zb.nz; ++b) n_labels_out[b] = ok[b] ? (n_kept[b] > 0 ? start_label + n_kept[b] : 1) : -1;
     return 0;
@@ -1538,8 +1546,9 @@
 
 int launch_enforce_connectivity(const int32_t *labels_in, int D, int H, int W, long min_size_l, long max_size_l,
                                 int start_label, ConnWork w, int32_t *labels_out, int *n_labels_out_host,
-                                hipStream_t st)
-{
+                                hipStream_t st, bool *write_deferred)
+{
+    if (write_deferred) *write_deferred = false;
     const int n = D * H * W;
     const int grid = cdiv(n, 256);
     const int min_size = (int)std::min<long>(min_size_l, 0x7fffffff);
@@ -1550,9 +1559,12 @@
     if (D == 1 && !knobs().conn_general) {
         bool ok = false;
         int n_kept = 0;
-        if (conn_fast_2d(labels_in, H, W, min_size, max_size, start_label, w, labels_out, &n_kept, &ok, st)) return -1;
+        if (conn_fast_2d(labels_in, H, W, min_size, max_size, start_label, w, labels_out, &n_kept, &ok, st, ZBatch(), nullptr,
+                         write_deferred != nullptr))
+            return -1;
         if (ok) {
             *n_labels_out_host = n_kept > 0 ? start_label + n_kept : 1;
+            if (write_deferred) *write_deferred = true;
             return 0;
         }
         g_conn_general_runs.fetch_add(1);
diff --git a/pyimsegm_amd/csrc/graph.hip b/pyimsegm_amd/csrc/graph.hip
--- a/pyimsegm_amd/csrc/graph.hip
+++ b/pyimsegm_amd/csrc/graph.hip
@@ -237,18 +237,25 @@
     return 0;
 }
 
+int launch_adjacency_zero(int K, uint32_t *bitmap, long long *cacc, hipStream_t st, ZBatch zb)
+{
+    const int words = cdiv(K, 32);
+    const size_t bm_bytes = (size_t)K * words * sizeof(uint32_t), gap = (size_t)((const char *)cacc - (const char *)bitmap);
+    if ((const char *)cacc >= (const char *)bitmap + bm_bytes && gap <= bm_bytes + 64)
+        return launch_zero(bitmap, gap + (size_t)K * 3 * sizeof(long long), st, zb);
+    if (launch_zero(bitmap, bm_bytes, st, zb) || launch_zero(cacc, (size_t)K * 3 * sizeof(long long), st, zb)) return -1;
+    return 0;
+}
+
 int launch_adjacency_bitmap(const int32_t *labels, int H, int W, int K, uint32_t *bitmap, long long *cacc, double *centres_out,
-                            uint8_t *present_out, hipStream_t st, ZBatch zb)
+                            uint8_t *present_out, hipStream_t st, ZBatch zb, int sums_done)
 {
     int words = cdiv(K, 32);
-    const size_t bm_bytes = (size_t)K * words * sizeof(uint32_t), gap = (size_t)((const char *)cacc - (const char *)bitmap);
-    if ((const char *)cacc >= (const char *)bitmap + bm_bytes && gap <= bm_bytes + 64) {
-        if (launch_zero(bitmap, gap + (size_t)K * 3 * sizeof(long long), st, zb)) return -1;
-    } else {
-        if (launch_zero(bitmap, bm_bytes, st, zb) || launch_zero(cacc, (size_t)K * 3 * sizeof(long long), st, zb)) return -1;
-    }
-    dim3 grid(cdiv(W, 64), cdiv(H, 4 * GR_ROWS), zb.nz);
-    hipLaunchKernelGGL(k_adjacency_centres, grid, 256, 0, st, labels, H, W, K, words, bitmap, cacc, zb.zs);
+    if (!sums_done) {
+        if (launch_adjacency_zero(K, bitmap, cacc, st, zb)) return -1;
+        dim3 grid(cdiv(W, 64), cdiv(H, 4 * GR_ROWS), zb.nz);
+        hipLaunchKernelGGL(k_adjacency_centres, grid, 256, 0, st, labels, H, W, K, words, bitmap, cacc, zb.zs);
+    }
     hipLaunchKernelGGL(k_centres_finalize, dim3(cdiv(K, 256), 1, zb.nz), 256, 0, st, cacc, K, centres_out, present_out, zb.zs);
     HIP_TRY(hipGetLastError());
     return 0;
diff --git a/pyimsegm_amd/csrc/session.h b/pyimsegm_amd/csrc/session.h
--- a/pyimsegm_amd/csrc/session.h
+++ b/pyimsegm_amd/csrc/session.h
@@ -169,6 +169,9 @@
         tex_planes, tex_resp, tex_small, tex_aux, vol_cent, annot, hist, featK, seg, gseg, narrow;
     GraphPlan gplan;
     bool graph_ready = false;
+    bool defer_labels = false, labels_deferred = false, lc_pass1 = false, lc_adj = false;
+    int lc_K = 0, lc_Ecap = 0;
+    double lc_maxabs = 0.0;
     int *slic_fail_host = nullptr;
     int feat_mask = 0, feat_F = 0;
     int place_F = 0, place_col = 0;
diff --git a/pyimsegm_amd/csrc/slic.h b/pyimsegm_amd/csrc/slic.h
--- a/pyimsegm_amd/csrc/slic.h
+++ b/pyimsegm_amd/csrc/slic.h
@@ -149,9 +149,11 @@
 long gc_grid_fallbacks();
 int launch_enforce_connectivity(const int32_t *labels_in, int D, int H, int W, long min_size, long max_size,
                                 int start_label, ConnWork w, int32_t *labels_out, int *n_labels_out_host,
-                                hipStream_t st);
+                                hipStream_t st, bool *write_deferred = nullptr);
+int launch_conn_write_labels(const ConnWork &w, int n, int32_t *labels_out, hipStream_t st, ZBatch zb = ZBatch());
 int launch_enforce_connectivity_batch(const int32_t *labels_in, int H, int W, long min_size, long max_size, int start_label, ConnWork w,
-                                      int32_t *labels_out, int *n_labels_out, hipStream_t st, ZBatch zb, int32_t *stage_dev);
+                                      int32_t *labels_out, int *n_labels_out, hipStream_t st, ZBatch zb, int32_t *stage_dev,
+                                      bool defer_write = false);
 
 int launch_label_hist(const int32_t *labels, const int32_t *annot, size_t n, int K, int nb, unsigned long long *hist,
                       hipStream_t st);
@@ -159,7 +161,11 @@
                        int want_var, long long *acc, double *mean_out, double *energy_out, double *var_out,
                        float *mean32_scratch, hipStream_t st, int planar = 0, int prescale = 0, double mul = 1.0,
                        double div = 1.0, long plane_stride = -1, const double *ssq_dev = nullptr, ZBatch zb = ZBatch(),
-                       const double *minmax_dev = nullptr);
+                       const double *minmax_dev = nullptr, int pass1_done = 0);
+bool label_consumers_take(int H, int W);
+int launch_label_consumers(const void *img, int dtype, const int32_t *parent, const int32_t *newlabel, int32_t *labels_out, int H, int W,
+                           int K, double maxabs, long long *acc, uint32_t *bitmap, long long *cacc, hipStream_t st, ZBatch zb = ZBatch(),
+                           const double *minmax_dev = nullptr);
 
 struct SepJob {
     double *resp;
@@ -189,7 +195,8 @@
                              int32_t *edges_out, int edge_capacity, int32_t *n_edges_dev, double *centres_out,
                              uint8_t *present_out, int32_t *rowcount, hipStream_t st);
 int launch_adjacency_bitmap(const int32_t *labels, int H, int W, int K, uint32_t *bitmap, long long *cacc, double *centres_out,
-                            uint8_t *present_out, hipStream_t st, ZBatch zb = ZBatch());
+                            uint8_t *present_out, hipStream_t st, ZBatch zb = ZBatch(), int sums_done = 0);
+int launch_adjacency_zero(int K, uint32_t *bitmap, long long *cacc, hipStream_t st, ZBatch zb);
 int launch_gather_labels(const int32_t *lut, const int32_t *idx, size_t n, int32_t *out, hipStream_t st, ZBatch zb = ZBatch());
 int launch_zero(void *ptr, size_t bytes, hipStream_t st, ZBatch zb);
 int launch_copy_rows(void *dst, size_t dst_stride, const void *src, size_t src_stride, size_t bytes, int rows, hipStream_t st);
diff --git a/pyimsegm_amd/csrc/stats.hip b/pyimsegm_amd/csrc/stats.hip
--- a/pyimsegm_amd/csrc/stats.hip
+++ b/pyimsegm_amd/csrc/stats.hip
@@ -62,27 +62,13 @@
 
 template <typename T, int NC = 3, int PASS = 1> struct StatRows { static constexpr int value = (sizeof(T) == 8 || (NC == 1 && PASS == 1)) ? ST_ROWS / 2 : ST_ROWS; };
 
-template <typename T, int PASS, bool U8INT, int NC = 3>
-__global__ void __launch_bounds__(256, 4)
-k_color_stats(const T *__restrict__ img, const int32_t *__restrict__ labels, StatParams sp,
-              const float *__restrict__ mean32, long long *__restrict__ acc)
-{
-    constexpr int RW = StatRows<T, NC, PASS>::value;
-    ZSHIFT(img, sp.zs); ZSHIFT(labels, sp.zs); ZSHIFT(mean32, sp.zs); ZSHIFT(acc, sp.zs); ZSHIFT(sp.ssq_dev, sp.zs);
-    ZSHIFT(sp.minmax, sp.zs);
-    double scale_v, scale_e;
-    image_scales(sp, scale_v, scale_e);
+template <typename T, int PASS, bool U8INT, int NC, int RW, typename LabelAt>
+__device__ __forceinline__ void stats_tile(const T *__restrict__ img, const StatParams &sp, const float *__restrict__ mean32,
+                                           long long *__restrict__ acc, const double scale_v, const double scale_e, int *keys,
+                                           long long (*lacc)[13], const int x, const int y0, LabelAt label_at)
+{
     constexpr int NQ = (PASS == 1) ? 13 : 6;
-    __shared__ int keys[ST_SLOTS];
-    __shared__ long long lacc[ST_SLOTS][13];
-    const int tid = threadIdx.x, lane = tid & 63, wave = tid >> 6;
-    if (tid < ST_SLOTS) {
-        keys[tid] = -1;
-        for (int j = 0; j < NQ; ++j) lacc[tid][j] = 0;
-    }
-    __syncthreads();
-    const int x = blockIdx.x * 64 + lane;
-    const int y0 = (blockIdx.y * 4 + wave) * RW;
+    const int tid = threadIdx.x, lane = tid & 63;
     static_assert(!U8INT || (PASS == 1 && sizeof(T) == 1 && NC == 3), "integer block sums: uint8 colour image, first pass");
     int lab[RW];
     float v[RW][NC];
@@ -99,7 +85,7 @@
         const int y = y0 + r;
         const bool ok = (y < sp.H) && (x < sp.W);
         const size_t p = ok ? (size_t)y * sp.W + x : 0;
-        lab[r] = ok ? labels[p] : 0x7fffffff;
+        lab[r] = label_at(r, ok, p);
         if (NC == 3 && sizeof(T) == 1 && !sp.planar && !sp.prescale && p + 1 < sp.n_pixels) {
             uint32_t w;
             __builtin_memcpy(&w, reinterpret_cast<const uint8_t *>(img) + 3 * p, 4);
@@ -273,6 +259,138 @@
         if (val == 0) continue;
         int col = (PASS == 1) ? j : 7 + j;
         atomic_add_i64(acc + (size_t)k * 13 + col, val);
+    }
+}
+
+template <typename T, int PASS, bool U8INT, int NC = 3>
+__global__ void __launch_bounds__(256, 4)
+k_color_stats(const T *__restrict__ img, const int32_t *__restrict__ labels, StatParams sp,
+              const float *__restrict__ mean32, long long *__restrict__ acc)
+{
+    constexpr int RW = StatRows<T, NC, PASS>::value;
+    ZSHIFT(img, sp.zs); ZSHIFT(labels, sp.zs); ZSHIFT(mean32, sp.zs); ZSHIFT(acc, sp.zs); ZSHIFT(sp.ssq_dev, sp.zs);
+    ZSHIFT(sp.minmax, sp.zs);
+    double scale_v, scale_e;
+    image_scales(sp, scale_v, scale_e);
+    constexpr int NQ = (PASS == 1) ? 13 : 6;
+    __shared__ int keys[ST_SLOTS];
+    __shared__ long long lacc[ST_SLOTS][13];
+    const int tid = threadIdx.x, lane = tid & 63, wave = tid >> 6;
+    if (tid < ST_SLOTS) {
+        keys[tid] = -1;
+        for (int j = 0; j < NQ; ++j) lacc[tid][j] = 0;
+    }
+    __syncthreads();
+    const int x = blockIdx.x * 64 + lane;
+    const int y0 = (blockIdx.y * 4 + wave) * RW;
+    stats_tile<T, PASS, U8INT, NC, RW>(img, sp, mean32, acc, scale_v, scale_e, keys, lacc, x, y0,
+                                   [&](int, bool ok, size_t p) { return ok ? labels[p] : 0x7fffffff; });
+}
+
+constexpr int LC_ROWS = 8, LC_MIN_BLOCKS = 6;
+constexpr int LC_SLOTS = 128;
+constexpr int LC_MAX_SIDE = 1 << 18;
+
+template <typename T, bool U8INT>
+__global__ void __launch_bounds__(256, LC_MIN_BLOCKS)
+k_label_consumers(const T *__restrict__ img, const int32_t *__restrict__ parent, const int32_t *__restrict__ newlabel,
+                  int32_t *__restrict__ labels_out, StatParams sp, long long *__restrict__ acc, int words, uint32_t *bitmap,
+                  long long *__restrict__ cacc)
+{
+    constexpr int RW = LC_ROWS;
+    ZSHIFT(img, sp.zs); ZSHIFT(parent, sp.zs); ZSHIFT(newlabel, sp.zs); ZSHIFT(labels_out, sp.zs); ZSHIFT(acc, sp.zs);
+    ZSHIFT(bitmap, sp.zs); ZSHIFT(cacc, sp.zs); ZSHIFT(sp.ssq_dev, sp.zs); ZSHIFT(sp.minmax, sp.zs);
+    double scale_v, scale_e;
+    image_scales(sp, scale_v, scale_e);
+    __shared__ int keys[ST_SLOTS];
+    __shared__ long long lacc[ST_SLOTS][13];
+    __shared__ int h_key[LC_SLOTS], h_n[LC_SLOTS], h_sy[LC_SLOTS], h_sx[LC_SLOTS];
+    const int tid = threadIdx.x, lane = tid & 63, wave = tid >> 6;
+    if (tid < ST_SLOTS) {
+        keys[tid] = -1;
+        for (int j = 0; j < 13; ++j) lacc[tid][j] = 0;
+    }
+    if (tid < LC_SLOTS) {
+        h_key[tid] = -1;
+        h_n[tid] = 0;
+        h_sy[tid] = 0;
+        h_sx[tid] = 0;
+    }
+    __syncthreads();
+    const int H = sp.H, W = sp.W;
+    const int x = blockIdx.x * 64 + lane;
+    const int y0 = (blockIdx.y * 4 + wave) * RW;
+    const bool xin = x < W;
+    int lab[RW + 1];
+#pragma unroll
+    for (int r = 0; r <= RW; ++r) {
+        const bool ok = xin && y0 + r < H;
+        lab[r] = ok ? parent[(size_t)(y0 + r) * W + x] : -1;
+    }
+#pragma unroll
+    for (int r = 0; r <= RW; ++r) lab[r] = lab[r] >= 0 ? newlabel[lab[r]] : -1;
+    int halo = -1;
+    {
+        const int hx = blockIdx.x * 64 + 64, hy = y0 + lane;
+        if (lane < RW && hx < W && hy < H) halo = newlabel[parent[(size_t)hy * W + hx]];
+    }
+#pragma unroll
+    for (int r = 0; r < RW; ++r)
+        if (lab[r] >= 0) labels_out[(size_t)(y0 + r) * W + x] = lab[r];
+    const unsigned long long le = (lane == 63) ? ~0ULL : ((2ULL << lane) - 1ULL);
+#pragma unroll
+    for (int r = 0; r < RW; ++r) {
+        const int y = y0 + r;
+        const int l = lab[r];
+        const int right = lane_next(l, __builtin_amdgcn_readlane(halo, r));
+        const int left = lane_prev(l, -2);
+        const bool act = l >= 0;
+        if (act) {
+            const int nb[2] = { right, lab[r + 1] };
+#pragma unroll
+            for (int j = 0; j < 2; ++j) {
+                if (nb[j] < 0 || nb[j] == l) continue;
+                const int a = min(l, nb[j]), b = max(l, nb[j]);
+                uint32_t *wp = bitmap + (size_t)b * words + (a >> 5);
+                const uint32_t bit = 1u << (a & 31);
+                if (!(*wp & bit)) atomicOr(wp, bit);
+            }
+        }
+        const bool start = act && left != l;
+        const unsigned long long starts = __ballot(start);
+        const int nact = __popcll(__ballot(act));
+        if (start) {
+            const unsigned long long above = starts & ~le;
+            const int len = (above ? __ffsll((long long)above) - 1 : nact) - lane;
+            const int n = len, sy = len * y, sx = len * x + (len * (len - 1)) / 2;
+            int slot = (int)(((unsigned int)l * 2654435761u) >> 25);
+            bool placed = false;
+            for (int probe = 0; probe < LC_SLOTS; ++probe) {
+                const int old = atomicCAS(&h_key[slot], -1, l);
+                if (old == -1 || old == l) {
+                    placed = true;
+                    break;
+                }
+                slot = (slot + 1) & (LC_SLOTS - 1);
+            }
+            if (placed) {
+                atomicAdd(&h_n[slot], n);
+                atomicAdd(&h_sy[slot], sy);
+                atomicAdd(&h_sx[slot], sx);
+            } else {
+                atomic_add_i64(cacc + (size_t)l * 3 + 0, n);
+                atomic_add_i64(cacc + (size_t)l * 3 + 1, (long long)sy);
+                atomic_add_i64(cacc + (size_t)l * 3 + 2, (long long)sx);
+            }
+        }
+    }
+    stats_tile<T, 1, U8INT, 3, RW>(img, sp, nullptr, acc, scale_v, scale_e, keys, lacc, x, y0,
+                               [&](int r, bool, size_t) { return lab[r] >= 0 ? lab[r] : 0x7fffffff; });
+    if (tid < LC_SLOTS && h_key[tid] >= 0) {
+        const int k = h_key[tid];
+        atomic_add_i64(cacc + (size_t)k * 3 + 0, h_n[tid]);
+        atomic_add_i64(cacc + (size_t)k * 3 + 1, h_sy[tid]);
+        atomic_add_i64(cacc + (size_t)k * 3 + 2, h_sx[tid]);
     }
 }
 
@@ -345,14 +463,11 @@
         hipLaunchKernelGGL((k_color_stats<T, 2, false>), grid, 256, 0, st, img, labels, sp, mean32, acc);
 }
 
-int launch_color_stats(const void *img, int dtype, const int32_t *labels, int H, int W, int K, double maxabs,
-                       int want_var, long long *acc, double *mean_out, double *energy_out, double *var_out,
-                       float *mean32_scratch, hipStream_t st, int planar, int prescale, double mul, double div,
-                       long plane_stride, const double *ssq_dev, ZBatch zb, const double *minmax_dev)
+static StatParams stat_params(int dtype, int H, int W, int K, double maxabs, int planar, int prescale, double mul, double div,
+                              long plane_stride, const double *ssq_dev, ZBatch zb, const double *minmax_dev)
 {
     StatParams sp;
     sp.zs = zb.zs;
-    const unsigned nz = (unsigned)zb.nz;
     sp.H = H; sp.W = W; sp.K = K;
     sp.n_pixels = (size_t)H * W;
     sp.planar = planar; sp.prescale = prescale; sp.mul = mul; sp.div = div; sp.ssq_dev = ssq_dev;
@@ -360,11 +475,54 @@
     sp.minmax = minmax_dev;
     stat_scales((double)H * W, maxabs, sp.scale_v, sp.scale_e);
     sp.u8_int = (dtype == DT_U8 && !prescale && sp.scale_v >= 1.0 && sp.scale_e >= 1.0) ? 1 : 0;
+    return sp;
+}
+
+template <typename T, bool U8INT>
+static void launch_consumers(const void *img, const int32_t *parent, const int32_t *newlabel, int32_t *labels_out, const StatParams &sp,
+                             long long *acc, int words, uint32_t *bitmap, long long *cacc, hipStream_t st, int nz)
+{
+    const dim3 grid(cdiv(sp.W, 64), cdiv(sp.H, 4 * LC_ROWS), nz);
+    hipLaunchKernelGGL((k_label_consumers<T, U8INT>), grid, 256, 0, st, (const T *)img, parent, newlabel, labels_out, sp, acc, words, bitmap,
+                       cacc);
+}
+
+bool label_consumers_take(int H, int W) { return H >= 1 && W >= 1 && H <= LC_MAX_SIDE && W <= LC_MAX_SIDE; }
+
+int launch_label_consumers(const void *img, int dtype, const int32_t *parent, const int32_t *newlabel, int32_t *labels_out, int H, int W,
+                           int K, double maxabs, long long *acc, uint32_t *bitmap, long long *cacc, hipStream_t st, ZBatch zb,
+                           const double *minmax_dev)
+{
+    if (!label_consumers_take(H, W)) {
+        set_error("label consumers: image side beyond the 32-bit centre sums of a tile");
+        return -1;
+    }
+    const StatParams sp = stat_params(dtype, H, W, K, maxabs, 0, 0, 1.0, 1.0, -1, nullptr, zb, minmax_dev);
+    const int words = cdiv(K, 32);
+    hipLaunchKernelGGL(k_stats_clear, dim3(cdiv(K, 256), 1, (unsigned)zb.nz), 256, 0, st, acc, K, 0, 13, zb.zs);
+    if (launch_adjacency_zero(K, bitmap, cacc, st, zb)) return -1;
+    if (dtype == DT_U8 && sp.u8_int) launch_consumers<uint8_t, true>(img, parent, newlabel, labels_out, sp, acc, words, bitmap, cacc, st, zb.nz);
+    else if (dtype == DT_U8) launch_consumers<uint8_t, false>(img, parent, newlabel, labels_out, sp, acc, words, bitmap, cacc, st, zb.nz);
+    else if (dtype == DT_F32) launch_consumers<float, false>(img, parent, newlabel, labels_out, sp, acc, words, bitmap, cacc, st, zb.nz);
+    else launch_consumers<double, false>(img, parent, newlabel, labels_out, sp, acc, words, bitmap, cacc, st, zb.nz);
+    HIP_TRY(hipGetLastError());
+    return 0;
+}
+
+int launch_color_stats(const void *img, int dtype, const int32_t *labels, int H, int W, int K, double maxabs,
+                       int want_var, long long *acc, double *mean_out, double *energy_out, double *var_out,
+                       float *mean32_scratch, hipStream_t st, int planar, int prescale, double mul, double div,
+                       long plane_stride, const double *ssq_dev, ZBatch zb, const double *minmax_dev, int pass1_done)
+{
+    const StatParams sp = stat_params(dtype, H, W, K, maxabs, planar, prescale, mul, div, plane_stride, ssq_dev, zb, minmax_dev);
+    const unsigned nz = (unsigned)zb.nz;
     const dim3 kgrid(cdiv(K, 256), 1, nz);
-    hipLaunchKernelGGL(k_stats_clear, kgrid, 256, 0, st, acc, K, 0, 13, zb.zs);
-    if (dtype == DT_U8) launch_pass<uint8_t>(1, (const uint8_t *)img, labels, sp, mean32_scratch, acc, st, zb.nz);
-    else if (dtype == DT_F32) launch_pass<float>(1, (const float *)img, labels, sp, mean32_scratch, acc, st, zb.nz);
-    else launch_pass<double>(1, (const double *)img, labels, sp, mean32_scratch, acc, st, zb.nz);
+    if (!pass1_done) {
+        hipLaunchKernelGGL(k_stats_clear, kgrid, 256, 0, st, acc, K, 0, 13, zb.zs);
+        if (dtype == DT_U8) launch_pass<uint8_t>(1, (const uint8_t *)img, labels, sp, mean32_scratch, acc, st, zb.nz);
+        else if (dtype == DT_F32) launch_pass<float>(1, (const float *)img, labels, sp, mean32_scratch, acc, st, zb.nz);
+        else launch_pass<double>(1, (const double *)img, labels, sp, mean32_scratch, acc, st, zb.nz);
+    }
     hipLaunchKernelGGL(k_stats_finalize1, kgrid, 256, 0, st, acc, sp, mean_out, energy_out, mean32_scratch);
     if (want_var) {
         if (dtype == DT_U8) launch_pass<uint8_t>(2, (const uint8_t *)img, labels, sp, mean32_scratch, acc, st, zb.nz);
```

New measurement: 5636 Mpixels/s. 0.973x the previous value.
